# iPERDance/iPERCore

Hardware: AMD Instinct MI355X
Metric: synthesized frames/sec at 512x512 (run_imitator) (higher is better)
Workload: dtype f32; 1 GPU; run_imitator 512x512 single src/ref pair, 300-frame reference clip frame-sharded over 1 GPU(s), AttLWB-SPADE generator fp32 (BASELINE configs[1] at N = 1, configs[2] at N = 8); poses=imitate, image_size=512, frame_batch=300, frame_batch_requested=384, world_size=1, parallelism=frame-shard x1, batches_in_flight=1, weights=random-init (seeded) of the real architecture, 36,276,992 params

## Files before the change

### include/lwg_hip.h

```cpp
#ifndef LWG_HIP_H
#define LWG_HIP_H

#include <stddef.h>
#include <stdint.h>

#ifdef __cplusplus
extern "C" {
#endif

typedef void* lwg_stream_t;

#define LWG_ABI_VERSION 10
int lwg_abi_version(void);

#define LWG_MAX_TAPS 52
enum { LWG_EPI_NONE = 0, LWG_EPI_RESIDUAL = 1, LWG_EPI_SPADE = 2 };
enum { LWG_ACTIVATION_NONE = 0, LWG_ACTIVATION_RELU = 1, LWG_ACTIVATION_TANH = 2, LWG_ACTIVATION_SIGMOID = 3 };
#define LWG_ACTIVATION_RELU_MASK 5
enum { LWG_DT_F32 = 0, LWG_DT_BF16 = 1,
       LWG_DT_F32_Q4 = 2 };

typedef struct LwgConvArgs {
    const float* x0;
    const float* x1;
    int C0, C1;
    int B, H, W;
    int OH, OW;
    int M;
    int stride;
    int ntaps;
    int cshift;
    const float* w;
    int N;
    const float* bias;
    float* y;
    int YH, YW, YC, ycoff;
    int omul, ooy, oox;
    int epi;
    int act;
    const float* res;
    const float* xn;
    const float* mean;
    const float* rstd;
    int xdt;
    int ydt;
    signed char dy[LWG_MAX_TAPS];
    signed char dx[LWG_MAX_TAPS];
} LwgConvArgs;

int lwg_conv2d_nhwc_f32(const LwgConvArgs* args, lwg_stream_t stream);
size_t lwg_conv2d_ws_floats(const LwgConvArgs* args);
int lwg_conv2d_nhwc_f32_ws(const LwgConvArgs* args, float* ws, lwg_stream_t stream);
int lwg_conv_slice_count(const LwgConvArgs* args);

int lwg_conv2d_nhwc_bf16(const LwgConvArgs* args, lwg_stream_t stream);
int lwg_conv2d_winograd_f32(const LwgConvArgs* args, lwg_stream_t stream);
size_t lwg_conv2d_winograd_ws_floats(const LwgConvArgs* args);
int lwg_conv2d_winograd_f32_ws(const LwgConvArgs* args, float* ws, lwg_stream_t stream);
int lwg_conv2d_winograd_plan(const LwgConvArgs* args, int with_ws, long long* blocks, int* slices, int* nbv, int* workgroups);
int lwg_winograd_panel_f32(const float* wpanel, float* upk, int Cin, int N, const int* tap9, lwg_stream_t stream);
typedef struct LwgWinoDesc {
    const float* wpanel;
    float* upk;
    int Cin, N, first_block;
    int tap9[9];
} LwgWinoDesc;
int lwg_winograd_panels_f32(const LwgWinoDesc* descs_dev, int ndesc, int total_blocks, lwg_stream_t stream);
int lwg_conv2d_winograd4_f32(const LwgConvArgs* args, lwg_stream_t stream);
int lwg_winograd4_panel_f32(const float* wpanel, float* upk, int Cin, int N, const int* tap9, lwg_stream_t stream);
int lwg_conv2d_nhwc_bf16_hr(const LwgConvArgs* args, lwg_stream_t stream);
int lwg_conv2d_winograd_bf16(const LwgConvArgs* args, lwg_stream_t stream);
int lwg_conv2d_nhwc_c8_bf16(const LwgConvArgs* args, lwg_stream_t stream);
int lwg_conv_transpose4_nhwc_bf16(const LwgConvArgs* args, lwg_stream_t stream);
int lwg_conv_transpose4_nhwc_f32(const LwgConvArgs* args, lwg_stream_t stream);
int lwg_conv_transpose4_is_one_grid(const LwgConvArgs* args);
int lwg_conv_transpose4_winograd_f32(const LwgConvArgs* args, lwg_stream_t stream);

int lwg_conv_transpose4_winograd24_f32(const LwgConvArgs* args, lwg_stream_t stream);

int lwg_conv2d_nhwc_f32_split(const LwgConvArgs* args, lwg_stream_t stream);

size_t lwg_conv2d_wgrad_ws_floats(int Ktot, int N, int M);
int lwg_conv2d_wgrad_nhwc_f32(const LwgConvArgs* args, const float* dy, float* dw, float* ws, lwg_stream_t stream);
int lwg_conv2d_wgrad_unpacked_f32(const LwgConvArgs* args, const float* dy, float* ws, float* dw, int D0, int D1, int KH, int KW,
                                  int transposed, const int* kidx, int cin, int nout, float* db, lwg_stream_t stream);
int lwg_colsum_nhwc_f32(const float* x, size_t rows, int C, float* out, float* ws, lwg_stream_t stream);
size_t lwg_conv2d_wgrad_winograd_ws_floats(const LwgConvArgs* args);
int lwg_conv2d_wgrad_winograd_f32(const LwgConvArgs* args, const float* dy, float* ws, float* dw, int cin, int nout, lwg_stream_t stream);

int lwg_act_bwd_f32(const float* dy, const float* y, size_t n, int act, float* out, lwg_stream_t stream);
int lwg_norm_fwd_nhwc_f32(const float* x, const float* mean, const float* rstd, const float* gamma, const float* beta, int gstride,
                          int B, int HW, int C, int act, float* y, lwg_stream_t stream);
int lwg_norm_bwd_nhwc_f32(const float* dy, const float* y, const float* x, const float* mean, const float* rstd,
                          const float* gamma, int gstride, int B, int HW, int C, int act, int nsplit, float* dx, float* dgamma,
                          float* dbeta, float* ws, lwg_stream_t stream);
int lwg_adam_step_f32(float* p, const float* g, float* m, float* v, size_t n, float lr, float beta1, float beta2, float eps, int t,
                      lwg_stream_t stream);
int lwg_adam_step_dev_f32(float* p, const float* g, float* m, float* v, size_t n, float lr, float beta1, float beta2, float eps,
                          int* t_dev, lwg_stream_t stream);
int lwg_pack_panel_f32(const float* w, int D0, int D1, int KH, int KW, int transposed, const int* kidx, int ntaps, int cin,
                       int cin_pad, int nout, int n_pad, float* out, lwg_stream_t stream);
int lwg_unpack_wgrad_f32(const float* dwk, int D0, int D1, int KH, int KW, int transposed, const int* kidx, int ntaps, int cin,
                         int cin_pad, int nout, int n_pad, float* dw, lwg_stream_t stream);
typedef struct LwgPackDesc {
    const float* w;
    float* out;
    int D1, KHW, transposed, ntaps, cin, cin_pad, nout, n_pad, Kp, first_block;
    int kidx[LWG_MAX_TAPS];
} LwgPackDesc;
int lwg_pack_panels_f32(const LwgPackDesc* descs_dev, int ndesc, int total_blocks, lwg_stream_t stream);
int lwg_maxpool2_fwd_nhwc_f32(const float* x, float* y, int B, int H, int W, int C, lwg_stream_t stream);
int lwg_maxpool2_bwd_nhwc_f32(const float* x, const float* dy, float* dx, int B, int H, int W, int C, lwg_stream_t stream);
int lwg_crop_resize_bilinear_f32(const float* x, const long long* box, float* y, float* valid, int N, int C, int H, int W, int OH, int OW,
                                 lwg_stream_t stream);
int lwg_crop_resize_bilinear_bwd_f32(const float* dy, const long long* box, float* dx, int N, int C, int H, int W, int OH, int OW, lwg_stream_t stream);
int lwg_prelu_f32(const float* x, const float* slope, const float* res, size_t rows, int C, float* y, lwg_stream_t stream);
int lwg_prelu_bwd_f32(const float* x, const float* slope, const float* dy, size_t rows, int C, float* dx, lwg_stream_t stream);

int lwg_instnorm_stats_nhwc_f32(const float* x, int B, int HW, int C, float eps, float* mean, float* rstd,
                                float* ws, int nsplit, lwg_stream_t stream);
int lwg_instnorm_stats_nhwc_bf16(const void* x, int B, int HW, int C, float eps, float* mean, float* rstd, float* ws, int nsplit,
                                 lwg_stream_t stream);
int lwg_instnorm_apply_nhwc_f32(const float* x, const float* mean, const float* rstd, const float* res,
                                float* y, int B, int HW, int C, int act, lwg_stream_t stream);

int lwg_flow_resize_f32(const float* T, int n, int S, int h, int w, float* out, lwg_stream_t stream);
int lwg_lwb_attention_f32(const float* q, const float* Ks, const float* Vs, const float* bk, const float* bv,
                          const float* T, float* out, int B, int ns, int h, int w, int C, int S,
                          int src_batched, lwg_stream_t stream);
int lwg_lwb_attention_bf16(const void* q, const void* Ks, const void* Vs, const float* bk, const float* bv, const float* T, void* out,
                           int B, int ns, int h, int w, int C, int S, int src_batched, lwg_stream_t stream);
int lwg_lwb_attention_x_records(int h, int w, int C, int element_size);
int lwg_lwb_attention_x_f32(const float* x, const float* Kq, const float* kappa, const float* Vs, const float* bv, const float* T,
                            float* out, float* stats, int B, int ns, int h, int w, int C, int src_batched, lwg_stream_t stream);
int lwg_lwb_attention_x_bf16(const void* x, const void* Kq, const float* kappa, const void* Vs, const float* bv, const float* T,
                             void* out, float* stats, int B, int ns, int h, int w, int C, int src_batched, lwg_stream_t stream);
size_t lwg_instnorm_finalize_ws_floats(int B, int C, int nrec);
int lwg_instnorm_finalize_f32(float* ws, int B, int C, int nrec, float eps, float* mean, float* rstd, lwg_stream_t stream);
int lwg_lwb_attention_bwd_f32(const float* q, const float* Ks, const float* Vs, const float* bk, const float* bv,
                              const float* T, const float* dout, float* dq, float* dKs, float* dVs, int B, int ns,
                              int h, int w, int C, int S, int src_batched, lwg_stream_t stream);
int lwg_lwb_attention_kv_f32(const float* q, const float* kv, const float* bk, const float* bv, const float* T, float* out,
                             int B, int ns, int h, int w, int C, int S, int src_batched, lwg_stream_t stream);
int lwg_lwb_attention_kv_bwd_f32(const float* q, const float* kv, const float* bk, const float* bv, const float* T,
                                 const float* dout, float* dq, float* dkv, int B, int ns, int h, int w, int C, int S,
                                 int src_batched, lwg_stream_t stream);
int lwg_lwb_fuse_f32(const float* tsf_x, const float* src_x, const float* gate, const float* T, float* out, int B, int ns,
                     int h, int w, int C, int S, int src_batched, float scale_w, float scale_o, lwg_stream_t stream);
int lwg_lwb_fuse_bf16(const void* tsf_x, const void* src_x, const void* gate, const float* T, void* out, int B, int ns, int h, int w,
                      int C, int S, int src_batched, float scale_w, float scale_o, lwg_stream_t stream);
int lwg_lwb_fuse_bwd_f32(const float* src_x, const float* gate, const float* T, const float* dout, float* d_tsf, float* d_src,
                         float* d_gate, int B, int ns, int h, int w, int C, int S, int src_batched, float scale_w, float scale_o,
                         lwg_stream_t stream);

size_t lwg_rasterize_ws_bytes(int B, int nf, int S);
int lwg_project_faces_f32(const float* verts, const float* cam, const int32_t* faces, int B, int nv, int nf,
                          float eye_dist, float* faces_v, float* f2pts, lwg_stream_t stream);
int lwg_rasterize_fim_wim_f32(const float* faces_v, int B, int nf, int S, float near, float far, int32_t* fim,
                              float* wim, void* ws, lwg_stream_t stream);
int lwg_texture_sample_f32(const int32_t* fim, const float* wim, const float* faces_v, const float* textures, int B, int nf,
                           int S, int T, int tex_batched, float eps, const float* bg_color3_host, float* rgb, lwg_stream_t stream);

int lwg_flow_compose_f32(const int32_t* fim, const float* wim, int B, int S, const float* map_fn, int nf,
                         const float* f_uvs2img, const float* uv_img4, int Hu, int Wu, const float* src_f2pts,
                         int ns, float* tsf_inputs, float* Tst, float* cond_nchw, float* Tuv, lwg_stream_t stream);
int lwg_bc_transform_f32(const float* f2pts, const int32_t* fim, const float* wim, int B, int S, int nf, float* T,
                         lwg_stream_t stream);
int lwg_encode_fim_f32(const int32_t* fim, const float* map_fn, int B, int S, int nf, int D, float* out,
                       lwg_stream_t stream);

size_t lwg_smpl_lbs_ws_floats(int B, int nv, int nj);
int lwg_smpl_lbs_f32(const float* pose, int pose_stride, const float* beta, int beta_stride, int nbeta,
                     const float* cam, int cam_stride, const float* v_template, const float* offsets, int off_batched,
                     const float* shapedirs, const float* posedirs, const float* J_regressor, const int32_t* parents,
                     const float* lbs_weights, const int32_t* links, int nlinks, int B, int nv, int nj, float* verts,
                     float* j3d, float* j2d, float* ws, lwg_stream_t stream);

int lwg_head_compose_f32(const float* x, const float* wpk, const float* bg, size_t bg_bstride, int B, int S, int C,
                         float* pred, float* mask, float* img, lwg_stream_t stream);
int lwg_head_compose_q4_f32(const float* x, const float* wpk, const float* bg, size_t bg_bstride, int B, int S, int C,
                            float* pred, float* mask, float* img, lwg_stream_t stream);
int lwg_thin_conv_f32(const float* x, const float* wpk, int B, int S, int C, int ks, float* y, lwg_stream_t stream);
int lwg_head_compose_bf16(const void* x, const void* wb, const float* bg, size_t bg_bstride, int B, int S, int C, float* pred,
                          float* mask, float* img, lwg_stream_t stream);
int lwg_up4_head_compose_bf16(const LwgConvArgs* args, const void* whead, const float* bg, size_t bg_bstride, float* pred, float* mask, float* img,
                              lwg_stream_t stream);
int lwg_frames_to_u8(const float* pred, int B, int S, int bgr, uint8_t* out, lwg_stream_t stream);
int lwg_nchw_to_nhwc_f32(const float* src, float* dst, int B, int C, int Cp, int P, lwg_stream_t stream);
int lwg_nhwc_to_nchw_f32(const float* src, float* dst, int B, int C, int Cs, int P, lwg_stream_t stream);

int lwg_morph_f32(const float* in, float* out, int n, int H, int W, int ks, int mode, float* ws, lwg_stream_t stream);
int lwg_canny_f32(const float* sil, int n, int H, int W, const float* gauss9, const float* sobelx9, float low, float high,
                  float* edges, float* ws, lwg_stream_t stream);
int lwg_boundary_fill_f32(const float* src, const float* confidant, const float* outpad, const float* edges, int n, int H,
                          int W, float* out, int32_t* top3, int32_t* ws, lwg_stream_t stream);
int lwg_grid_sample_nchw_f32(const float* img, size_t img_bstride, const float* grid, int n, int C, int H, int W, int Ho,
                             int Wo, float* out, lwg_stream_t stream);
int lwg_uv_merge_f32(const float* src_warp, const float* vis, int ns, int H, int W, float* out, lwg_stream_t stream);
int lwg_uv_merge_parts_f32(const float* uv_imgs, const float* vis, int n, int H, int W, float* out, lwg_stream_t stream);
int lwg_pack_inputs_f32(const float* a, int Ca, const float* b, int Cb, const float* mask, int n, int H, int W, int Cp,
                        float* out, lwg_stream_t stream);

int lwg_device_cu_count(void);

#ifdef __cplusplus
}
#endif
#endif
```

### ipercore_amd/_lib.py

```python
import ctypes
import os
import re

_HERE = os.path.dirname(os.path.abspath(__file__))
LIB_PATH = os.path.join(_HERE, "liblwg_hip.so")
HEADER_PATH = os.path.join(os.path.dirname(_HERE), "include", "lwg_hip.h")

LWG_MAX_TAPS = 52
EPI_NONE, EPI_RESIDUAL, EPI_SPADE = 0, 1, 2
ACT_NONE, ACT_RELU, ACT_TANH, ACT_SIGMOID, ACT_LRELU = 0, 1, 2, 3, 4
ACT_RELU_MASK = 5
DT_F32, DT_BF16, DT_F32_Q4 = 0, 1, 2

c_f = ctypes.c_void_p
c_i = ctypes.c_int


class LwgConvArgs(ctypes.Structure):
    _fields_ = [
        ("x0", c_f), ("x1", c_f),
        ("C0", c_i), ("C1", c_i),
        ("B", c_i), ("H", c_i), ("W", c_i),
        ("OH", c_i), ("OW", c_i),
        ("M", c_i), ("stride", c_i), ("ntaps", c_i), ("cshift", c_i),
        ("w", c_f), ("N", c_i), ("bias", c_f),
        ("y", c_f), ("YH", c_i), ("YW", c_i), ("YC", c_i), ("ycoff", c_i),
        ("omul", c_i), ("ooy", c_i), ("oox", c_i),
        ("epi", c_i), ("act", c_i),
        ("res", c_f), ("xn", c_f), ("mean", c_f), ("rstd", c_f),
        ("xdt", c_i), ("ydt", c_i),
        ("dy", ctypes.c_byte * LWG_MAX_TAPS), ("dx", ctypes.c_byte * LWG_MAX_TAPS),
    ]


class LwgWinoDesc(ctypes.Structure):
    _fields_ = [("wpanel", ctypes.c_void_p), ("upk", ctypes.c_void_p), ("Cin", c_i), ("N", c_i), ("first_block", c_i), ("tap9", c_i * 9)]


class LwgPackDesc(ctypes.Structure):
    _fields_ = [("w", c_f), ("out", c_f)] + [(n, c_i) for n in ("D1", "KHW", "transposed", "ntaps", "cin", "cin_pad", "nout", "n_pad", "Kp",
                                                               "first_block")] + [("kidx", c_i * LWG_MAX_TAPS)]


_SIGS = {
    "lwg_abi_version": (c_i, []),
    "lwg_device_cu_count": (c_i, []),
    "lwg_conv2d_nhwc_f32": (c_i, [ctypes.POINTER(LwgConvArgs), c_f]),
    "lwg_conv2d_ws_floats": (ctypes.c_size_t, [ctypes.POINTER(LwgConvArgs)]),
    "lwg_conv2d_nhwc_f32_ws": (c_i, [ctypes.POINTER(LwgConvArgs), c_f, c_f]),
    "lwg_conv2d_nhwc_bf16": (c_i, [ctypes.POINTER(LwgConvArgs), c_f]),
    "lwg_conv2d_winograd_f32": (c_i, [ctypes.POINTER(LwgConvArgs), c_f]),
    "lwg_conv2d_winograd_ws_floats": (ctypes.c_size_t, [ctypes.POINTER(LwgConvArgs)]),
    "lwg_conv2d_winograd_f32_ws": (c_i, [ctypes.POINTER(LwgConvArgs), c_f, c_f]),
    "lwg_conv2d_winograd_plan": (c_i, [ctypes.POINTER(LwgConvArgs), c_i, ctypes.POINTER(ctypes.c_longlong), ctypes.POINTER(c_i), ctypes.POINTER(c_i),
                                       ctypes.POINTER(c_i)]),
    "lwg_winograd_panel_f32": (c_i, [c_f, c_f, c_i, c_i, ctypes.POINTER(c_i), c_f]),
    "lwg_winograd_panels_f32": (c_i, [c_f, c_i, c_i, c_f]),
    "lwg_conv2d_winograd4_f32": (c_i, [ctypes.POINTER(LwgConvArgs), c_f]),
    "lwg_winograd4_panel_f32": (c_i, [c_f, c_f, c_i, c_i, ctypes.POINTER(c_i), c_f]),
    "lwg_conv2d_nhwc_bf16_hr": (c_i, [ctypes.POINTER(LwgConvArgs), c_f]),
    "lwg_conv2d_winograd_bf16": (c_i, [ctypes.POINTER(LwgConvArgs), c_f]),
    "lwg_conv2d_nhwc_c8_bf16": (c_i, [ctypes.POINTER(LwgConvArgs), c_f]),
    "lwg_conv_transpose4_nhwc_bf16": (c_i, [ctypes.POINTER(LwgConvArgs), c_f]),
    "lwg_conv_transpose4_nhwc_f32": (c_i, [ctypes.POINTER(LwgConvArgs), c_f]),
    "lwg_conv_transpose4_winograd_f32": (c_i, [ctypes.POINTER(LwgConvArgs), c_f]),
    "lwg_conv_transpose4_winograd24_f32": (c_i, [ctypes.POINTER(LwgConvArgs), c_f]),
    "lwg_conv_transpose4_is_one_grid": (c_i, [ctypes.POINTER(LwgConvArgs)]),
    "lwg_conv_slice_count": (c_i, [ctypes.POINTER(LwgConvArgs)]),
    "lwg_conv2d_nhwc_f32_split": (c_i, [ctypes.POINTER(LwgConvArgs), c_f]),
    "lwg_conv2d_wgrad_ws_floats": (ctypes.c_size_t, [c_i, c_i, c_i]),
    "lwg_conv2d_wgrad_nhwc_f32": (c_i, [ctypes.POINTER(LwgConvArgs), c_f, c_f, c_f, c_f]),
    "lwg_conv2d_wgrad_unpacked_f32": (c_i, [ctypes.POINTER(LwgConvArgs), c_f, c_f, c_f] + [c_i] * 5 + [ctypes.POINTER(ctypes.c_int), c_i, c_i, c_f, c_f]),
    "lwg_colsum_nhwc_f32": (c_i, [c_f, ctypes.c_size_t, c_i, c_f, c_f, c_f]),
    "lwg_conv2d_wgrad_winograd_ws_floats": (ctypes.c_size_t, [ctypes.POINTER(LwgConvArgs)]),
    "lwg_conv2d_wgrad_winograd_f32": (c_i, [ctypes.POINTER(LwgConvArgs), c_f, c_f, c_f, c_i, c_i, c_f]),
    "lwg_act_bwd_f32": (c_i, [c_f, c_f, ctypes.c_size_t, c_i, c_f, c_f]),
    "lwg_norm_fwd_nhwc_f32": (c_i, [c_f, c_f, c_f, c_f, c_f, c_i, c_i, c_i, c_i, c_i, c_f, c_f]),
    "lwg_norm_bwd_nhwc_f32": (c_i, [c_f, c_f, c_f, c_f, c_f, c_f, c_i, c_i, c_i, c_i, c_i, c_i, c_f, c_f, c_f, c_f, c_f]),
    "lwg_adam_step_f32": (c_i, [c_f, c_f, c_f, c_f, ctypes.c_size_t, ctypes.c_float, ctypes.c_float, ctypes.c_float, ctypes.c_float, c_i, c_f]),
    "lwg_adam_step_dev_f32": (c_i, [c_f, c_f, c_f, c_f, ctypes.c_size_t, ctypes.c_float, ctypes.c_float, ctypes.c_float, ctypes.c_float, c_f, c_f]),
    "lwg_pack_panel_f32": (c_i, [c_f] + [c_i] * 5 + [ctypes.POINTER(ctypes.c_int)] + [c_i] * 5 + [c_f, c_f]),
    "lwg_pack_panels_f32": (c_i, [c_f, c_i, c_i, c_f]),
    "lwg_unpack_wgrad_f32": (c_i, [c_f] + [c_i] * 5 + [ctypes.POINTER(ctypes.c_int)] + [c_i] * 5 + [c_f, c_f]),
    "lwg_maxpool2_fwd_nhwc_f32": (c_i, [c_f, c_f, c_i, c_i, c_i, c_i, c_f]),
    "lwg_maxpool2_bwd_nhwc_f32": (c_i, [c_f, c_f, c_f, c_i, c_i, c_i, c_i, c_f]),
    "lwg_crop_resize_bilinear_f32": (c_i, [c_f, c_f, c_f, c_f, c_i, c_i, c_i, c_i, c_i, c_i, c_f]),
    "lwg_crop_resize_bilinear_bwd_f32": (c_i, [c_f, c_f, c_f, c_i, c_i, c_i, c_i, c_i, c_i, c_f]),
    "lwg_prelu_f32": (c_i, [c_f, c_f, c_f, ctypes.c_size_t, c_i, c_f, c_f]),
    "lwg_prelu_bwd_f32": (c_i, [c_f, c_f, c_f, ctypes.c_size_t, c_i, c_f, c_f]),
    "lwg_instnorm_stats_nhwc_f32": (c_i, [c_f, c_i, c_i, c_i, ctypes.c_float, c_f, c_f, c_f, c_i, c_f]),
    "lwg_instnorm_apply_nhwc_f32": (c_i, [c_f, c_f, c_f, c_f, c_f, c_i, c_i, c_i, c_i, c_f]),
    "lwg_lwb_attention_f32": (c_i, [c_f, c_f, c_f, c_f, c_f, c_f, c_f, c_i, c_i, c_i, c_i, c_i, c_i, c_i, c_f]),
    "lwg_lwb_attention_bf16": (c_i, [c_f, c_f, c_f, c_f, c_f, c_f, c_f, c_i, c_i, c_i, c_i, c_i, c_i, c_i, c_f]),
    "lwg_instnorm_stats_nhwc_bf16": (c_i, [c_f, c_i, c_i, c_i, ctypes.c_float, c_f, c_f, c_f, c_i, c_f]),
    "lwg_head_compose_bf16": (c_i, [c_f, c_f, c_f, ctypes.c_size_t, c_i, c_i, c_i, c_f, c_f, c_f, c_f]),
    "lwg_up4_head_compose_bf16": (c_i, [ctypes.POINTER(LwgConvArgs), c_f, c_f, ctypes.c_size_t, c_f, c_f, c_f, c_f]),
    "lwg_flow_resize_f32": (c_i, [c_f, c_i, c_i, c_i, c_i, c_f, c_f]),
    "lwg_lwb_fuse_f32": (c_i, [c_f] * 5 + [c_i] * 7 + [ctypes.c_float, ctypes.c_float, c_f]),
    "lwg_lwb_fuse_bf16": (c_i, [c_f] * 5 + [c_i] * 7 + [ctypes.c_float, ctypes.c_float, c_f]),
    "lwg_lwb_fuse_bwd_f32": (c_i, [c_f] * 7 + [c_i] * 7 + [ctypes.c_float, ctypes.c_float, c_f]),
    "lwg_lwb_attention_x_f32": (c_i, [c_f] * 8 + [c_i] * 6 + [c_f]),
    "lwg_lwb_attention_x_bf16": (c_i, [c_f] * 8 + [c_i] * 6 + [c_f]),
    "lwg_lwb_attention_x_records": (c_i, [c_i, c_i, c_i, c_i]),
    "lwg_instnorm_finalize_ws_floats": (ctypes.c_size_t, [c_i, c_i, c_i]),
    "lwg_instnorm_finalize_f32": (c_i, [c_f, c_i, c_i, c_i, ctypes.c_float, c_f, c_f, c_f]),
    "lwg_lwb_attention_bwd_f32": (c_i, [c_f] * 10 + [c_i] * 7 + [c_f]),
    "lwg_lwb_attention_kv_f32": (c_i, [c_f] * 6 + [c_i] * 7 + [c_f]),
    "lwg_lwb_attention_kv_bwd_f32": (c_i, [c_f] * 8 + [c_i] * 7 + [c_f]),
    "lwg_rasterize_ws_bytes": (ctypes.c_size_t, [c_i, c_i, c_i]),
    "lwg_project_faces_f32": (c_i, [c_f, c_f, c_f, c_i, c_i, c_i, ctypes.c_float, c_f, c_f, c_f]),
    "lwg_rasterize_fim_wim_f32": (c_i, [c_f, c_i, c_i, c_i, ctypes.c_float, ctypes.c_float, c_f, c_f, c_f, c_f]),
    "lwg_texture_sample_f32": (c_i, [c_f, c_f, c_f, c_f, c_i, c_i, c_i, c_i, c_i, ctypes.c_float, ctypes.POINTER(ctypes.c_float), c_f, c_f]),
    "lwg_flow_compose_f32": (c_i, [c_f, c_f, c_i, c_i, c_f, c_i, c_f, c_f, c_i, c_i, c_f, c_i, c_f, c_f, c_f, c_f, c_f]),
    "lwg_bc_transform_f32": (c_i, [c_f, c_f, c_f, c_i, c_i, c_i, c_f, c_f]),
    "lwg_encode_fim_f32": (c_i, [c_f, c_f, c_i, c_i, c_i, c_i, c_f, c_f]),
    "lwg_smpl_lbs_ws_floats": (ctypes.c_size_t, [c_i, c_i, c_i]),
    "lwg_smpl_lbs_f32": (c_i, [c_f, c_i, c_f, c_i, c_i, c_f, c_i, c_f, c_f, c_i, c_f, c_f, c_f, c_f, c_f, c_f, c_i, c_i, c_i,
                               c_i, c_f, c_f, c_f, c_f, c_f]),
    "lwg_head_compose_f32": (c_i, [c_f, c_f, c_f, ctypes.c_size_t, c_i, c_i, c_i, c_f, c_f, c_f, c_f]),
    "lwg_head_compose_q4_f32": (c_i, [c_f, c_f, c_f, ctypes.c_size_t, c_i, c_i, c_i, c_f, c_f, c_f, c_f]),
    "lwg_thin_conv_f32": (c_i, [c_f, c_f, c_i, c_i, c_i, c_i, c_f, c_f]),
    "lwg_nchw_to_nhwc_f32": (c_i, [c_f, c_f, c_i, c_i, c_i, c_i, c_f]),
    "lwg_nhwc_to_nchw_f32": (c_i, [c_f, c_f, c_i, c_i, c_i, c_i, c_f]),
    "lwg_frames_to_u8": (c_i, [c_f, c_i, c_i, c_i, c_f, c_f]),
    "lwg_morph_f32": (c_i, [c_f, c_f, c_i, c_i, c_i, c_i, c_i, c_f, c_f]),
    "lwg_canny_f32": (c_i, [c_f, c_i, c_i, c_i, ctypes.POINTER(ctypes.c_float), ctypes.POINTER(ctypes.c_float),
                            ctypes.c_float, ctypes.c_float, c_f, c_f, c_f]),
    "lwg_boundary_fill_f32": (c_i, [c_f, c_f, c_f, c_f, c_i, c_i, c_i, c_f, c_f, c_f, c_f]),
    "lwg_grid_sample_nchw_f32": (c_i, [c_f, ctypes.c_size_t, c_f, c_i, c_i, c_i, c_i, c_i, c_i, c_f, c_f]),
    "lwg_uv_merge_f32": (c_i, [c_f, c_f, c_i, c_i, c_i, c_f, c_f]),
    "lwg_uv_merge_parts_f32": (c_i, [c_f, c_f, c_i, c_i, c_i, c_f, c_f]),
    "lwg_pack_inputs_f32": (c_i, [c_f, c_i, c_f, c_i, c_f, c_i, c_i, c_i, c_i, c_f, c_f]),
}

_lib = None


def header_symbols():
    with open(HEADER_PATH) as fp:
        src = re.sub(r"/\*.*?\*/", "", fp.read(), flags=re.S)
    return sorted(set(re.findall(r"\b(lwg_[a-z0-9_]+)\s*\(", src)))


def lib():
    global _lib
    if _lib is None:
        if not os.path.exists(LIB_PATH):
            raise RuntimeError(
                f"{LIB_PATH} not found: the HIP kernels are not built (run `python -c 'import __graft_entry__ as g; "
                "g.build()'` or `make -C ipercore_amd/csrc`).  There is no CPU fallback.")
        import torch
        handle = ctypes.CDLL(LIB_PATH)
        for name, (res, args) in _SIGS.items():
            fn = getattr(handle, name)
            fn.restype = res
            fn.argtypes = args
        if handle.lwg_abi_version() != 10:
            raise RuntimeError("liblwg_hip.so ABI version mismatch")
        _lib = handle
    return _lib


def check(err, what):
    if err != 0:
        raise RuntimeError(f"{what} failed with hipError_t {err}")
```

### ipercore_amd/csrc/conv_winograd4.hip

```cpp
#include <hip/hip_runtime.h>
#include "lwg_common.h"
#include "lwg_conv_wino.h"

#define W4_THREADS 512
#define W4_PBX 8
#define W4_PBY 4
#define W4_NB 64
#define W4_KS 8
#define W4_HW 34
#define W4_HH 18
#ifndef W4_RS
#define W4_RS 40
#endif
#define W4_PLANE (18 * W4_RS + 4)
#define W4_RAW (W4_KS * W4_PLANE)
#define W4_VS (36 * W4_KS * 32)
#define W4_NEL (W4_HW * W4_HH * 2)
#define W4_NQ 3
#define W4_DUMP_OFF (2 * W4_RAW + 2 * W4_VS)
#define W4_DUMP (W4_THREADS + 3 * W4_PLANE)
#define W4_LOOP (W4_DUMP_OFF + W4_DUMP)
#define W4_MSR 68
#define W4_NPL 28
#define W4_MS (W4_NPL * 16 * W4_MSR)
#define W4_BIAS_OFF (W4_LOOP > W4_MS ? W4_LOOP : W4_MS)
#ifndef LWG_W4_XCD
#define LWG_W4_XCD 1
#endif
#ifndef LWG_W4_CHUNK
#define LWG_W4_CHUNK 1
#endif
#ifndef LWG_W4_RDMAP
#define LWG_W4_RDMAP 1
#endif
#ifndef LWG_W4_SMALL
#define LWG_W4_SMALL 1
#endif
#define W4SB() __builtin_amdgcn_sched_barrier(0)

#ifdef LWG_W4_TS
#define W4TS(i) do { if (tid == 0 && lab_bi == 1) reinterpret_cast<unsigned long long*>(const_cast<float*>(a.res))[(size_t)blockIdx.x * 16 + (i)] = __builtin_readcyclecounter(); } while (0)
#define W4TSA(i) do { if (tid == 0) reinterpret_cast<unsigned long long*>(const_cast<float*>(a.res))[(size_t)blockIdx.x * 16 + (i)] = __builtin_readcyclecounter(); } while (0)
#else
#define W4TS(i) do { } while (0)
#define W4TSA(i) do { } while (0)
#endif

#ifndef W4_NT
#define W4_NT 0
#endif
#ifndef W4_NT_LD
#define W4_NT_LD W4_NT
#endif
#ifndef W4_NT_RES
#define W4_NT_RES 0
#endif
#ifndef W4_NT_ST
#define W4_NT_ST 2
#endif

__device__ __forceinline__ void w4_bt6(const float (&r)[6], float (&v)[6]) {
    const float a = __builtin_fmaf(-4.f, r[2], r[4]), b = __builtin_fmaf(-4.f, r[1], r[3]);
    const float c = r[4] - r[2], e = r[3] - r[1];
    v[0] = __builtin_fmaf(-5.f, r[2], __builtin_fmaf(4.f, r[0], r[4]));
    v[1] = a + b;
    v[2] = a - b;
    v[3] = __builtin_fmaf(2.f, e, c);
    v[4] = __builtin_fmaf(-2.f, e, c);
    v[5] = __builtin_fmaf(-5.f, r[3], __builtin_fmaf(4.f, r[1], r[5]));
}

template <int EPI, bool TWO, bool SM = false>
__global__ __launch_bounds__(SM ? 256 : W4_THREADS, 1) void lwg_conv_winograd4_kernel(const LwgConvArgs a) {
    constexpr bool SMS = SM && EPI == LWG_EPI_SPADE;
    constexpr int NVP = SM && !SMS ? 2 : 1;
    constexpr int NTH = SM ? 256 : W4_THREADS;
    constexpr int NQ = SM ? 5 : W4_NQ;
    constexpr int NBV = SM ? 32 : W4_NB;
    constexpr int MSR = SM ? 36 : W4_MSR;
    constexpr int NHF = SM ? 2 : 1;
    extern __shared__ __attribute__((aligned(16))) float smem[];
    const int wid = __builtin_amdgcn_readfirstlane(threadIdx.x >> 6);
    const float* __restrict__ bias = a.bias;
    const int H = a.H, W = a.W, Cin = a.C0 + a.C1, N = a.N;
    float* __restrict__ y = a.y;
    float* const raw0 = smem;
    float* const Ms = smem;
    const int tid = threadIdx.x, lane = tid & 63;
    const CwGrid g = cw_grid(a.B, H, W, N, 4 * W4_PBX, 4 * W4_PBY, NBV);
    const CwOrder o = cw_order(cw4_order_kind(LWG_W4_XCD, LWG_W4_CHUNK, SM, gridDim.x, N / NBV, Cin, N, g.tiles, g.total), gridDim.x, blockIdx.x, N / NBV, g);
    int blk = blockIdx.x;
    const int nst = Cin / W4_KS;
    const __amdgpu_buffer_rsrc_t ru = __builtin_amdgcn_make_buffer_rsrc(const_cast<float*>(a.w), 0, (int)(144u * (unsigned)Cin * (unsigned)N), 0x00020000);
    const int q = wid & 3, ct = SM ? 0 : wid >> 2;
    const int half = SM ? 0 : wid >> 2;
    floatx16 acc[9];
    CwBlock<NQ, TWO> bk;
    unsigned uvoff, uvoffc;
    auto setup = [&](int id) {
        int cb, t;
        cw_block(o, id, cb, t);
        bk.locate(a, g, t, 4 * W4_PBX, 4 * W4_PBY, SMS ? cw4_n0_spade_small(cb) : cw_n0(cb, NBV));
        int tids = tid;
        asm volatile("" : "+v"(tids));
        bk.halo(a, tids, NTH, W4_HW, W4_NEL);
        const int col = SMS ? bk.n0 + (((lane & 31) >> 4) << 5) + (lane & 15) : bk.n0 + ct * 32 + (lane & 31);
        uvoff = (unsigned)(((lane >> 5) * 9 * N + 4 * col) * 4);
        uvoffc = (unsigned)(((lane >> 5) * 9 * N + 8 * N + col) * 4);
    };
    setup(blk);
    int wst[NQ];
#pragma unroll
    for (int k = 0; k < NQ; ++k) {
        const int i = tid + NTH * k;
        const int pix = i >> 1, hq = i & 1, hy = pix / W4_HW, hx = pix - hy * W4_HW;
        wst[k] = i < W4_NEL ? 4 * hq * W4_PLANE + hy * W4_RS + hx : W4_DUMP_OFF + tid;
    }
    floatx4 rreg[NQ];
    auto rld1 = [&](int st, int k) -> floatx4 {
#ifdef W4_LAB_HFIX
        const int c = 0 * st;
#else
        const int c = st * W4_KS;
#endif
        return bk.template rld1<W4_NT_LD>(a, c, k);
    };
    auto rst1 = [&](int buf, int k, floatx4 v) { cw_rst1(raw0 + buf * W4_RAW + wst[k], W4_PLANE, v); };
    floatx4 ufa[4], ufb[4];
    float ufc[4];
    const unsigned ukk = (unsigned)N * 72u;
    const unsigned uq = (unsigned)q * (unsigned)nst * 4u * ukk;
    const unsigned ubo = (unsigned)N * 16u;
    auto uldpart = [&](int set, int st, int kk, int part) {
#ifdef W4_LAB_UFIX
        const unsigned so = uq + 0u * (unsigned)(st + kk);
#else
        const unsigned so = uq + (unsigned)(st * 4 + kk) * ukk;
#endif
        if (part == 0) ufa[set] = cw_buf_load(ru, uvoff, so);
        else if (part == 1) ufb[set] = cw_buf_load(ru, uvoff, so + ubo);
        else ufc[set] = __builtin_bit_cast(float, __builtin_amdgcn_raw_buffer_load_b32(ru, (int)uvoffc, (int)so, 0));
    };
    auto uldset = [&](int set, int st, int kk) {
#ifdef W4_LAB_UFIX
        const unsigned so = uq + 0u * (unsigned)(st + kk);
#else
        const unsigned so = uq + (unsigned)(st * 4 + kk) * ukk;
#endif
        ufa[set] = cw_buf_load(ru, uvoff, so);
        ufb[set] = cw_buf_load(ru, uvoff, so + ubo);
        ufc[set] = __builtin_bit_cast(float, __builtin_amdgcn_raw_buffer_load_b32(ru, (int)uvoffc, (int)so, 0));
    };
    const int patch = tid & 31, tc = (tid >> 5) & 7;
    const int pty = patch >> 3, ptx = patch & 7;
    unsigned dbs = (unsigned)(tc * W4_PLANE + (4 * pty) * W4_RS + 4 * ptx) >> 2;
    asm volatile("" : "+v"(dbs));
    dbs <<= 2;
    unsigned dbx[NHF], vbx[NHF], vbt[NHF];
    float alpha[NHF], beta[NHF], nbeta[NHF];
#pragma unroll
    for (int hi = 0; hi < NHF; ++hi) {
        const int hf = SM ? hi : half;
        dbx[hi] = (unsigned)(tc * W4_PLANE + (4 * pty + hf) * W4_RS + 4 * ptx) >> 2;
        asm volatile("" : "+v"(dbx[hi]));
        dbx[hi] <<= 2;
        vbx[hi] = (unsigned)(2 * W4_RAW + (hf ? 30 : 0) * W4_KS * 32 + tc * 32 + patch);
        vbt[hi] = (unsigned)(2 * W4_RAW + (hf ? 18 : 6) * W4_KS * 32 + tc * 32 + patch);
        asm volatile("" : "+v"(vbx[hi]));
        asm volatile("" : "+v"(vbt[hi]));
        alpha[hi] = hf ? -1.f : -4.f;
        beta[hi] = hf ? 2.f : 1.f;
        nbeta[hi] = -beta[hi];
    }
    unsigned fbs[2];
    fbs[0] = (unsigned)(2 * W4_RAW + (6 * q) * W4_KS * 32 + lane);
    fbs[1] = (unsigned)(2 * W4_RAW + (6 * (4 + (q >> 1)) + 3 * (q & 1)) * W4_KS * 32 + lane);
    asm volatile("" : "+v"(fbs[0]));
    asm volatile("" : "+v"(fbs[1]));
    float fb[9];
    auto frag1 = [&](int buf, int kk, int j) -> float {
        return smem[fbs[j < 6 ? 0 : 1] + buf * W4_VS + ((j < 6 ? j : j - 6) * W4_KS + 2 * kk) * 32];
    };
    auto rd6 = [&](unsigned base, int buf, int r, float (&d)[6]) {
        const floatx4 v4 = *reinterpret_cast<const floatx4*>(smem + base + buf * W4_RAW + r * W4_RS);
        const float2 v2 = *reinterpret_cast<const float2*>(smem + base + buf * W4_RAW + r * W4_RS + 4);
        d[0] = v4[0]; d[1] = v4[1]; d[2] = v4[2]; d[3] = v4[3]; d[4] = v2.x; d[5] = v2.y;
    };
    auto vst6 = [&](unsigned base, int buf, int i, const float (&v)[6]) {
        float* dst = smem + base + buf * W4_VS + (6 * i) * W4_KS * 32;
#pragma unroll
        for (int nu = 0; nu < 6; ++nu) dst[nu * W4_KS * 32] = v[nu];
    };
    auto transform_full = [&](int buf) {
#pragma unroll
        for (int hi = 0; hi < NHF; ++hi) {
            float X[6], P[6], Q[6], v[6];
            {
                float dR[3][6];
                rd6(dbx[hi], buf, 0, dR[0]); rd6(dbx[hi], buf, 2, dR[1]); rd6(dbx[hi], buf, 4, dR[2]);
#pragma unroll
                for (int j = 0; j < 6; ++j) X[j] = __builtin_fmaf(-5.f, dR[1][j], __builtin_fmaf(4.f, dR[0][j], dR[2][j]));
            }
            {
                float dR[2][6];
                rd6(dbs, buf, 2, dR[0]); rd6(dbs, buf, 4, dR[1]);
#pragma unroll
                for (int j = 0; j < 6; ++j) P[j] = __builtin_fmaf(alpha[hi], dR[0][j], dR[1][j]);
                rd6(dbs, buf, 1, dR[0]); rd6(dbs, buf, 3, dR[1]);
#pragma unroll
                for (int j = 0; j < 6; ++j) Q[j] = __builtin_fmaf(alpha[hi], dR[0][j], dR[1][j]);
            }
            w4_bt6(X, v); vst6(vbx[hi], buf, 0, v);
            float T[6];
#pragma unroll
            for (int j = 0; j < 6; ++j) T[j] = __builtin_fmaf(beta[hi], Q[j], P[j]);
            w4_bt6(T, v); vst6(vbt[hi], buf, 0, v);
#pragma unroll
            for (int j = 0; j < 6; ++j) T[j] = __builtin_fmaf(nbeta[hi], Q[j], P[j]);
            w4_bt6(T, v); vst6(vbt[hi], buf, 1, v);
        }
    };
    auto iteration = [&](int s, auto SET, auto NXT) {
        constexpr int set = decltype(SET)::value;
        constexpr bool nxt = decltype(NXT)::value != 0;
        const int s3 = s + 3 < nst ? s + 3 : nst - 1;
        float X[6], P[6], Q[6], dR[3][6];
        auto mf = [&](int kk, int j, bool refill) {
            acc[j] = __builtin_amdgcn_mfma_f32_32x32x2f32(j < 4 ? ufa[kk][j & 3] : j < 8 ? ufb[kk][j & 3] : ufc[kk], fb[j], acc[j], 0, 0, 0);
#ifndef W4_KO_FRAG
            if (refill && (j & 1)) {
                fb[j - 1] = kk < 3 ? frag1(set, kk + 1, j - 1) : frag1(set ^ 1, 0, j - 1);
                fb[j] = kk < 3 ? frag1(set, kk + 1, j) : frag1(set ^ 1, 0, j);
            } else if (refill && j == 8) {
                fb[8] = kk < 3 ? frag1(set, kk + 1, 8) : frag1(set ^ 1, 0, 8);
            }
#endif
            W4SB();
        };
        auto ul = [&](int kk, int part) {
#ifndef W4_KO_ULD
            if (kk < 2) uldpart(kk + 2, s, kk + 2, part);
            else if (nxt) uldpart(kk - 2, s + 1, kk - 2, part);
#endif
            W4SB();
        };
        auto halo = [&](int k) {
#ifdef W4_KO_HALO
            return;
#endif
            if (nxt) { rst1(set, k, rreg[k]); rreg[k] = rld1(s3, k); }
            W4SB();
        };
#ifdef W4_KO_TR
        constexpr bool trn = false;
#else
        constexpr bool trn = nxt;
#endif
        auto tr = [&](int hi, int step) {
            if (trn) {
                if (step < 3) rd6(dbx[hi], set ^ 1, 2 * step, dR[step]);
                else if (step < 5) {
#pragma unroll
                    for (int j = 3 * (step - 3); j < 3 * (step - 3) + 3; ++j) X[j] = __builtin_fmaf(-5.f, dR[1][j], __builtin_fmaf(4.f, dR[0][j], dR[2][j]));
                } else if (step < 7) rd6(dbs, set ^ 1, 2 * (step - 5) + 2, dR[step - 5]);
                else if (step == 7) {
                    float v[6];
                    w4_bt6(X, v);
                    vst6(vbx[hi], set ^ 1, 0, v);
                } else if (step == 8) {
#pragma unroll
                    for (int j = 0; j < 6; ++j) P[j] = __builtin_fmaf(alpha[hi], dR[0][j], dR[1][j]);
                } else if (step < 11) rd6(dbs, set ^ 1, 2 * (step - 9) + 1, dR[step - 9]);
                else if (step == 11) {
#pragma unroll
                    for (int j = 0; j < 6; ++j) Q[j] = __builtin_fmaf(alpha[hi], dR[0][j], dR[1][j]);
                } else {
                    float T[6], v[6];
#pragma unroll
                    for (int j = 0; j < 6; ++j) T[j] = __builtin_fmaf(step == 12 ? beta[hi] : nbeta[hi], Q[j], P[j]);
                    w4_bt6(T, v);
                    vst6(vbt[hi], set ^ 1, step - 12, v);
                }
            }
            W4SB();
        };
        if constexpr (!SM) {
            mf(0, 0, true); ul(0, 0);
            mf(0, 1, true); halo(0);
            mf(0, 2, true); ul(0, 1); tr(0, 0);
            mf(0, 3, true); halo(1); tr(0, 1);
            mf(0, 4, true); ul(0, 2); tr(0, 2);
            mf(0, 5, true); halo(2);
            mf(0, 6, true); tr(0, 3);
            mf(0, 7, true); tr(0, 4);
            mf(0, 8, true); tr(0, 5);
            mf(1, 0, true); ul(1, 0); tr(0, 6);
            mf(1, 1, true); tr(0, 7);
            mf(1, 2, true); ul(1, 1); tr(0, 8); tr(0, 9);
            mf(1, 3, true); tr(0, 10);
            mf(1, 4, true); ul(1, 2);
            mf(1, 5, true); tr(0, 11);
            mf(1, 6, true); tr(0, 12);
            mf(1, 7, true);
            mf(1, 8, true); tr(0, 13);
            mf(2, 0, true); ul(2, 0);
            mf(2, 1, true);
            mf(2, 2, true); ul(2, 1);
            mf(2, 3, true);
            mf(2, 4, true); ul(2, 2);
            mf(2, 5, true); mf(2, 6, true); mf(2, 7, true); mf(2, 8, true);
        } else {
            mf(0, 0, true); ul(0, 0); halo(0);
            mf(0, 1, true); tr(0, 0);
            mf(0, 2, true); ul(0, 1); tr(0, 1);
            mf(0, 3, true); halo(1); tr(0, 2);
            mf(0, 4, true); ul(0, 2); tr(0, 3);
            mf(0, 5, true); halo(2); tr(0, 4);
            mf(0, 6, true); tr(0, 5);
            mf(0, 7, true); halo(3); tr(0, 6);
            mf(0, 8, true); tr(0, 7);
            mf(1, 0, true); ul(1, 0); tr(0, 8); tr(0, 9);
            mf(1, 1, true); halo(4); tr(0, 10);
            mf(1, 2, true); ul(1, 1); tr(0, 11);
            mf(1, 3, true); tr(0, 12);
            mf(1, 4, true); ul(1, 2); tr(0, 13);
            mf(1, 5, true); tr(1, 0);
            mf(1, 6, true); tr(1, 1);
            mf(1, 7, true); tr(1, 2);
            mf(1, 8, true); tr(1, 3);
            mf(2, 0, true); ul(2, 0); tr(1, 4);
            mf(2, 1, true); tr(1, 5);
            mf(2, 2, true); ul(2, 1); tr(1, 6);
            mf(2, 3, true); tr(1, 7);
            mf(2, 4, true); ul(2, 2); tr(1, 8); tr(1, 9);
            mf(2, 5, true); tr(1, 10);
            mf(2, 6, true); tr(1, 11);
            mf(2, 7, true); tr(1, 12);
            mf(2, 8, true); tr(1, 13);
        }
        __syncthreads();
        W4SB();
        mf(3, 0, nxt); ul(3, 0);
        mf(3, 1, nxt);
        mf(3, 2, nxt); ul(3, 1);
        mf(3, 3, nxt);
        mf(3, 4, nxt); ul(3, 2);
        mf(3, 5, nxt); mf(3, 6, nxt); mf(3, 7, nxt); mf(3, 8, nxt);
    };

    floatx4 r0[NQ], r1[NQ];
    float bq;
    auto issue_loads = [&]() {
        bq = bias ? bias[SMS ? bk.n0 + (((tid & 31) >> 4) << 5) + (tid & 15) : bk.n0 + (tid & (NBV - 1))] : 0.f;
#pragma unroll
        for (int k = 0; k < NQ; ++k) {
            r0[k] = rld1(0, k);
            r1[k] = rld1(1, k);
        }
        uldset(0, 0, 0);
        uldset(1, 0, 1);
#pragma unroll
        for (int k = 0; k < NQ; ++k) rreg[k] = rld1(nst > 2 ? 2 : 1, k);
    };
    issue_loads();
#ifdef LWG_W4_TS
    int lab_bi = 0;
#endif
    W4TSA(11);
    for (;;) {
    W4TS(0);
#pragma unroll
    for (int k = 0; k < NQ; ++k) {
        rst1(0, k, r0[k]);
        rst1(1, k, r1[k]);
    }
    if (tid < NBV) smem[W4_BIAS_OFF + tid] = bq;
    __syncthreads();
    transform_full(0);
    __syncthreads();
#pragma unroll
    for (int j = 0; j < 9; ++j) fb[j] = frag1(0, 0, j);
#pragma unroll
    for (int j = 0; j < 9; ++j)
#pragma unroll
        for (int r = 0; r < 16; ++r) acc[j][r] = 0.f;
    if (q == 1) {
#pragma unroll
        for (int g = 0; g < 4; ++g) {
            const floatx4 b4 = *reinterpret_cast<const floatx4*>(smem + W4_BIAS_OFF + ct * 32 + 8 * g + 4 * (lane >> 5));
#pragma unroll
            for (int k = 0; k < 4; ++k) acc[1][4 * g + k] = b4[k];
        }
    }
    W4TS(1);
    {
        int s = 0;
        for (; s + 2 < nst; s += 2) {
            iteration(s, IntC<0>(), IntC<1>());
            iteration(s + 1, IntC<1>(), IntC<1>());
        }
        iteration(s, IntC<0>(), IntC<1>());
        iteration(s + 1, IntC<1>(), IntC<0>());
    }
    W4TS(2);
    const int eb = bk.b, ex0 = bk.x0, ey0 = bk.y0, en0 = bk.n0;
#pragma unroll
    for (int r = 0; r < 16; ++r) {
        const float m0 = acc[0][r], m1 = acc[1][r], m2 = acc[2][r], m3 = acc[3][r], m4 = acc[4][r], m5 = acc[5][r];
        const float s12 = m1 + m2, d12 = m1 - m2, s34 = m3 + m4, d34 = m3 - m4;
        acc[0][r] = (m0 + s12) + s34;
        acc[1][r] = __builtin_fmaf(2.f, d34, d12);
        acc[2][r] = __builtin_fmaf(4.f, s34, s12);
        acc[3][r] = __builtin_fmaf(8.f, d34, d12) + m5;
    }
    if (q & 1) {
#pragma unroll
        for (int r = 0; r < 16; ++r) {
            const float h0 = acc[6][r], h1 = acc[7][r];
            acc[6][r] = h0 + h1;
            acc[7][r] = h0 - h1;
        }
    } else {
#pragma unroll
        for (int r = 0; r < 16; ++r) {
            const float h0 = acc[6][r], h1 = acc[7][r], h2 = acc[8][r];
            acc[6][r] = (h0 + h1) + h2;
            acc[7][r] = h1 - h2;
            acc[8][r] = h1 + h2;
        }
    }
    W4TS(4);
    int tide = tid;
    asm volatile("" : "+v"(tide));
    const int lanee = tide & 63;
    const int rb = wid & 3;
    const unsigned l5 = (unsigned)lanee & 31u, gsel = (0x0FF0F00Fu >> l5) & 1u;
    const int gidx = __builtin_popcount((gsel ? 0x0FF0F00Fu : 0xF00F0FF0u) & ((1u << l5) - 1u));
    const int p16 = LWG_W4_RDMAP && !SM ? (wid >> 2) * 4 + 2 * (lanee >> 5) + (gsel ? 0 : 1) + 8 * (gidx >> 3) : (wid >> 2) * 8 + (lanee >> 3);
    const int n4 = SMS ? (lanee & 3) * 4 : LWG_W4_RDMAP && !SM ? (gidx & 7) * 4 : (lanee & 7) * 4;
    const int cbase = SMS ? (en0 >> 6) * 32 + ((en0 >> 4) & 1) * 16 : en0 >> 1;
    floatx4 mu, rs;
    if (EPI == LWG_EPI_SPADE) {
        mu = *reinterpret_cast<const floatx4*>(a.mean + (size_t)eb * a.YC + cbase + n4);
        rs = *reinterpret_cast<const floatx4*>(a.rstd + (size_t)eb * a.YC + cbase + n4);
    }
    typedef unsigned int w4_u4 __attribute__((ext_vector_type(4)));
    const unsigned img_bytes = (unsigned)(H * W) * (unsigned)a.YC * 4u;
    const __amdgpu_buffer_rsrc_t ry = __builtin_amdgcn_make_buffer_rsrc(y + (size_t)eb * H * W * a.YC, 0, (int)img_bytes, 0x00020000);
    const float* const esrc = EPI == LWG_EPI_SPADE ? a.xn : EPI == LWG_EPI_RESIDUAL ? a.res : a.y;
    const __amdgpu_buffer_rsrc_t re = __builtin_amdgcn_make_buffer_rsrc(const_cast<float*>(esrc) + (size_t)eb * H * W * a.YC, 0, (int)img_bytes, 0x00020000);
    const int chan = EPI == LWG_EPI_SPADE ? cbase + n4 : a.ycoff + en0 + n4;
    bool more = false;
    int nblk = blk;
#pragma unroll
    for (int ph = 0; ph < 2; ++ph) {
        if (ph == 1) __syncthreads();
        if (((lanee >> 4) & 1) == ph) {
            float* dst = Ms + (lanee & 15) * MSR + ct * 32 + 4 * (lanee >> 5);
#pragma unroll
            for (int g = 0; g < 4; ++g) {
#pragma unroll
                for (int bb = 0; bb < 4; ++bb)
                    *reinterpret_cast<floatx4*>(dst + (4 * q + bb) * 16 * MSR + 8 * g) = floatx4{acc[bb][4 * g], acc[bb][4 * g + 1], acc[bb][4 * g + 2], acc[bb][4 * g + 3]};
#pragma unroll
                for (int i = 0; i < 3; ++i)
                    *reinterpret_cast<floatx4*>(dst + (16 + 3 * q + i) * 16 * MSR + 8 * g) = floatx4{acc[6 + i][4 * g], acc[6 + i][4 * g + 1], acc[6 + i][4 * g + 2], acc[6 + i][4 * g + 3]};
            }
        }
        unsigned vo[NVP][4];
#pragma unroll
        for (int hp = 0; hp < NVP; ++hp) {
            const int p = ph * 16 + (SMS ? lanee >> 2 : SM ? 8 * hp + (lanee >> 3) : p16);
            const int ox = ex0 + 4 * (p & 7) + rb, oyb = ey0 + 4 * (p >> 3);
#pragma unroll
            for (int i = 0; i < 4; ++i)
                vo[hp][i] = cw4_out_voff(ox, oyb + i, H, W, a.YC, chan);
        }
        floatx4 ext[2][4];
        if (EPI != LWG_EPI_NONE) {
#pragma unroll
            for (int h = 0; h < (EPI == LWG_EPI_SPADE ? 1 : 2); ++h)
#pragma unroll
                for (int i = 0; i < 4; ++i) ext[h][i] = __builtin_bit_cast(floatx4, __builtin_amdgcn_raw_buffer_load_b128(re, (int)cw4_out_group(vo[NVP == 2 ? h : 0][i], h, !SM), 0, W4_NT_RES));
        }
        if (ph == 1) {
            W4TS(8);
            nblk = blk + (int)gridDim.x;
            more = cw_has_block(o, nblk);
            setup(more ? nblk : blk);
            W4TS(9);
            issue_loads();
            W4TS(10);
        }
        __syncthreads();
        if (ph == 0) W4TS(5); else W4TS(7);
        floatx4 gam[4];
#pragma unroll
        for (int h = 0; h < 2; ++h) {
            const float* base = Ms + (SMS ? lanee >> 2 : SM ? 8 * h + (lanee >> 3) : p16) * MSR + (SMS ? h * 16 : SM ? 0 : h * 32) + n4;
            floatx4 F[6];
#pragma unroll
            for (int xi = 0; xi < 4; ++xi) F[xi] = *reinterpret_cast<const floatx4*>(base + (4 * xi + rb) * 16 * MSR);
            const int ia = rb == 0 ? 0 : rb == 2 ? 2 : 1, ib = (rb & 1) ? 4 : 3;
            const float cb = (float)(1 << rb);
#pragma unroll
            for (int r = 0; r < 2; ++r) {
                const float* hb = base + (16 + 6 * r) * 16 * MSR;
                const floatx4 pa = *reinterpret_cast<const floatx4*>(hb + ia * 16 * MSR);
                const floatx4 pb = *reinterpret_cast<const floatx4*>(hb + ib * 16 * MSR);
                floatx4 f;
#pragma unroll
                for (int c = 0; c < 4; ++c) f[c] = __builtin_fmaf(cb, pb[c], pa[c]);
                if (rb == 3) f += *reinterpret_cast<const floatx4*>(hb + 5 * 16 * MSR);
                F[4 + r] = f;
            }
            floatx4 o[4];
#pragma unroll
            for (int c = 0; c < 4; ++c) {
                const float s12 = F[1][c] + F[2][c], d12 = F[1][c] - F[2][c], s34 = F[3][c] + F[4][c], d34 = F[3][c] - F[4][c];
                o[0][c] = (F[0][c] + s12) + s34;
                o[1][c] = __builtin_fmaf(2.f, d34, d12);
                o[2][c] = __builtin_fmaf(4.f, s34, s12);
                o[3][c] = __builtin_fmaf(8.f, d34, d12) + F[5][c];
            }
            if (EPI == LWG_EPI_SPADE) {
                if (h == 0) {
#pragma unroll
                    for (int i = 0; i < 4; ++i) gam[i] = o[i];
                    continue;
                }
#pragma unroll
                for (int i = 0; i < 4; ++i)
#pragma unroll
                    for (int c = 0; c < 4; ++c) o[i][c] = (ext[0][i][c] - mu[c]) * rs[c] * (1.f + gam[i][c]) + o[i][c];
            } else if (EPI == LWG_EPI_RESIDUAL) {
                if (a.act == LWG_ACT_RELU_MASK) {
#pragma unroll
                    for (int i = 0; i < 4; ++i)
#pragma unroll
                        for (int c = 0; c < 4; ++c) o[i][c] = ext[h][i][c] > 0.f ? o[i][c] : 0.f;
                } else {
#pragma unroll
                    for (int i = 0; i < 4; ++i) o[i] += ext[h][i];
                }
            }
            lwg_act_dispatch(a.act, [&](auto ACTC) {
                constexpr int EA = decltype(ACTC)::value;
#pragma unroll
                for (int i = 0; i < 4; ++i)
#pragma unroll
                    for (int c = 0; c < 4; ++c) o[i][c] = lwg_act_c<EA>(o[i][c], a.act);
            });
#pragma unroll
            for (int i = 0; i < 4; ++i)
                __builtin_amdgcn_raw_buffer_store_b128(__builtin_bit_cast(w4_u4, o[i]), ry, (int)cw4_out_group(vo[NVP == 2 ? h : 0][i], h, EPI != LWG_EPI_SPADE && !SM), 0, W4_NT_ST);
        }
        if (ph == 0) W4TS(6);
    }
    W4TS(3);
#ifdef LWG_W4_TS
    ++lab_bi;
#endif
    if (!more) break;
    blk = nblk;
    __syncthreads();
    }
    W4TSA(12);
#ifdef LWG_W4_TS
    if (tid == 0) reinterpret_cast<unsigned long long*>(const_cast<float*>(a.res))[(size_t)blockIdx.x * 16 + 13] = (unsigned long long)lab_bi;
#endif
}


__global__ __launch_bounds__(256) void lwg_winograd4_panel_kernel(const float* __restrict__ wp, float* __restrict__ U, int Cin, int N, LwgWinoTaps taps) {
    const int n = blockIdx.x * 64 + (threadIdx.x & 63), c = blockIdx.y * 4 + (threadIdx.x >> 6);
    if (n >= N || c >= Cin) return;
    double g[3][3];
#pragma unroll
    for (int r = 0; r < 3; ++r)
#pragma unroll
        for (int s = 0; s < 3; ++s) {
            const int k = ((c >> 5) * 9 + taps.t[3 * r + s]) * 32 + (c & 31);
            g[r][s] = (double)wp[((size_t)(k >> 2) * N + n) * 4 + (k & 3)];
        }
    const double G[6][3] = {{1.0 / 4, 0, 0}, {-1.0 / 6, -1.0 / 6, -1.0 / 6}, {-1.0 / 6, 1.0 / 6, -1.0 / 6}, {1.0 / 24, 1.0 / 12, 1.0 / 6}, {1.0 / 24, -1.0 / 12, 1.0 / 6}, {0, 0, 1}};
    double t[6][3];
#pragma unroll
    for (int i = 0; i < 6; ++i)
#pragma unroll
        for (int s = 0; s < 3; ++s) t[i][s] = G[i][0] * g[0][s] + G[i][1] * g[1][s] + G[i][2] * g[2][s];
    const int s8 = c >> 3, kk = (c & 7) >> 1, kh = c & 1;
#pragma unroll
    for (int qq = 0; qq < 4; ++qq) {
        float* dst = U + ((((size_t)qq * (Cin >> 3) + s8) * 4 + kk) * 2 + kh) * 9 * (size_t)N;
        float o[9];
#pragma unroll
        for (int j = 0; j < 9; ++j) {
            const int xi = j < 6 ? qq : 4 + (qq >> 1), nu = j < 6 ? j : 3 * (qq & 1) + (j - 6);
            o[j] = (float)(t[xi][0] * G[nu][0] + t[xi][1] * G[nu][1] + t[xi][2] * G[nu][2]);
        }
        *reinterpret_cast<floatx4*>(dst + 4 * n) = floatx4{o[0], o[1], o[2], o[3]};
        *reinterpret_cast<floatx4*>(dst + 4 * (size_t)N + 4 * n) = floatx4{o[4], o[5], o[6], o[7]};
        dst[8 * (size_t)N + n] = o[8];
    }
}

extern "C" int lwg_winograd4_panel_f32(const float* wpanel, float* upk, int Cin, int N, const int* tap9, lwg_stream_t stream_) {
    LwgWinoTaps taps;
    if (!cw_panel_args_ok(wpanel, upk, Cin, N, tap9, taps)) return (int)hipErrorInvalidValue;
    hipLaunchKernelGGL(lwg_winograd4_panel_kernel, dim3((unsigned)((N + 63) / 64), (unsigned)((Cin + 3) / 4)), dim3(256), 0,
                       reinterpret_cast<hipStream_t>(stream_), wpanel, upk, Cin, N, taps);
    return (int)hipGetLastError();
}

template <int EPI, bool SM>
static int lwg_wino4_go(const LwgConvArgs& a, dim3 grid, size_t lds, hipStream_t stream) {
    return a.C1 > 0 ? cw_launch<lwg_conv_winograd4_kernel<EPI, true, SM>>(grid, SM ? 256 : W4_THREADS, lds, stream, a)
                    : cw_launch<lwg_conv_winograd4_kernel<EPI, false, SM>>(grid, SM ? 256 : W4_THREADS, lds, stream, a);
}

extern "C" int lwg_conv2d_winograd4_f32(const LwgConvArgs* pa, lwg_stream_t stream_) {
    hipStream_t stream = reinterpret_cast<hipStream_t>(stream_);
    if (!pa || !cw_contract_ok(*pa, 144ull, 256ll)) return (int)hipErrorInvalidValue;
    const LwgConvArgs& a = *pa;
    const size_t lds = (size_t)(W4_BIAS_OFF + 64) * 4;
    const int cus = lwg_device_cus();
    long long total = cw_total_blocks(a.B, a.H, a.W, a.N, 4 * W4_PBX, 4 * W4_PBY, W4_NB);
    const bool sm = LWG_W4_SMALL && 2 * total <= cus;
    if (sm) total *= 2;
    const dim3 grid = cw_persistent_grid(total, cus);
    if (a.epi == LWG_EPI_SPADE) return sm ? lwg_wino4_go<LWG_EPI_SPADE, true>(a, grid, lds, stream) : lwg_wino4_go<LWG_EPI_SPADE, false>(a, grid, lds, stream);
    if (a.epi == LWG_EPI_RESIDUAL) return sm ? lwg_wino4_go<LWG_EPI_RESIDUAL, true>(a, grid, lds, stream) : lwg_wino4_go<LWG_EPI_RESIDUAL, false>(a, grid, lds, stream);
    return sm ? lwg_wino4_go<LWG_EPI_NONE, true>(a, grid, lds, stream) : lwg_wino4_go<LWG_EPI_NONE, false>(a, grid, lds, stream);
}
```

### ipercore_amd/csrc/lwb_attn_x.hip

```cpp
#include "lwg_common.h"
#include "lwg_conv_args.h"

typedef unsigned int uintx4 __attribute__((ext_vector_type(4)));

template <typename ST> struct AttnXTraits;
template <> struct AttnXTraits<float> {
    static constexpr int CPL = 4;
    __device__ static __forceinline__ void unpack(const uintx4 v, float (&f)[4]) {
#pragma unroll
        for (int k = 0; k < 4; ++k) {
            const unsigned u = v[k];
            f[k] = __builtin_bit_cast(float, u);
        }
    }
    __device__ static __forceinline__ uintx4 pack(const float (&f)[4]) {
        uintx4 v;
#pragma unroll
        for (int k = 0; k < 4; ++k) v[k] = __builtin_bit_cast(unsigned, f[k]);
        return v;
    }
};
template <> struct AttnXTraits<__bf16> {
    static constexpr int CPL = 8;
    __device__ static __forceinline__ void unpack(const uintx4 v, float (&f)[8]) {
#pragma unroll
        for (int k = 0; k < 4; ++k) {
            f[2 * k] = __builtin_bit_cast(float, v[k] << 16);
            f[2 * k + 1] = __builtin_bit_cast(float, v[k] & 0xffff0000u);
        }
    }
    __device__ static __forceinline__ uintx4 pack(const float (&f)[8]) {
        typedef __bf16 bf16x2 __attribute__((ext_vector_type(2)));
        uintx4 v;
#pragma unroll
        for (int k = 0; k < 4; ++k) {
            bf16x2 p;
            p[0] = (__bf16)f[2 * k];
            p[1] = (__bf16)f[2 * k + 1];
            v[k] = __builtin_bit_cast(unsigned, p);
        }
        return v;
    }
};

template <typename ST, int LPP, bool STATS, int NSU, int PW, int OCC, bool PIPE = false>
__global__ __launch_bounds__(256 * PW, PW == 1 ? OCC : 1) void lwg_lwb_attnx_kernel(const ST* __restrict__ x, const ST* __restrict__ Kq,
                                                                 const float* __restrict__ kappa, const ST* __restrict__ Vs,
                                                                 const float* __restrict__ bv, const float* __restrict__ T,
                                                                 ST* __restrict__ out, float* __restrict__ stats, int B, int ns, int h, int w,
                                                                 int src_batched) {
    using TR = AttnXTraits<ST>;
    constexpr int CPL = TR::CPL;
    constexpr int C = CPL * LPP;
    constexpr int PPW = 64 / LPP;
    constexpr int PPP = 4 * PPW;
    constexpr int NPASS = 64 / PPP;
    constexpr int NIT = NPASS / PW;
    static_assert(NPASS % PW == 0, "PW must divide the tile's pass count");
    constexpr int NT = NSU > 0 ? NSU : 1;
    constexpr unsigned ROWB = (unsigned)C * sizeof(ST);
    const int lane = threadIdx.x & 63, wid = threadIdx.x >> 6;
    const int wq = wid & 3, pl = wid >> 2;
    const int cl = lane % LPP, pg = lane / LPP;
    const int tiles_x = (w + 7) >> 3;
    int tile, b;
    if (LWG_ATTNX_INTERLEAVE) {
        const int xcd = blockIdx.x & 7;
        const long idx = blockIdx.x >> 3;
        const long grp = idx / B;
        tile = (int)(grp * 8 + xcd);
        b = (int)(idx - grp * B);
        if (tile >= tiles_x * ((h + 7) >> 3)) return;
    } else {
        const long L = lwg_xcd_remap(blockIdx.x, gridDim.x);
        tile = (int)(L / B);
        b = (int)(L - (long)tile * B);
    }
    const int ty = tile / tiles_x, tx = tile - ty * tiles_x;
    const int hw = h * w;
    const unsigned nsrc = (unsigned)(src_batched ? B * ns : ns);
    __amdgpu_buffer_rsrc_t rK = __builtin_amdgcn_make_buffer_rsrc(const_cast<ST*>(Kq), 0, (int)(nsrc * (unsigned)hw * ROWB), 0x00020000);
    __amdgpu_buffer_rsrc_t rV = __builtin_amdgcn_make_buffer_rsrc(const_cast<ST*>(Vs), 0, (int)(nsrc * (unsigned)hw * ROWB), 0x00020000);
    __amdgpu_buffer_rsrc_t rA = __builtin_amdgcn_make_buffer_rsrc(const_cast<float*>(kappa), 0, (int)(nsrc * (unsigned)hw * 4u), 0x00020000);
    const float inv_sqrt_c = 1.0f / sqrtf((float)C);
    constexpr bool BV_REG = CPL == 4 || LWG_ATTNX_BVREG16;
    float bvr[CPL];
    if (BV_REG) {
#pragma unroll
        for (int k = 0; k < CPL; ++k) bvr[k] = bv[CPL * cl + k];
    }
    const float2* Tb = reinterpret_cast<const float2*>(T) + (size_t)b * ns * hw;

    auto pixel_of = [&](int pass, int& yc, int& xc) -> bool {
        const int p = pass * PPP + wq * PPW + pg;
        const int y = ty * 8 + (p >> 3), xx = tx * 8 + (p & 7);
        const bool live = y < h && xx < w;
        yc = live ? y : ty * 8;
        xc = live ? xx : tx * 8;
        return live;
    };
    extern __shared__ __attribute__((aligned(16))) char smem_ax[];
    char* xs = smem_ax;
    float2* Tl = reinterpret_cast<float2*>(smem_ax + NPASS * 4096);
    {
        __amdgpu_buffer_rsrc_t rX = __builtin_amdgcn_make_buffer_rsrc(const_cast<ST*>(x) + (size_t)b * hw * C, 0, (int)((unsigned)hw * ROWB), 0x00020000);
#pragma unroll
        for (int it = 0; it < NIT; ++it) {
            const int pass = it * PW + pl;
            int yc, xc;
            pixel_of(pass, yc, xc);
            const unsigned voff = (unsigned)(yc * w + xc) * ROWB + (unsigned)(CPL * cl) * (unsigned)sizeof(ST);
            __builtin_amdgcn_raw_ptr_buffer_load_lds(rX, (__attribute__((address_space(3))) void*)(xs + (pass * 4 + wq) * 1024), 16, (int)voff, 0, 0, 0);
        }
        for (int i = threadIdx.x; i < ns * 64; i += 256 * PW) {
            const int s = i >> 6, p = i & 63;
            const int y = ty * 8 + (p >> 3), xx = tx * 8 + (p & 7);
            const bool in = y < h && xx < w;
            Tl[i] = Tb[(size_t)s * hw + (size_t)(in ? y : ty * 8) * w + (in ? xx : tx * 8)];
        }
        asm volatile("s_waitcnt vmcnt(0)" ::: "memory");
        __syncthreads();
    }
    auto x_row = [&](int pass) -> uintx4 { return *reinterpret_cast<const uintx4*>(xs + ((pass * 4 + wq) * 64 + lane) * 16); };

    float shift[CPL], s1[CPL], s2[CPL];
    if (STATS) {
        TR::unpack(*reinterpret_cast<const uintx4*>(xs + cl * 16), shift);
#pragma unroll
        for (int k = 0; k < CPL; ++k) s1[k] = s2[k] = 0.f;
    }
    int nlive = 0;
    auto stats_add = [&](const float (&xv)[CPL]) {
        ++nlive;
        if (PW == 1) {
#pragma unroll
            for (int k = 0; k < CPL; ++k) {
                const float d = xv[k] - shift[k];
                s1[k] += d;
                s2[k] = __builtin_fmaf(d, d, s2[k]);
            }
        }
    };
    auto taps_of = [&](const float2 t, float (&wt)[4], int& tx0, int& ty0) {
        const float ix = ((t.x + 1.f) * (float)w - 1.f) * 0.5f, iy = ((t.y + 1.f) * (float)h - 1.f) * 0.5f;
        const float fx0 = floorf(ix), fy0 = floorf(iy);
        const float wx1 = ix - fx0, wy1 = iy - fy0, wx0 = (fx0 + 1.f) - ix, wy0 = (fy0 + 1.f) - iy;
        tx0 = (int)fminf(fmaxf(fx0, -2.f), (float)w + 1.f);
        ty0 = (int)fminf(fmaxf(fy0, -2.f), (float)h + 1.f);
        wt[0] = wy0 * wx0; wt[1] = wy0 * wx1; wt[2] = wy1 * wx0; wt[3] = wy1 * wx1;
    };
    auto fold = [&](const float (&ka)[CPL], const float (&va)[CPL], float kap, const float (&xv)[CPL], float& mrun, float& lrun, float (&o)[CPL]) {
        float dot = 0.f;
#pragma unroll
        for (int k = 0; k < CPL; ++k) dot = __builtin_fmaf(ka[k], xv[k], dot);
#pragma unroll
        for (int off = LPP >> 1; off > 0; off >>= 1) dot += __shfl_xor(dot, off, 64);
        const float logit = (dot + kap) * inv_sqrt_c;
        const float mnew = fmaxf(mrun, logit);
        const float corr = expf(mrun - mnew);
        const float pr = expf(logit - mnew);
        lrun = __builtin_fmaf(lrun, corr, pr);
#pragma unroll
        for (int k = 0; k < CPL; ++k) o[k] = __builtin_fmaf(o[k], corr, pr * va[k]);
        mrun = mnew;
    };
    auto finish = [&](long gp, float lrun, const float (&o)[CPL]) {
        const float invl = 1.f / lrun;
        float r[CPL];
        if (!BV_REG) {
#pragma unroll
            for (int k = 0; k < CPL; k += 4) {
                const floatx4 b4 = *reinterpret_cast<const floatx4*>(bv + CPL * cl + k);
#pragma unroll
                for (int j = 0; j < 4; ++j) bvr[k + j] = b4[j];
            }
        }
#pragma unroll
        for (int k = 0; k < CPL; ++k) r[k] = __builtin_fmaf(o[k], invl, bvr[k]);
        *reinterpret_cast<uintx4*>(out + gp * C + CPL * cl) = TR::pack(r);
    };

    if constexpr (PIPE) {
        static_assert(NSU == 2 && PW == 1 && (NIT % 2) == 0, "the pipelined form is the ns = 2 frame-batch form");
        bool mine = false;
#pragma unroll 1
        for (int it = 0; it < NIT; ++it) {
            int yc, xc;
            const bool live = pixel_of(it, yc, xc);
            const int ptile = it * PPP + wq * PPW + pg;
#pragma unroll
            for (int s = 0; s < 2; ++s) {
                const float2 t = Tl[s * 64 + ptile];
                float wt[4];
                int tx0, ty0;
                taps_of(t, wt, tx0, ty0);
                mine |= live && tx0 >= -1 && tx0 < w && ty0 >= -1 && ty0 < h;
            }
        }
        if (__syncthreads_or(mine ? 1 : 0) == 0) {
#pragma unroll 1
            for (int it = 0; it < NIT; ++it) {
                int yc, xc;
                const bool live = pixel_of(it, yc, xc);
                float xv[CPL];
                TR::unpack(x_row(it), xv);
                if (live) {
                    if (STATS) stats_add(xv);
                    float o[CPL];
#pragma unroll
                    for (int k = 0; k < CPL; ++k) o[k] = 0.f;
                    finish(((long)b * h + yc) * w + xc, 2.f, o);
                }
            }
        } else {
            struct Taps { uintx4 kr[2][4], vr[2][4]; float ar[2][4], wt[2][4]; };
            auto issue = [&](int pass, Taps& g) {
                int yc, xc;
                const bool live = pixel_of(pass, yc, xc);
                const int ptile = pass * PPP + wq * PPW + pg;
#pragma unroll
                for (int s = 0; s < 2; ++s) {
                    int tx0, ty0;
                    taps_of(Tl[s * 64 + ptile], g.wt[s], tx0, ty0);
                    const unsigned pbase = (unsigned)(src_batched ? b * ns + s : s) * (unsigned)hw;
#pragma unroll
                    for (int tp = 0; tp < 4; ++tp) {
                        const int tyy = ty0 + (tp >> 1), txx = tx0 + (tp & 1);
                        const bool ok = live && tyy >= 0 && tyy < h && txx >= 0 && txx < w;
                        const unsigned pix = pbase + (unsigned)(tyy * w + txx);
                        const unsigned voff = ok ? pix * ROWB + (unsigned)(CPL * cl) * (unsigned)sizeof(ST) : 0xC0000000u;
                        g.kr[s][tp] = __builtin_bit_cast(uintx4, __builtin_amdgcn_raw_buffer_load_b128(rK, (int)voff, 0, 0));
                        g.vr[s][tp] = __builtin_bit_cast(uintx4, __builtin_amdgcn_raw_buffer_load_b128(rV, (int)voff, 0, 0));
                        g.ar[s][tp] = __builtin_bit_cast(float, __builtin_amdgcn_raw_buffer_load_b32(rA, ok ? (int)(pix * 4u) : (int)0xC0000000u, 0, 0));
                    }
                }
            };
            auto consume = [&](int pass, const Taps& g) {
                int yc, xc;
                const bool live = pixel_of(pass, yc, xc);
                float xv[CPL];
                TR::unpack(x_row(pass), xv);
                if (STATS && live) stats_add(xv);
                float mrun = -INFINITY, lrun = 0.f;
                float o[CPL];
#pragma unroll
                for (int k = 0; k < CPL; ++k) o[k] = 0.f;
#pragma unroll
                for (int s = 0; s < 2; ++s) {
                    float ka[CPL], va[CPL], kap = 0.f;
#pragma unroll
                    for (int k = 0; k < CPL; ++k) ka[k] = va[k] = 0.f;
#pragma unroll
                    for (int tp = 0; tp < 4; ++tp) {
                        float k8[CPL], v8[CPL];
                        TR::unpack(g.kr[s][tp], k8);
                        TR::unpack(g.vr[s][tp], v8);
#pragma unroll
                        for (int k = 0; k < CPL; ++k) {
                            ka[k] = __builtin_fmaf(k8[k], g.wt[s][tp], ka[k]);
                            va[k] = __builtin_fmaf(v8[k], g.wt[s][tp], va[k]);
                        }
                        kap = __builtin_fmaf(g.ar[s][tp], g.wt[s][tp], kap);
                    }
                    fold(ka, va, kap, xv, mrun, lrun, o);
                }
                if (live) finish(((long)b * h + yc) * w + xc, lrun, o);
            };
            Taps g0, g1;
            issue(0, g0);
#pragma unroll 1
            for (int it = 0; it < NIT; it += 2) {
                issue(it + 1, g1);
                consume(it, g0);
                issue(it + 2 < NIT ? it + 2 : it + 1, g0);
                consume(it + 1, g1);
            }
        }
    } else {
#pragma unroll 1
    for (int it = 0; it < NIT; ++it) {
        const int pass = it * PW + pl;
        int yc, xc;
        const bool live = pixel_of(pass, yc, xc);
        const long gp = ((long)b * h + yc) * w + xc;
        const int ptile = pass * PPP + wq * PPW + pg;
        float xv[CPL];
        TR::unpack(x_row(pass), xv);
        if (STATS && live) stats_add(xv);
        float mrun = -INFINITY, lrun = 0.f;
        float o[CPL];
#pragma unroll
        for (int k = 0; k < CPL; ++k) o[k] = 0.f;

        auto source = [&](int s, const float2 t) {
            float wt[4];
            int tx0, ty0;
            taps_of(t, wt, tx0, ty0);
            const bool any_tap = live && tx0 >= -1 && tx0 < w && ty0 >= -1 && ty0 < h;
            float ka[CPL], va[CPL], kap = 0.f;
#pragma unroll
            for (int k = 0; k < CPL; ++k) ka[k] = va[k] = 0.f;
            if (__builtin_amdgcn_ballot_w64(any_tap) != 0ull) {
                const unsigned sidx = (unsigned)(src_batched ? b * ns + s : s);
                const unsigned pbase = sidx * (unsigned)hw;
                uintx4 kr[4], vr[4];
                float ar[4];
#pragma unroll
                for (int tp = 0; tp < 4; ++tp) {
                    const int tyy = ty0 + (tp >> 1), txx = tx0 + (tp & 1);
                    const bool ok = live && tyy >= 0 && tyy < h && txx >= 0 && txx < w;
                    const unsigned pix = pbase + (unsigned)(tyy * w + txx);
                    const unsigned voff = ok ? pix * ROWB + (unsigned)(CPL * cl) * (unsigned)sizeof(ST) : 0xC0000000u;
                    kr[tp] = __builtin_bit_cast(uintx4, __builtin_amdgcn_raw_buffer_load_b128(rK, (int)voff, 0, 0));
                    vr[tp] = __builtin_bit_cast(uintx4, __builtin_amdgcn_raw_buffer_load_b128(rV, (int)voff, 0, 0));
                    ar[tp] = __builtin_bit_cast(float, __builtin_amdgcn_raw_buffer_load_b32(rA, ok ? (int)(pix * 4u) : (int)0xC0000000u, 0, 0));
                }
#pragma unroll
                for (int tp = 0; tp < 4; ++tp) {
                    float k8[CPL], v8[CPL];
                    TR::unpack(kr[tp], k8);
                    TR::unpack(vr[tp], v8);
#pragma unroll
                    for (int k = 0; k < CPL; ++k) {
                        ka[k] = __builtin_fmaf(k8[k], wt[tp], ka[k]);
                        va[k] = __builtin_fmaf(v8[k], wt[tp], va[k]);
                    }
                    kap = __builtin_fmaf(ar[tp], wt[tp], kap);
                }
            }
            fold(ka, va, kap, xv, mrun, lrun, o);
        };
        if (NSU > 0) {
#pragma unroll
            for (int s = 0; s < NT; ++s) source(s, Tl[s * 64 + ptile]);
        } else {
#pragma unroll 1
            for (int s = 0; s < ns; ++s) source(s, Tl[s * 64 + ptile]);
        }
        if (live) finish(gp, lrun, o);
    }
    }

    if (STATS) {
        if (PW > 1) {
            __shared__ float acc[4][64][2 * CPL];
            if (pl == 0) {
#pragma unroll
                for (int k = 0; k < 2 * CPL; ++k) acc[wq][lane][k] = 0.f;
            }
            __syncthreads();
#pragma unroll 1
            for (int p = 0; p < NPASS; ++p) {
                if (pl == p % PW) {
                    int yc, xc;
                    if (pixel_of(p, yc, xc)) {
                        float xv[CPL];
                        TR::unpack(x_row(p), xv);
#pragma unroll
                        for (int k = 0; k < CPL; ++k) {
                            const float d = xv[k] - shift[k];
                            acc[wq][lane][k] += d;
                            acc[wq][lane][CPL + k] = __builtin_fmaf(d, d, acc[wq][lane][CPL + k]);
                        }
                    }
                }
                __syncthreads();
            }
            if (pl == 0) {
#pragma unroll
                for (int k = 0; k < CPL; ++k) {
                    s1[k] = acc[wq][lane][k];
                    s2[k] = acc[wq][lane][CPL + k];
                }
            }
        }
        __syncthreads();
        float (*sh)[2][C] = reinterpret_cast<float (*)[2][C]>(smem_ax);
        float* shn = reinterpret_cast<float*>(smem_ax + 4 * 2 * C * sizeof(float));
        float fn = (float)nlive;
#pragma unroll
        for (int off = LPP; off < 64; off <<= 1) {
#pragma unroll
            for (int k = 0; k < CPL; ++k) {
                s1[k] += __shfl_xor(s1[k], off, 64);
                s2[k] += __shfl_xor(s2[k], off, 64);
            }
            fn += __shfl_xor(fn, off, 64);
        }
        if (pg == 0) {
            if (pl == 0) {
#pragma unroll
                for (int k = 0; k < CPL; ++k) {
                    sh[wq][0][CPL * cl + k] = s1[k];
                    sh[wq][1][CPL * cl + k] = s2[k];
                }
            }
            if (cl == 0) shn[wid] = fn;
        }
        __syncthreads();
        if (wid == 0 && pg == 0) {
            float tn = 0.f;
#pragma unroll
            for (int k = 0; k < 4 * PW; ++k) tn += shn[k];
            const int nrec = tiles_x * ((h + 7) >> 3);
#pragma unroll
            for (int k = 0; k < CPL; ++k) {
                const int c = CPL * cl + k;
                const float t1 = ((sh[0][0][c] + sh[1][0][c]) + sh[2][0][c]) + sh[3][0][c];
                const float t2 = ((sh[0][1][c] + sh[1][1][c]) + sh[2][1][c]) + sh[3][1][c];
                const float mean = shift[k] + t1 / tn;
                const float m2 = t2 - t1 * t1 / tn;
                float* rec = stats + (((size_t)b * nrec + tile) * C + c) * 3;
                rec[0] = tn;
                rec[1] = mean;
                rec[2] = m2 > 0.f ? m2 : 0.f;
            }
        }
    }
}

extern "C" int lwg_lwb_attention_x_records(int h, int w, int C, int esz) {
    if (h <= 0 || w <= 0 || C <= 0 || (esz != 2 && esz != 4)) return 0;
    const int lpp = C / (16 / esz);
    if (lpp < 8 || lpp > 64 || (lpp & (lpp - 1)) != 0) return 0;
    return ((w + 7) >> 3) * ((h + 7) >> 3);
}

template <typename ST>
static int lwg_attnx_launch(const ST* x, const ST* Kq, const float* kappa, const ST* Vs, const float* bv, const float* T, ST* out, float* stats,
                            int B, int ns, int h, int w, int C, int src_batched, hipStream_t stream) {
    if (!x || !Kq || !kappa || !Vs || !bv || !T || !out || B <= 0 || ns <= 0 || ns > 64 || h <= 0 || w <= 0) return (int)hipErrorInvalidValue;
    const unsigned long long nsrc = (unsigned long long)(src_batched ? B * ns : ns);
    if (nsrc * (unsigned long long)h * w * (unsigned long long)C * sizeof(ST) >= 0xC0000000ull) return (int)hipErrorInvalidValue;
    const long tiles = (long)((w + 7) >> 3) * ((h + 7) >> 3);
    constexpr int CPL = AttnXTraits<ST>::CPL;
    const int npass = (C / CPL) / 4;
    const dim3 grid((unsigned)((LWG_ATTNX_INTERLEAVE ? (tiles + 7) / 8 * 8 : tiles) * B));
    const bool wide = LWG_ATTNX_WIDE && tiles * B < 512 && npass >= 4;
#define LWG_ATTNX_GO(LPP, ST_, NSU, PW)                                                                                              \
    {                                                                                                                                \
             \
        constexpr bool pipe = LWG_ATTNX_PIPE && CPL == 4 && (LPP) == 64 && (NSU) == 2 && (PW) == 1;                                  \
        auto kern = lwg_lwb_attnx_kernel<ST, LPP, ST_, NSU, PW, (pipe ? 2 : CPL == 4 ? LWG_ATTNX_OCC : LWG_ATTNX_OCC16), pipe>;        \
        const size_t lds = (size_t)((LPP) / 4) * 4096 + (size_t)ns * 512;                         \
        static unsigned long long lds_ok = 0;                                                                                        \
        if (lds > 65536) {                                                                                                           \
            const hipError_t e = lwg_allow_dynamic_lds(reinterpret_cast<const void*>(kern), lds, lds_ok);                            \
            if (e != hipSuccess) return (int)e;                                                                                      \
        }                                                                                                                            \
        hipLaunchKernelGGL(kern, grid, dim3(256 * PW), lds, stream, x, Kq, kappa, Vs, bv, T, out, stats, B, ns, h, w, src_batched);   \
    }
#define LWG_ATTNX_PW(LPP, ST_, NSU)                                                                                                  \
    {                                                                                                                                \
        if constexpr ((LPP) / 4 >= 4) {                                                                                              \
            if (wide) LWG_ATTNX_GO(LPP, ST_, NSU, 4) else LWG_ATTNX_GO(LPP, ST_, NSU, 1)                                             \
        } else {                                                                                                                     \
            LWG_ATTNX_GO(LPP, ST_, NSU, 1)                                                                                           \
        }                                                                                                                            \
    }
#define LWG_ATTNX_LAUNCH(LPP)                                                                                                        \
    if (stats) { if (LWG_ATTNX_NSU2 && ns == 2) LWG_ATTNX_PW(LPP, true, 2) else LWG_ATTNX_PW(LPP, true, 0) }                         \
    else { if (LWG_ATTNX_NSU2 && ns == 2) LWG_ATTNX_PW(LPP, false, 2) else LWG_ATTNX_PW(LPP, false, 0) }
    switch (C / CPL) {
        case 8: LWG_ATTNX_LAUNCH(8) break;
        case 16: LWG_ATTNX_LAUNCH(16) break;
        case 32: LWG_ATTNX_LAUNCH(32) break;
        case 64: if constexpr (CPL == 4) { LWG_ATTNX_LAUNCH(64) break; }
                 return (int)hipErrorInvalidValue;
        default: return (int)hipErrorInvalidValue;
    }
#undef LWG_ATTNX_LAUNCH
#undef LWG_ATTNX_PW
#undef LWG_ATTNX_GO
    return (int)hipGetLastError();
}

extern "C" int lwg_lwb_attention_x_f32(const float* x, const float* Kq, const float* kappa, const float* Vs, const float* bv, const float* T,
                                       float* out, float* stats, int B, int ns, int h, int w, int C, int src_batched, lwg_stream_t stream_) {
    if (C != 32 && C != 64 && C != 128 && C != 256) return (int)hipErrorInvalidValue;
    return lwg_attnx_launch<float>(x, Kq, kappa, Vs, bv, T, out, stats, B, ns, h, w, C, src_batched, reinterpret_cast<hipStream_t>(stream_));
}

extern "C" int lwg_lwb_attention_x_bf16(const void* x, const void* Kq, const float* kappa, const void* Vs, const float* bv, const float* T,
                                        void* out, float* stats, int B, int ns, int h, int w, int C, int src_batched, lwg_stream_t stream_) {
    if (C != 64 && C != 128 && C != 256) return (int)hipErrorInvalidValue;
    return lwg_attnx_launch<__bf16>(static_cast<const __bf16*>(x), static_cast<const __bf16*>(Kq), kappa, static_cast<const __bf16*>(Vs), bv, T,
                                    static_cast<__bf16*>(out), stats, B, ns, h, w, C, src_batched, reinterpret_cast<hipStream_t>(stream_));
}

__global__ __launch_bounds__(1024) void lwg_in_stats_merge_seg(const float* __restrict__ ws, int C, int nrec, int nseg, float eps,
                                                              float* __restrict__ part, float* __restrict__ mean, float* __restrict__ rstd) {
    const int lane = threadIdx.x & 63, wid = threadIdx.x >> 6;
    const int c = blockIdx.x * 64 + lane, b = blockIdx.y, seg = blockIdx.z;
    const bool cok = c < C;
    const float* base = ws + ((size_t)b * nrec * C + (cok ? c : 0)) * 3;
    const float r = base[1];
    const int per = (nrec + nseg - 1) / nseg;
    const int r0 = seg * per, r1 = min(nrec, r0 + per);
    float sa = 0.f, ss = 0.f, sq = 0.f;
    if (cok) {
        for (int i = r0 + wid; i < r1; i += 16) {
            const float* o = base + (size_t)i * C * 3;
            const float n = o[0], d = o[1] - r;
            sa += n;
            ss = __builtin_fmaf(n, d, ss);
            sq += __builtin_fmaf(n * d, d, o[2]);
        }
    }
    __shared__ float sh[16][3][64];
    sh[wid][0][lane] = sa;
    sh[wid][1][lane] = ss;
    sh[wid][2][lane] = sq;
    __syncthreads();
    if (wid == 0 && cok) {
        float ta = 0.f, ts = 0.f, tq = 0.f;
#pragma unroll
        for (int k = 0; k < 16; ++k) { ta += sh[k][0][lane]; ts += sh[k][1][lane]; tq += sh[k][2][lane]; }
        if (nseg == 1) {
            const float m2 = tq - ts * ts / ta;
            mean[(size_t)b * C + c] = r + ts / ta;
            rstd[(size_t)b * C + c] = 1.0f / sqrtf((m2 > 0.f ? m2 : 0.f) / ta + eps);
        } else {
            float* o = part + (((size_t)b * nseg + seg) * C + c) * 3;
            o[0] = ta; o[1] = ts; o[2] = tq;
        }
    }
}

__global__ __launch_bounds__(256) void lwg_in_stats_merge_fin(const float* __restrict__ ws, const float* __restrict__ part, int BC, int C, int nrec,
                                                             int nseg, float eps, float* __restrict__ mean, float* __restrict__ rstd) {
    const int i = blockIdx.x * 256 + threadIdx.x;
    if (i >= BC) return;
    const int b = i / C, c = i - b * C;
    const float r = ws[((size_t)b * nrec * C + c) * 3 + 1];
    float ta = 0.f, ts = 0.f, tq = 0.f;
    for (int s = 0; s < nseg; ++s) {
        const float* o = part + (((size_t)b * nseg + s) * C + c) * 3;
        ta += o[0]; ts += o[1]; tq += o[2];
    }
    const float m2 = tq - ts * ts / ta;
    mean[i] = r + ts / ta;
    rstd[i] = 1.0f / sqrtf((m2 > 0.f ? m2 : 0.f) / ta + eps);
}

extern "C" size_t lwg_instnorm_finalize_ws_floats(int B, int C, int nrec) {
    if (B <= 0 || C <= 0 || nrec <= 0) return 0;
    const size_t nseg = nrec > 512 ? (size_t)(nrec + 255) / 256 : 0;
    return (size_t)B * nrec * C * 3 + (size_t)B * nseg * C * 3;
}
extern "C" int lwg_instnorm_finalize_f32(float* ws, int B, int C, int nrec, float eps, float* mean, float* rstd, lwg_stream_t stream_) {
    if (!ws || !mean || !rstd || B <= 0 || C <= 0 || nrec <= 0 || B > 65535) return (int)hipErrorInvalidValue;
    hipStream_t stream = reinterpret_cast<hipStream_t>(stream_);
    const int nseg = nrec > 512 ? (nrec + 255) / 256 : 1;
    if (nseg > 65535) return (int)hipErrorInvalidValue;
    float* part = ws + (size_t)B * nrec * C * 3;
    hipLaunchKernelGGL(lwg_in_stats_merge_seg, dim3((C + 63) / 64, B, nseg), dim3(1024), 0, stream, ws, C, nrec, nseg, eps, part, mean, rstd);
    if (nseg > 1)
        hipLaunchKernelGGL(lwg_in_stats_merge_fin, dim3((B * C + 255) / 256), dim3(256), 0, stream, ws, part, B * C, C, nrec, nseg, eps, mean, rstd);
    return (int)hipGetLastError();
}
```

### ipercore_amd/csrc/lwg_conv_wino.h

```cpp
#pragma once
#include <stddef.h>
#include "lwg_conv_args.h"

#ifdef __HIPCC__
#define CW_FN __host__ __device__ __forceinline__
#else
#define CW_FN static inline
#endif
#ifdef __HIP_DEVICE_COMPILE__
#define CW_UNIFORM(v) __builtin_amdgcn_readfirstlane(v)
#else
#define CW_UNIFORM(v) (v)
#endif
#define CW_OOB 0xC0000000u
#define CW_KS 8
#define CW_NB 64
struct CwGrid { int bx, by, tiles, total; };
CW_FN CwGrid cw_grid(int B, int H, int W, int N, int ex, int ey, int nbv) {
    const int bx = (W + ex - 1) / ex, by = (H + ey - 1) / ey, tiles = bx * by * B;
    return CwGrid{bx, by, tiles, tiles * (N / nbv)};
}
CW_FN long long cw_total_blocks(int B, int H, int W, int N, int ex, int ey, int nbv) {
    return (long long)((W + ex - 1) / ex) * ((H + ey - 1) / ey) * B * (N / nbv);
}

enum { CW_COLMAJOR = 0, CW_CHUNK = 1, CW_XCD = 2 };
struct CwOrder { int kind, nwg, wg, ncb, tiles, total, xg, xr; };

CW_FN int cw4_order_kind(int xcd_sw, int chunk_sw, bool sm, unsigned nwg, int ncb, int Cin, int N, int tiles, int total) {
    const bool xcd = xcd_sw && !sm && (nwg & 7u) == 0 && (ncb == 4 || ncb == 8 || (ncb == 2 && (Cin >= 192 || xcd_sw == 2))) && (int)nwg < total && tiles >= (int)nwg / ncb;
    return xcd ? CW_XCD : chunk_sw == 2 || (chunk_sw == 1 && 144u * (unsigned)Cin * (unsigned)N <= (5u << 20)) ? CW_CHUNK : CW_COLMAJOR;
}
CW_FN CwOrder cw_order(int kind, unsigned nwg, unsigned wg, int ncb, const CwGrid& g) {
    return CwOrder{kind, (int)nwg, (int)wg, ncb, g.tiles, g.total, (int)nwg / ncb, (int)(((wg & 7u) / (unsigned)ncb) * (nwg >> 3) + (wg >> 3))};
}
CW_FN bool cw_has_block(const CwOrder& o, int id) {
    return o.kind == CW_XCD ? (id / o.nwg) * o.xg + o.xr < o.tiles : id < o.total;
}
CW_FN void cw_block(const CwOrder& o, int id, int& cb, int& t) {
    if (o.kind == CW_XCD) {
        cb = (int)((unsigned)o.wg & 7u) & (o.ncb - 1);
        t = CW_UNIFORM((id / o.nwg) * o.xg + o.xr);
    } else if (o.kind == CW_CHUNK) {
        const int G = o.nwg, per = G * o.ncb;
        const int ch = CW_UNIFORM(id / per);
        const int r = id - ch * per, base = ch * G;
        const int nt = o.tiles - base < G ? o.tiles - base : G;
        cb = CW_UNIFORM(r / nt);
        t = CW_UNIFORM(base + r - cb * nt);
    } else {
        cb = CW_UNIFORM(id / o.tiles);
        t = CW_UNIFORM(id - cb * o.tiles);
    }
}
CW_FN int cw_image(const CwGrid& g, int t) { return t / (g.bx * g.by); }
CW_FN void cw_corner(const CwGrid& g, int t_in_image, int ex, int ey, int& x0, int& y0) { x0 = (t_in_image % g.bx) * ex, y0 = (t_in_image / g.bx) * ey; }
CW_FN int cw_n0(int cb, int nbv) { return cb * nbv; }
CW_FN int cw4_n0_spade_small(int cb) { return (cb >> 1) * 64 + (cb & 1) * 16; }
CW_FN int cw_halo_pixel(int i, int hw, int nel, int lgp, int x0, int y0, int H, int W) {
    const int pix = i >> lgp, hy = pix / hw, hx = pix - hy * hw;
    const int gy = y0 - 1 + hy, gx = x0 - 1 + hx;
    return i < nel && gy >= 0 && gy < H && gx >= 0 && gx < W ? gy * W + gx : -1;
}
CW_FN unsigned cw_halo_pixel_voff(int lin, int i, int lgp, int C, int ebytes) {
    return lin >= 0 ? (unsigned)(lin * C + (16 / ebytes) * (i & ((1 << lgp) - 1))) * (unsigned)ebytes : CW_OOB;
}
CW_FN unsigned cw_halo_voff(int i, int hw, int nel, int lgp, int x0, int y0, int H, int W, int C, int ebytes) {
    return cw_halo_pixel_voff(cw_halo_pixel(i, hw, nel, lgp, x0, y0, H, W), i, lgp, C, ebytes);
}
CW_FN bool cw_stage_second(int c, int C0, bool two) { return two && c >= C0; }
CW_FN unsigned cw_stage_soff(int c, int C0, bool two, int ebytes) { return (unsigned)(cw_stage_second(c, C0, two) ? c - C0 : c) * (unsigned)ebytes; }
CW_FN unsigned cw4_out_voff(int ox, int oy, int H, int W, int YC, int chan) {
    return ox < W && oy < H ? (unsigned)((oy * W + ox) * YC + chan) * 4u : CW_OOB;
}
CW_FN unsigned cw4_out_group(unsigned vo, int h, bool grouped) { return vo + (grouped ? 128u * (unsigned)h : 0u); }

#define CW_NO_OUT_BUFFER (-1ll)
CW_FN bool cw_contract_ok(const LwgConvArgs& a, unsigned long long pair_bytes, long long out_slack) {
    if (!a.x0 || !a.w || !a.y || a.M <= 0 || a.ntaps != 9 || a.stride != 1 || a.omul != 1 || a.C0 <= 0 || (a.C0 % CW_KS) != 0 || a.C1 < 0 ||
        (a.C1 % CW_KS) != 0 || ((a.C0 + a.C1) % (2 * CW_KS)) != 0 || (a.C1 > 0 && !a.x1) || a.N <= 0 || (a.N % CW_NB) != 0 || a.OH != a.H ||
        a.OW != a.W || a.YH != a.H || a.YW != a.W || a.xdt != LWG_DT_F32 || a.ydt != LWG_DT_F32 || (long long)a.M != (long long)a.B * a.H * a.W ||
        a.ycoff < 0 || (a.ycoff % 4) != 0 || (a.YC % 4) != 0 || (a.act == LWG_ACTIVATION_RELU_MASK && a.epi != LWG_EPI_RESIDUAL))
        return false;
    if (a.epi == LWG_EPI_SPADE) {
        if (!a.xn || !a.mean || !a.rstd || !a.bias || a.YC * 2 != a.N || a.ycoff != 0) return false;
    } else {
        if (a.ycoff + a.N > a.YC) return false;
        if (a.epi != LWG_EPI_NONE && (a.epi != LWG_EPI_RESIDUAL || !a.res)) return false;
    }
    const unsigned long long cmax = (unsigned long long)(a.C0 > a.C1 ? a.C0 : a.C1);
    if ((unsigned long long)a.H * a.W * cmax * 4ull >= (unsigned long long)CW_OOB || pair_bytes * (a.C0 + a.C1) * a.N >= 0xffffffffull) return false;
    if (out_slack >= 0 && (unsigned long long)a.H * a.W * a.YC * 4ull + (unsigned long long)out_slack >= (unsigned long long)CW_OOB) return false;
    return true;
}
CW_FN bool cwb_contract_ok(const LwgConvArgs& a) {
    if (!a.x0 || !a.w || !a.y || a.B <= 0 || a.H <= 0 || a.W <= 0 || a.C0 <= 0 || a.C1 < 0 || a.N <= 0 || a.xdt != LWG_DT_BF16 || a.ydt != LWG_DT_BF16 ||
        a.ntaps != 9 || a.stride != 1 || a.omul != 1 || a.ooy != 0 || a.oox != 0 || a.OH != a.H || a.OW != a.W || a.YH != a.H || a.YW != a.W ||
        (long long)a.M != (long long)a.B * a.H * a.W)
        return false;
    for (int t = 0; t < 9; ++t)
        if (a.dy[t] != t / 3 - 1 || a.dx[t] != t % 3 - 1) return false;
    const int Cin = a.C0 + a.C1;
    if (a.N % 64 != 0 || Cin % 64 != 0 || (a.YC & 7) != 0 || (a.ycoff & 7) != 0 || a.ycoff < 0 || (a.C1 != 0 && (a.C0 % 64 != 0 || !a.x1))) return false;
    if (a.act != LWG_ACTIVATION_NONE && a.act != LWG_ACTIVATION_RELU && a.act != LWG_ACTIVATION_TANH && a.act != LWG_ACTIVATION_SIGMOID) return false;
    if ((unsigned long long)a.H * a.W * (unsigned long long)(a.C0 > a.C1 ? a.C0 : a.C1) * 2ull >= (unsigned long long)CW_OOB ||
        32ull * (unsigned long long)Cin * (unsigned long long)a.N >= (unsigned long long)CW_OOB || cw_total_blocks(a.B, a.H, a.W, a.N, 16, 16, 64) >= 0x7fffffffll)
        return false;
    if (a.epi == LWG_EPI_SPADE) return a.xn && a.mean && a.rstd && a.bias && a.YC * 2 == a.N && a.ycoff == 0;
    return a.ycoff + a.N <= a.YC && (a.epi == LWG_EPI_NONE || (a.epi == LWG_EPI_RESIDUAL && a.res));
}

struct LwgWinoTaps { int t[9]; };
CW_FN bool cw_panel_args_ok(const float* wpanel, const float* upk, int Cin, int N, const int* tap9, LwgWinoTaps& taps) {
    if (!wpanel || !upk || !tap9 || Cin <= 0 || (Cin % 32) != 0 || N <= 0) return false;
    for (int i = 0; i < 9; ++i) {
        if (tap9[i] < 0 || tap9[i] > 8) return false;
        taps.t[i] = tap9[i];
    }
    return true;
}

#ifdef __HIPCC__
#include "lwg_common.h"

template <int V> struct IntC { static constexpr int value = V; };
template <int POLICY = 0>
__device__ __forceinline__ floatx4 cw_buf_load(__amdgpu_buffer_rsrc_t r, unsigned voff, unsigned soff) {
    return __builtin_bit_cast(floatx4, __builtin_amdgcn_raw_buffer_load_b128(r, (int)voff, (int)soff, POLICY));
}
__device__ __forceinline__ __amdgpu_buffer_rsrc_t cw_image_rsrc(const void* x, int b, int H, int W, int C, unsigned ebytes) {
    const unsigned img = (unsigned)(H * W);
    return __builtin_amdgcn_make_buffer_rsrc(const_cast<char*>(static_cast<const char*>(x)) + (size_t)b * img * C * ebytes, 0, (int)(img * (unsigned)C * ebytes), 0x00020000);
}

template <int NQ, bool TWO>
struct CwBlock {
    int b, x0, y0, n0;
    __amdgpu_buffer_rsrc_t rx0, rx1;
    unsigned voff0[NQ], voff1[NQ];

    __device__ __forceinline__ void locate(const LwgConvArgs& a, const CwGrid& g, int t, int ex, int ey, int n) {
        b = __builtin_amdgcn_readfirstlane(cw_image(g, t));
        cw_corner(g, t - b * g.bx * g.by, ex, ey, x0, y0);
        n0 = n;
        rx0 = cw_image_rsrc(a.x0, b, a.H, a.W, a.C0, 4u);
        if constexpr (TWO) rx1 = cw_image_rsrc(a.x1, b, a.H, a.W, a.C1, 4u);
    }
    __device__ __forceinline__ void halo(const LwgConvArgs& a, int tid, int nth, int hw, int nel) {
#pragma unroll
        for (int k = 0; k < NQ; ++k) {
            voff0[k] = cw_halo_voff(tid + nth * k, hw, nel, 1, x0, y0, a.H, a.W, a.C0, 4);
            if constexpr (TWO) voff1[k] = cw_halo_voff(tid + nth * k, hw, nel, 1, x0, y0, a.H, a.W, a.C1, 4);
        }
    }
    template <int POLICY = 0>
    __device__ __forceinline__ floatx4 rld1(const LwgConvArgs& a, int c, int k) const {
        if constexpr (!TWO) {
            return cw_buf_load<POLICY>(rx0, voff0[k], cw_stage_soff(c, a.C0, false, 4));
        } else {
            const bool second = cw_stage_second(c, a.C0, true);
            const __amdgpu_buffer_rsrc_t r = second ? rx1 : rx0;
            const unsigned v = second ? voff1[k] : voff0[k];
            return cw_buf_load<POLICY>(r, v, cw_stage_soff(c, a.C0, true, 4));
        }
    }
};
__device__ __forceinline__ void cw_rst1(float* dst, int plane, floatx4 v) {
#pragma unroll
    for (int k = 0; k < 4; ++k) dst[k * plane] = v[k];
}

template <void (*KERNEL)(const LwgConvArgs)>
static inline int cw_launch(dim3 grid, unsigned threads, size_t lds, hipStream_t stream, const LwgConvArgs& a) {
    static unsigned long long done = 0ull;
    if (hipError_t e = lwg_allow_dynamic_lds(reinterpret_cast<const void*>(KERNEL), lds, done); e != hipSuccess) return (int)e;
    hipLaunchKernelGGL(KERNEL, grid, dim3(threads), lds, stream, a);
    return (int)hipGetLastError();
}
static inline dim3 cw_persistent_grid(long long total, int cus) { return dim3((unsigned)(LWG_WINO_PERSIST && total > cus ? cus : total)); }
#endif
```

### ipercore_amd/networks/generator.py

```python
import math

import torch
import torch.nn as nn

from .. import ops
from . import packing
from .params import generator_param_shapes


class _Node(nn.Module):

    def __init__(self):
        super().__init__()


class ParamTree(nn.Module):
    def __init__(self, shapes):
        super().__init__()
        self._shapes = dict(shapes)
        for name, shape in shapes.items():
            parts = name.split(".")
            node = self
            for p in parts[:-1]:
                if not hasattr(node, p):
                    node.add_module(p, _Node())
                node = getattr(node, p)
            node.register_parameter(parts[-1], nn.Parameter(torch.empty(*shape)))
        self.reset_parameters()

    @torch.no_grad()
    def reset_parameters(self):
        named = dict(self.named_parameters())
        for name, p in named.items():
            if name.endswith(".weight"):
                fan_in = p.shape[1] * p.shape[2] * p.shape[3]
                bound = 1.0 / math.sqrt(fan_in)
                p.uniform_(-bound, bound)
                b = named.get(name[:-len("weight")] + "bias")
                if b is not None:
                    b.uniform_(-bound, bound)


class _Packed:

    def __init__(self, gen):
        sd = {k: v for k, v in gen.named_parameters()}
        dev = next(gen.parameters()).device
        self.device = dev
        self.version = _param_version(gen)
        nf, n_res, n_down = gen.num_filters, gen.n_res_block, len(gen.num_filters)
        P = packing

        def conv(name, stride=1, pad=None, cin_pad=None, n_pad=None):
            return P.spec_to(P.pack_conv(sd[name + ".weight"], sd.get(name + ".bias"), stride, pad, cin_pad, n_pad), dev)

        def convT(name, n_pad=None):
            return [P.spec_to(s, dev) for s in P.pack_conv_transpose(sd[name + ".weight"], sd.get(name + ".bias"), n_pad)]

        def site(p):
            Wq = sd[p + ".fq.weight"].detach()[:, :, 0, 0].double()
            Wk = sd[p + ".fk.weight"].detach()[:, :, 0, 0].double()
            bq = sd[p + ".fq.bias"].detach().double()
            Wkq = (Wq.t() @ Wk).float()[:, :, None, None].contiguous()
            wkap = (Wk.t() @ bq).float()[None, :, None, None].contiguous()
            d = {
                "fkq": P.spec_to(P.pack_conv(Wkq, None, 1, 0), dev),
                "fkap": P.spec_to(P.pack_conv(wkap, None, 1, 0, None, 64), dev),
                "fv": P.spec_to(P.pack_conv(sd[p + ".fv.weight"], None, 1, 0), dev),
                "bv": sd[p + ".fv.bias"].detach().float().contiguous(),
                "shared": conv(p + ".spade.mlp_shared.0"),
                "gb": P.spec_to(P.pack_spade_gamma_beta(sd[p + ".spade.mlp_gamma.weight"], sd[p + ".spade.mlp_gamma.bias"],
                                                        sd[p + ".spade.mlp_beta.weight"], sd[p + ".spade.mlp_beta.bias"]), dev),
            }
            return d

        cin_pad = 8
        self.tsf_enc = [conv(f"tsf_net_enc.layers.{i}.0", stride=2, cin_pad=cin_pad if i == 0 else None) for i in range(n_down)]
        self.src_enc = [conv(f"src_net.encoders.layers.{i}.0", stride=2, cin_pad=cin_pad if i == 0 else None) for i in range(n_down)]
        self.src_res = [(conv(f"src_net.res_blocks.{i}.main.0"), conv(f"src_net.res_blocks.{i}.main.2")) for i in range(n_res)]
        self.src_dec = [convT(f"src_net.decoders.layers.{i}.0") for i in range(n_down)]
        self.src_head = P.pack_head(sd["src_net.img_reg.0.weight"], sd["src_net.att_reg.0.weight"]).to(dev)
        self.res = [(conv(f"res_blocks.{i}.main.0"), conv(f"res_blocks.{i}.main.2")) for i in range(n_res)]
        if gen.lwb_kind == "att":
            pass
        elif gen.lwb_kind in ("sg_add", "sg_avg"):
            site = lambda p: {"g0": conv(p + ".gate_conv.0"), "g2": conv(p + ".gate_conv.2")}
        else:
            site = lambda p: {}
        self.enc_sites = [site(f"enc_attlwbs.{i}") for i in range(n_down)]
        self.res_sites = [site(f"res_attlwbs.{i}") for i in range(n_res)]
        self.upconvs = [convT(f"tsf_net_dec.upconvs.{i}.0") for i in range(n_down)]
        self.skippers = [conv(f"tsf_net_dec.skippers.{i}.0") for i in range(n_down - 1)]
        self.head = P.pack_head(sd["tsf_img_reg.0.weight"], sd["tsf_att_reg.0.weight"]).to(dev)
        self.head16 = P.pack_head_bf16(sd["tsf_img_reg.0.weight"], sd["tsf_att_reg.0.weight"]).to(dev) if nf[0] == 64 else None
        self.bg = pack_bg_layers(sd, gen.bg_filters, n_res, dev) if gen.has_bg else None


def pack_bg_layers(sd, bgf, n_res, dev):
    P = packing

    def conv(name, stride=1, pad=None, cin_pad=None, n_pad=None):
        return P.spec_to(P.pack_conv(sd[name + ".weight"], sd.get(name + ".bias"), stride, pad, cin_pad, n_pad), dev)

    def convT(name, n_pad=None):
        return [P.spec_to(s, dev) for s in P.pack_conv_transpose(sd[name + ".weight"], sd.get(name + ".bias"), n_pad)]
    i = 0
    layers = [("conv", conv(f"bg_net.main.{i}", stride=1, pad=3, cin_pad=4))]
    i += 3
    for d in range(1, len(bgf)):
        layers.append(("conv", conv(f"bg_net.main.{i}", stride=2)))
        i += 3
    for _ in range(n_res):
        layers.append(("res", (conv(f"bg_net.main.{i}.main.0"), conv(f"bg_net.main.{i}.main.3"))))
        i += 1
    for d in range(len(bgf) - 1, 0, -1):
        layers.append(("convT", convT(f"bg_net.main.{i}")))
        i += 3
    layers.append(("out", conv(f"bg_net.main.{i}", stride=1, pad=3, n_pad=64)))
    return layers


def run_bg_layers(layers, bg4):
    scratch = _Scratch()
    x = bg4

    def norm(t, act, res=None):
        B, h, w, C = t.shape
        mean, rstd = t.new_empty(B, C), t.new_empty(B, C)
        nsplit = max(1, min(64, (h * w) // 64))
        ops.instnorm_stats(t, mean, rstd, scratch.get(B * C * nsplit * 3, t.device), eps=1e-5, nsplit=nsplit)
        return ops.instnorm_apply(t, mean, rstd, torch.empty_like(t), act=act, res=res)

    for kind, spec in layers:
        B, H, W, _ = x.shape
        if kind == "conv":
            y = ops.conv2d(x, spec, x.new_empty(B, H // spec.stride, W // spec.stride, spec.N))
            x = norm(y, ops.ACT_RELU)
        elif kind == "res":
            h = norm(ops.conv2d(x, spec[0], torch.empty_like(x)), ops.ACT_RELU)
            x = norm(ops.conv2d(h, spec[1], torch.empty_like(x)), ops.ACT_NONE, res=x)
        elif kind == "convT":
            y = x.new_empty(B, 2 * H, 2 * W, spec[0].N)
            x = norm(ops.conv_transpose2d(x, spec, y, act=ops.ACT_NONE), ops.ACT_RELU)
        else:
            y = ops.conv2d(x, spec, x.new_empty(B, H, W, spec.N), act=ops.ACT_TANH)
            return ops.nhwc_to_nchw(y, channels=3)


def _param_version(gen):
    return tuple((p.data_ptr(), p._version) for p in gen.parameters())


class SourceFeatures:

    def __init__(self, enc, res, kv, ns, batched=False):
        self.enc, self.res, self.kv, self.ns, self.batched = enc, res, kv, ns, batched


class AttentionLWBGenerator(nn.Module):
    has_bg = True
    lwb_kind = "att"

    def __init__(self, cfg, temporal=False):
        super().__init__()
        self._name = _get(cfg, "name", "AttLWB-SPADE")
        tsf = _get(cfg, "TSFNet")
        sid = _get(cfg, "SIDNet")
        self.num_filters = [int(c) for c in _get(tsf, "num_filters")]
        self.n_res_block = int(_get(tsf, "n_res_block"))
        if [int(c) for c in _get(sid, "num_filters")] != self.num_filters or int(_get(sid, "n_res_block")) != self.n_res_block:
            raise ValueError("SIDNet and TSFNet must share num_filters / n_res_block (the LWB sites pair them up)")
        for c in self.num_filters:
            if c not in (64, 128, 256):
                raise ValueError(f"num_filters entries must be in {{64,128,256}} for the HIP kernels, got {c}")
        self.cond_nc = int(_get(tsf, "cond_nc"))
        self.temporal = temporal
        self.bg_filters, bg_cond = None, 4
        if self.has_bg:
            bgc = _get(cfg, "BGNet")
            self.bg_filters = [int(c) for c in _get(bgc, "num_filters")]
            bg_cond = int(_get(bgc, "cond_nc"))
        shapes = generator_param_shapes(self.num_filters, self.n_res_block, self.bg_filters or (), cond_nc=self.cond_nc,
                                        bg_cond_nc=bg_cond, with_bg=self.has_bg,
                                        lwb={"att": "att", "add": "plain", "avg": "plain"}.get(self.lwb_kind, "softgate"))
        tree = ParamTree(shapes)
        for name, child in tree.named_children():
            self.add_module(name, child)
        self._packed = None
        self.conv_precision = "winograd"

    def packed(self):
        if self._packed is None or self._packed.version != _param_version(self):
            self._packed = _Packed(self)
        return self._packed

    def _check(self, *tensors):
        if torch.is_grad_enabled() and any(p.requires_grad for p in self.parameters()) and self.training:
            raise NotImplementedError("these methods are the no_grad inference engine: call under torch.no_grad() / .eval(), or train "
                                      "through ipercore_amd.networks.training.TrainableGenerator (trainers.LWGTrainer; all five LWB generators)")
        for t in tensors:
            if t is not None and not t.is_cuda:
                raise RuntimeError("ipercore_amd generator runs on the MI355X only: got a CPU tensor (no fallback)")

    @staticmethod
    def _check_square(t):
        if t.shape[-1] != t.shape[-2]:
            raise ValueError(f"square images only (got {t.shape[-2]} x {t.shape[-1]}): the reference's image_size is one number and the "
                             "attention blocks' flow fields are resized to square feature maps")

    @torch.no_grad()
    def _encode_sources_impl(self, src8, batched=False, ns=None):
        pk = self.packed()
        x = src8
        adt = self._act_dtype()
        enc, res = [], []
        for i, spec in enumerate(pk.src_enc):
            n, H, W, _ = x.shape
            y = x.new_empty(n, H // 2, W // 2, spec.N, dtype=adt)
            x = ops.conv2d(x, spec, y, act=ops.ACT_RELU)
            enc.append(x)
        for c0, c1 in pk.src_res:
            h = ops.conv2d(x, c0, torch.empty_like(x), act=ops.ACT_RELU)
            x = ops.conv2d(h, c1, torch.empty_like(x), epi=ops.EPI_RESIDUAL, res=x)
            res.append(x)
        return SourceFeatures(enc, res, self._project_sources(pk, enc, res), ns if ns is not None else src8.shape[0], batched)

    def _project_sources(self, pk, enc, res):
        kv = []
        for feats, sites in ((enc, pk.enc_sites), (res, pk.res_sites)):
            for f, st in zip(feats, sites):
                if self.lwb_kind == "att":
                    n, h, w, _ = f.shape
                    with ops.conv_precision("fp32" if self.conv_precision in ("bf16", "bf16_winograd") else self.conv_precision):
                        kap = ops.conv2d(f.float(), st["fkap"], f.new_empty(n, h, w, 64, dtype=torch.float32))[..., 0].contiguous()
                    kv.append((ops.conv2d(f, st["fkq"], torch.empty_like(f)), ops.conv2d(f, st["fv"], torch.empty_like(f)), kap))
                else:
                    kv.append((f, None, None))
        return kv

    def _attlwb(self, st, tsf_x, kv, Tst, batched, scratch):
        B, h, w, C = tsf_x.shape
        if self.lwb_kind != "att":
            ns = Tst.shape[1]
            Tst = scratch.flow(Tst, h, w)
            if self.lwb_kind == "add":
                return ops.lwb_fuse(tsf_x, kv[0], Tst, torch.empty_like(tsf_x), src_batched=batched)
            if self.lwb_kind == "avg":
                return ops.lwb_fuse(tsf_x, kv[0], Tst, torch.empty_like(tsf_x), scale_o=1.0 / (ns + 1), src_batched=batched)
            g = ops.conv2d(tsf_x, st["g0"], torch.empty_like(tsf_x), act=ops.ACT_RELU)
            g = ops.conv2d(g, st["g2"], torch.empty_like(tsf_x), act=ops.ACT_SIGMOID)
            return ops.lwb_fuse(tsf_x, kv[0], Tst, torch.empty_like(tsf_x), gate=g,
                                scale_w=1.0 if self.lwb_kind == "sg_add" else 1.0 / ns, src_batched=batched)
        mean = tsf_x.new_empty(B, C, dtype=torch.float32)
        rstd = tsf_x.new_empty(B, C, dtype=torch.float32)
        nrec = ops.attn_records(h, w, C, tsf_x.dtype)
        ws = scratch.get(ops.instnorm_finalize_ws(B, C, nrec), tsf_x.device)
        flow = scratch.flow(Tst, h, w)
        if tuple(flow.shape[2:4]) != (h, w):
            raise NotImplementedError("the attention block takes flows resized to its feature size: non-square feature maps are not built "
                                      "(image_size is one number throughout the reference)")
        att = ops.lwb_attention_x(tsf_x, kv[0], kv[2], kv[1], st["bv"], flow, torch.empty_like(tsf_x), stats=ws,
                                  src_batched=batched)
        ops.instnorm_finalize(ws, B, C, nrec, mean, rstd, eps=1e-5)
        actv = ops.conv2d(att, st["shared"], tsf_x.new_empty(B, h, w, st["shared"].N), act=ops.ACT_RELU)
        return ops.conv2d(actv, st["gb"], torch.empty_like(tsf_x), epi=ops.EPI_SPADE, xn=tsf_x, mean=mean, rstd=rstd)

    @staticmethod
    def _upconv(x, specs, act, q4=False):
        B, H, W, _ = x.shape
        if q4:
            return ops.conv_transpose2d(x, specs, x.new_empty(B, specs[0].N // 4, 2 * H, 2 * W, 4), act=act, q4=True)
        y = x.new_empty(B, 2 * H, 2 * W, specs[0].N)
        return ops.conv_transpose2d(x, specs, y, act=act)

    @torch.no_grad()
    def _run_tsf_impl(self, tsf8, feats, Tst, bg=None, want_pred=True, want_mask=True, want_img=False):
        pk = self.packed()
        scratch = _Scratch()
        n_down = len(pk.tsf_enc)
        x = tsf8
        adt = self._act_dtype()
        if feats.kv[0][0].dtype != adt:
            raise RuntimeError(f"source features are {feats.kv[0][0].dtype} but the generator runs in {self.conv_precision} mode: "
                               "rebuild them (Imitator.set_source / forward_src) after changing conv_precision")
        enc = []
        site = 0
        for i, spec in enumerate(pk.tsf_enc):
            B, H, W, _ = x.shape
            x = ops.conv2d(x, spec, x.new_empty(B, H // 2, W // 2, spec.N, dtype=adt), act=ops.ACT_RELU)
            x = self._attlwb(pk.enc_sites[i], x, feats.kv[site], Tst, feats.batched, scratch)
            site += 1
            enc.append(x)
        for i, (c0, c1) in enumerate(pk.res):
            h = ops.conv2d(x, c0, torch.empty_like(x), act=ops.ACT_RELU)
            x = ops.conv2d(h, c1, torch.empty_like(x), epi=ops.EPI_RESIDUAL, res=x)
            x = self._attlwb(pk.res_sites[i], x, feats.kv[site], Tst, feats.batched, scratch)
            site += 1
        q4 = adt == torch.float32 and self.conv_precision in ("fp32", "winograd", "winograd2x2")
        for i in range(n_down):
            if i == n_down - 1 and pk.head16 is not None and ops.up4_head_eligible(x, pk.upconvs[i], ops.ACT_RELU):
                return ops.up4_head_compose_bf16(x, pk.upconvs[i], pk.head16, bg, want_pred=want_pred and bg is not None, want_mask=want_mask,
                                                 want_img=want_img)
            x = self._upconv(x, pk.upconvs[i], ops.ACT_RELU, q4=q4 and i == n_down - 1)
            if i != n_down - 1:
                skip = enc[n_down - 2 - i]
                sp = pk.skippers[i]
                x = ops.conv2d(skip, sp, x.new_empty(x.shape[0], x.shape[1], x.shape[2], sp.N), x1=x, act=ops.ACT_RELU)
        head = pk.head
        if x.dtype == torch.bfloat16:
            if pk.head16 is not None:
                head = pk.head16
            else:
                x = x.float()
        return ops.head_compose(x, head, bg, want_pred=want_pred and bg is not None, want_mask=want_mask, want_img=want_img, q4=q4)

    def _act_dtype(self):
        return torch.bfloat16 if self.conv_precision in ("bf16", "bf16_winograd") else torch.float32

    @torch.no_grad()
    def _run_bg_impl(self, bg4):
        return run_bg_layers(self.packed().bg, bg4)

    @torch.no_grad()
    def _run_src_decode_impl(self, x):
        pk = self.packed()
        for specs in pk.src_dec:
            x = self._upconv(x, specs, ops.ACT_RELU)
        _, mask, img = ops.head_compose(x.float(), pk.src_head, None, want_pred=False, want_mask=True, want_img=True)
        return img, mask

    def encode_sources(self, *a, **k):
        with ops.conv_precision(self.conv_precision):
            return self._encode_sources_impl(*a, **k)

    def run_tsf(self, *a, **k):
        with ops.conv_precision(self.conv_precision):
            return self._run_tsf_impl(*a, **k)

    def run_bg(self, *a, **k):
        with ops.conv_precision("fp32" if self.conv_precision in ("bf16", "bf16_winograd") else self.conv_precision):
            return self._run_bg_impl(*a, **k)

    def run_src_decode(self, *a, **k):
        with ops.conv_precision(self.conv_precision):
            return self._run_src_decode_impl(*a, **k)

    @torch.no_grad()
    def forward_bg(self, bg_inputs):
        if not self.has_bg:
            raise AttributeError("this generator has no background network")
        self._check(bg_inputs)
        bs, ns, c, h, w = bg_inputs.shape
        x = ops.nchw_to_nhwc(bg_inputs.reshape(bs * ns, c, h, w).contiguous().float(), c_pad=4)
        return self.run_bg(x).view(bs, ns, 3, h, w)

    @torch.no_grad()
    def forward_src(self, src_inputs, only_enc=True):
        self._check(src_inputs)
        self._check_square(src_inputs)
        bs, ns, c, h, w = src_inputs.shape
        src8 = ops.nchw_to_nhwc(src_inputs.reshape(bs * ns, c, h, w).contiguous().float(), c_pad=8)
        feats = self.encode_sources(src8, batched=bs > 1, ns=ns)
        enc = _FeatList(ops.nhwc_to_nchw(t.float()) for t in feats.enc)
        res = _FeatList(ops.nhwc_to_nchw(t.float()) for t in feats.res)
        enc.lwg_cache = res.lwg_cache = feats
        if only_enc:
            return enc, res
        img, mask = self.run_src_decode(feats.res[-1])
        return enc, res, img.view(bs, ns, 3, h, w), mask.view(bs, ns, 1, h, w)

    def _features_from_api(self, src_enc_outs, src_res_outs, bs):
        cache = getattr(src_enc_outs, "lwg_cache", None)
        if cache is not None and getattr(src_res_outs, "lwg_cache", None) is cache:
            return cache
        pk = self.packed()
        adt = self._act_dtype()
        enc = [ops.nchw_to_nhwc(t.contiguous().float()).to(adt) for t in src_enc_outs]
        res = [ops.nchw_to_nhwc(t.contiguous().float()).to(adt) for t in src_res_outs]
        n = enc[0].shape[0]
        return SourceFeatures(enc, res, self._project_sources(pk, enc, res), n // bs, batched=bs > 1)

    @torch.no_grad()
    def forward_tsf(self, tsf_inputs, src_enc_outs, src_res_outs, Tst, temp_enc_outs=None, temp_res_outs=None, Ttt=None):
        self._check(tsf_inputs, Tst)
        self._check_square(tsf_inputs)
        bs = tsf_inputs.shape[0]
        feats = self._features_from_api(src_enc_outs, src_res_outs, bs)
        T = Tst.contiguous().float()
        if temp_enc_outs is not None and Ttt is not None and self.lwb_kind == "att":
            if bs != 1:
                raise NotImplementedError("temporal attention runs one clip per process (bs = 1), as Imitator.inference does")
            tfe = self._features_from_api(temp_enc_outs, temp_res_outs, bs)
            feats = SourceFeatures(feats.enc, feats.res, [tuple(torch.cat([a, ta], dim=0) for a, ta in zip(site, tsite))
                                                          for site, tsite in zip(feats.kv, tfe.kv)],
                                   feats.ns + Ttt.shape[1], batched=False)
            T = torch.cat([T, Ttt.contiguous().float()], dim=1).contiguous()
        tsf8 = ops.nchw_to_nhwc(tsf_inputs.contiguous().float(), c_pad=8)
        _, mask, img = self.run_tsf(tsf8, feats, T, bg=None, want_pred=False, want_mask=True, want_img=True)
        return img, mask

    @torch.no_grad()
    def _forward_streams(self, src_inputs, tsf_inputs, Tst, only_tsf):
        bs, nt = Tst.shape[0], Tst.shape[1]
        if only_tsf:
            enc, res = self.forward_src(src_inputs, only_enc=True)
            src_imgs = src_masks = None
        else:
            enc, res, src_imgs, src_masks = self.forward_src(src_inputs, only_enc=False)
        imgs, masks = [], []
        for t in range(nt):
            if t != 0 and self.temporal:
                raise NotImplementedError("multi-step temporal training forward (Ttt inside forward()) is not built; "
                                          "temporal INFERENCE goes through Imitator(temporal=True) / forward_tsf(temp_*)")
            img, mask = self.forward_tsf(tsf_inputs[:, t], enc, res, Tst[:, t].contiguous())
            imgs.append(img)
            masks.append(mask)
        return src_imgs, src_masks, torch.stack(imgs, dim=1), torch.stack(masks, dim=1)

    @torch.no_grad()
    def forward(self, bg_inputs, src_inputs, tsf_inputs, Tst, Ttt=None, only_tsf=True):
        bg_img = self.forward_bg(bg_inputs)
        src_imgs, src_masks, imgs, masks = self._forward_streams(src_inputs, tsf_inputs, Tst, only_tsf)
        if only_tsf:
            return bg_img, imgs, masks
        return bg_img, src_imgs, src_masks, imgs, masks


class AttentionLWBFrontGenerator(AttentionLWBGenerator):
    has_bg = False

    @torch.no_grad()
    def forward(self, src_inputs, tsf_inputs, Tst, Ttt=None, only_tsf=True):
        src_imgs, src_masks, imgs, masks = self._forward_streams(src_inputs, tsf_inputs, Tst, only_tsf)
        if only_tsf:
            return imgs, masks
        return src_imgs, src_masks, imgs, masks


class AddLWBGenerator(AttentionLWBGenerator):
    lwb_kind = "add"


class AvgLWBGenerator(AttentionLWBGenerator):
    lwb_kind = "avg"


class SoftGateAddLWBGenerator(AttentionLWBGenerator):
    lwb_kind = "sg_add"


class SoftGateAvgLWBGenerator(AttentionLWBGenerator):
    lwb_kind = "sg_avg"


class _FeatList(list):
    """A list that can carry the engine's cache as an attribute (plain lists cannot)."""


class _Scratch:
    def __init__(self):
        self.buf = None
        self.flows = {}

    def flow(self, Tst, h, w):
        if Tst.shape[2] == h and Tst.shape[3] == w:
            return Tst
        if h != w:
            return Tst
        key = (h, w, Tst.data_ptr())
        if key not in self.flows:
            self.flows[key] = ops.flow_resize(Tst, h, w)
        return self.flows[key]

    def get(self, n, device):
        if self.buf is None or self.buf.numel() < n or self.buf.device != device:
            self.buf = torch.empty(max(n, 1 << 16), device=device, dtype=torch.float32)
        return self.buf


def _get(cfg, key, default=None):
    if isinstance(cfg, dict):
        if key in cfg:
            return cfg[key]
    elif hasattr(cfg, key):
        return getattr(cfg, key)
    if default is not None:
        return default
    raise KeyError(key)


class _ConcatPacked:

    def __init__(self, gen):
        sd = {k: v for k, v in gen.named_parameters()}
        dev = next(gen.parameters()).device
        self.version = _param_version(gen)
        P = packing
        nf, n_down = gen.num_filters, len(gen.num_filters)

        def conv(name, stride=1, pad=None, cin_pad=None):
            return P.spec_to(P.pack_conv(sd[name + ".weight"], sd.get(name + ".bias"), stride, pad, cin_pad, None), dev)
        self.enc = [conv(f"tsf_net.encoders.layers.{i}.0", stride=2, cin_pad=gen.cin_pad if i == 0 else None) for i in range(n_down)]
        self.res = [(conv(f"tsf_net.res_blocks.{i}.main.0"), conv(f"tsf_net.res_blocks.{i}.main.2")) for i in range(gen.n_res_block)]
        self.dec = [[P.spec_to(sp, dev) for sp in P.pack_conv_transpose(sd[f"tsf_net.decoders.layers.{i}.0.weight"],
                                                                       sd[f"tsf_net.decoders.layers.{i}.0.bias"], None)] for i in range(n_down)]
        self.head = P.pack_head(sd["tsf_net.img_reg.0.weight"], sd["tsf_net.att_reg.0.weight"]).to(dev)
        self.bg = pack_bg_layers(sd, gen.bg_filters, gen.bg_n_res_block, dev)


class InputConcatGenerator(nn.Module):
    has_bg = True

    def __init__(self, cfg, temporal=False):
        super().__init__()
        self._name = _get(cfg, "name", "InputConcat")
        tsf, bgc = _get(cfg, "TSFNet"), _get(cfg, "BGNet")
        self.num_filters = [int(c) for c in _get(tsf, "num_filters")]
        self.n_res_block = int(_get(tsf, "n_res_block"))
        self.cond_nc = int(_get(tsf, "cond_nc"))
        self.num_source = int(_get(tsf, "num_source", 4)) if self._uses_sources() else None
        self.bg_filters = [int(c) for c in _get(bgc, "num_filters")]
        self.bg_n_res_block = int(_get(bgc, "n_res_block"))
        self.temporal = temporal
        if self.num_filters[0] != 64 or any(c not in (64, 128, 256) for c in self.num_filters):
            raise ValueError(f"num_filters must start with 64 and stay in {{64,128,256}} for the HIP kernels, got {self.num_filters}")
        self.cin_pad = 8 if self.cond_nc <= 8 else (16 if self.cond_nc <= 16 else (self.cond_nc + 31) // 32 * 32)
        from .params import concat_generator_param_shapes
        tree = ParamTree(concat_generator_param_shapes(self.num_filters, self.n_res_block, self.bg_filters, self.cond_nc,
                                                        int(_get(bgc, "cond_nc", 4)), self.bg_n_res_block))
        for name, child in tree.named_children():
            self.add_module(name, child)
        self._packed = None

    def _uses_sources(self):
        return True

    def packed(self):
        if self._packed is None or self._packed.version != _param_version(self):
            self._packed = _ConcatPacked(self)
        return self._packed

    @staticmethod
    def _check(*tensors):
        for t in tensors:
            if t is not None and not t.is_cuda:
                raise RuntimeError("ipercore_amd generator runs on the MI355X only: got a CPU tensor (no fallback)")

    @torch.no_grad()
    def forward_bg(self, bg_inputs):
        self._check(bg_inputs)
        bs, ns, c, h, w = bg_inputs.shape
        x = ops.nchw_to_nhwc(bg_inputs.reshape(bs * ns, c, h, w).contiguous().float(), c_pad=4)
        return run_bg_layers(self.packed().bg, x).view(bs, ns, 3, h, w)

    def forward_src(self, src_inputs, only_enc=True):
        bs, ns, _, h, w = src_inputs.shape
        need = self.num_source
        if ns > need:
            src_inputs = src_inputs[:, 0:need]
        elif ns < need:
            src_inputs = torch.cat([src_inputs, torch.stack([src_inputs[:, s % ns] for s in range(need - ns)], dim=1)], dim=1)
        enc = src_inputs.reshape(bs, -1, h, w)
        return (enc, enc) if only_enc else (enc, enc, None, None)

    @torch.no_grad()
    def _autoencode(self, inputs):
        self._check(inputs)
        pk = self.packed()
        x = ops.nchw_to_nhwc(inputs.contiguous().float(), c_pad=self.cin_pad)
        for spec in pk.enc:
            n, H, W, _ = x.shape
            x = ops.conv2d(x, spec, x.new_empty(n, H // 2, W // 2, spec.N), act=ops.ACT_RELU)
        for c0, c1 in pk.res:
            t = ops.conv2d(x, c0, torch.empty_like(x), act=ops.ACT_RELU)
            x = ops.conv2d(t, c1, torch.empty_like(x), epi=ops.EPI_RESIDUAL, res=x)
        for specs in pk.dec:
            n, H, W, _ = x.shape
            x = ops.conv_transpose2d(x, specs, x.new_empty(n, 2 * H, 2 * W, specs[0].N), act=ops.ACT_RELU)
        _, mask, img = ops.head_compose(x, pk.head, None, want_pred=False, want_mask=True, want_img=True)
        return img, mask

    @torch.no_grad()
    def forward_tsf(self, tsf_inputs, src_enc_outs, src_res_outs=None, Tst=None, temp_enc_outs=None, temp_res_outs=None, Ttt=None):
        return self._autoencode(torch.cat([src_enc_outs, tsf_inputs[:, -3:]], dim=1))

    @torch.no_grad()
    def forward(self, bg_inputs, src_inputs, tsf_inputs, Tst=None, Ttt=None, only_tsf=True):
        bg_img = self.forward_bg(bg_inputs)
        enc, _ = self.forward_src(src_inputs, only_enc=True)
        outs = [self.forward_tsf(tsf_inputs[:, t], enc) for t in range(tsf_inputs.shape[1])]
        return bg_img, torch.stack([o[0] for o in outs], dim=1), torch.stack([o[1] for o in outs], dim=1)


class TextureWarpingGenerator(InputConcatGenerator):

    def __init__(self, cfg, temporal=False):
        super().__init__(cfg, temporal)
        self._name = _get(cfg, "name", "TextureWarping")

    def _uses_sources(self):
        return False

    def forward_src(self, src_inputs, only_enc=True):
        bs, ns, _, h, w = src_inputs.shape
        enc = src_inputs.reshape(bs, -1, h, w)
        return (enc, enc) if only_enc else (enc, enc, None, None)

    @torch.no_grad()
    def forward_tsf(self, tsf_inputs, src_enc_outs=None, src_res_outs=None, Tst=None, temp_enc_outs=None, temp_res_outs=None, Ttt=None):
        return self._autoencode(tsf_inputs)

    @torch.no_grad()
    def forward(self, bg_inputs, src_inputs, tsf_inputs, Tst=None, Ttt=None, only_tsf=True):
        bg_img = self.forward_bg(bg_inputs)
        bs, nt, c, h, w = tsf_inputs.shape
        img, mask = self._autoencode(tsf_inputs.reshape(bs * nt, c, h, w))
        return bg_img, img.view(bs, nt, 3, h, w), mask.view(bs, nt, 1, h, w)
```

### ipercore_amd/ops.py

```python
import ctypes

import torch

from . import _lib
from ._lib import ACT_LRELU, ACT_NONE, ACT_RELU, ACT_RELU_MASK, ACT_SIGMOID, ACT_TANH, EPI_NONE, EPI_RESIDUAL, EPI_SPADE

EYE_DIST = 2.7320508075688776


def _ptr(t, dtype=torch.float32):
    if t is None:
        return None
    if not t.is_cuda:
        raise RuntimeError("ipercore_amd ops need CUDA (HIP) tensors: the MI355X path has no CPU fallback")
    if t.dtype != dtype:
        raise TypeError(f"expected {dtype}, got {t.dtype}")
    if not t.is_contiguous():
        raise ValueError("tensor must be contiguous")
    return t.data_ptr()


CONV_PRECISION = "fp32"


class conv_precision(object):

    def __init__(self, mode):
        assert mode in ("fp32", "bf16", "bf16_winograd", "split", "winograd", "winograd2x2")
        self.mode = mode

    def __enter__(self):
        global CONV_PRECISION, WINO4
        self.prev = CONV_PRECISION, WINO4
        if self.mode == "winograd2x2":
            CONV_PRECISION, WINO4 = "winograd", False
        else:
            CONV_PRECISION = self.mode

    def __exit__(self, *exc):
        global CONV_PRECISION, WINO4
        CONV_PRECISION, WINO4 = self.prev


CONV_HOOK = None


def _stream():
    return torch.cuda.current_stream().cuda_stream


class ConvSpec:
    __slots__ = ("w", "bias", "N", "Cin", "ntaps", "dy", "dx", "stride", "cshift", "omul", "ooy", "oox", "algo_kn", "_w16v2", "_w16hr", "_w16x3", "_w16c8", "_w16up", "_w32up", "_wwino", "_wwino_t", "_wwino_t24", "_wwino4", "_wwino16")

    def __init__(self, w, bias, N, Cin, taps, stride=1, omul=1, ooy=0, oox=0, algo_kn=None):
        self.w, self.bias, self.N, self.Cin = w, bias, int(N), int(Cin)
        self.algo_kn = int(algo_kn) if algo_kn is not None else len(taps) * int(Cin) * int(N)
        self.ntaps = len(taps)
        self.dy = [int(t[0]) for t in taps]
        self.dx = [int(t[1]) for t in taps]
        self.stride, self.omul, self.ooy, self.oox = stride, omul, ooy, oox
        self._w16v2 = None
        self._w16hr = None
        self._w16x3 = None
        self._w16c8 = None
        self._w16up = None
        self._w32up = None
        self._wwino = None
        self._wwino_t = None
        self._wwino_t24 = None
        self._wwino4 = None
        self._wwino16 = None
        self.cshift = 0
        if self.Cin % 32 != 0:
            q = self.Cin // 4
            assert q in (1, 2, 4), "small-Cin path handles Cin in {4, 8, 16}"
            self.cshift = q.bit_length() - 1


def _w16v2(spec):
    if spec._w16v2 is None or spec._w16v2.device != spec.w.device:
        K4, N, _ = spec.w.shape
        cin, nt = spec.Cin, spec.ntaps
        assert cin % 64 == 0 and K4 * 4 == nt * cin, (cin, nt, K4)
        wk = spec.w.permute(0, 2, 1).reshape(cin // 64, 2, nt, 32, N)
        wk = wk.permute(0, 2, 1, 3, 4).reshape(cin // 64 * nt, 64, N)
        rows = wk.permute(0, 2, 1).reshape(cin // 64 * nt, N, 8, 8)
        n = torch.arange(N, device=spec.w.device)
        slot = torch.arange(8, device=spec.w.device)
        src = slot[None, :] ^ ((n[:, None] >> 1) & 7)
        rows = torch.gather(rows, 2, src[None, :, :, None].expand(rows.shape[0], N, 8, 8))
        spec._w16v2 = rows.reshape(cin // 64 * nt, N, 64).contiguous().to(torch.bfloat16)
    return spec._w16v2


def _hr_eligible(spec, x0, y, out_hw):
    if not BF16_HR or spec.stride != 1 or spec.ntaps not in (9, 4) or spec.N % 64 != 0 or spec.Cin % 64 != 0:
        return False
    if any(abs(d) > 1 for d in spec.dy) or any(abs(d) > 1 for d in spec.dx):
        return False
    OH, OW = ((y.shape[1], y.shape[2]) if spec.omul == 1 else (y.shape[1] // spec.omul, y.shape[2] // spec.omul)) if out_hw is None else out_hw
    return (OH, OW) == (x0.shape[1], x0.shape[2])


def _hr_tap_order(spec):
    return sorted(range(spec.ntaps), key=lambda t: (spec.dy[t], spec.dx[t]))


def _w16hr(spec, spade):
    key = bool(spade)
    if spec._w16hr is None or spec._w16hr[0] != key or spec._w16hr[1].device != spec.w.device:
        K4, N, _ = spec.w.shape
        cin, nt = spec.Cin, spec.ntaps
        wk = spec.w.permute(0, 2, 1).reshape(cin // 64, 2, nt, 32, N).permute(0, 2, 1, 3, 4).reshape(cin // 64, nt, 64, N)
        wk = wk[:, _hr_tap_order(spec)].reshape(cin // 64 * nt, 64, N)
        bias = spec.bias
        if spade:
            j = torch.arange(N, device=spec.w.device)
            q, r = j // 32, j % 32
            ch = 16 * q + (r % 16)
            old = 64 * (ch // 32) + (ch % 32) + 32 * (r // 16)
            wk = wk[:, :, old]
            bias = None if bias is None else bias[old].contiguous()
        panel = wk.reshape(cin // 64 * nt, 4, 16, N).permute(0, 1, 3, 2).contiguous().to(torch.bfloat16)
        spec._w16hr = (key, panel, bias)
    return spec._w16hr[1], spec._w16hr[2]


BF16_WINO_MIN_CIN = 64
_WINO_G = ((1.0, 0.0, 0.0), (0.5, 0.5, 0.5), (0.5, -0.5, 0.5), (0.0, 0.0, 1.0))


def _bf16_wino_eligible(spec, x0, y, x1, epi, act, out_hw, ycoff=0):
    if spec.ntaps != 9 or spec.stride != 1 or spec.omul != 1 or spec.N % 64 != 0 or spec.Cin % 64 != 0 or spec.Cin < BF16_WINO_MIN_CIN:
        return False
    if (y.shape[1], y.shape[2]) != (x0.shape[1], x0.shape[2]) or (out_hw is not None and tuple(out_hw) != (x0.shape[1], x0.shape[2])):
        return False
    if sorted(zip(spec.dy, spec.dx)) != _WINO_TAPS or epi not in (EPI_NONE, EPI_RESIDUAL, EPI_SPADE):
        return False
    if act not in (ACT_NONE, ACT_RELU, ACT_TANH, ACT_SIGMOID) or y.dtype != torch.bfloat16:
        return False
    if x1 is not None and (x1.dtype != torch.bfloat16 or x0.shape[3] % 64 != 0):
        return False
    if epi == EPI_SPADE:
        return y.shape[3] * 2 == spec.N and ycoff == 0
    return y.shape[3] % 8 == 0 and ycoff % 8 == 0 and ycoff + spec.N <= y.shape[3]


def wwino16_index(ks, p, n, e, N):
    return ((ks * 16 + p) * N + n) * 16 + e


def wwino16_spade_column(j):
    return 4 * (j // 8) + j % 4, (j % 8) // 4


def _wwino16(spec, spade):
    key = bool(spade)
    if spec._wwino16 is None or spec._wwino16[0] != key or spec._wwino16[1].device != spec.w.device:
        K4, N, _ = spec.w.shape
        cin, nt = spec.Cin, spec.ntaps
        assert nt == 9 and cin % 64 == 0 and N % 64 == 0 and K4 * 4 == nt * cin, (cin, nt, K4, N)
        dev = spec.w.device
        wk = spec.w.permute(0, 2, 1).reshape(cin // 32, nt, 32, N).permute(1, 0, 2, 3).reshape(nt, cin, N)
        order = [0] * 9
        for t in range(nt):
            order[3 * (spec.dy[t] + 1) + spec.dx[t] + 1] = t
        w33 = wk[order].reshape(3, 3, cin, N).to(torch.float64)
        G = torch.tensor(_WINO_G, dtype=torch.float64, device=dev)
        U = torch.einsum("ar,rscn,bs->abcn", G, w33, G)
        bias = spec.bias
        if spade:
            j = torch.arange(N, device=dev)
            ch, beta = 4 * (j // 8) + j % 4, (j % 8) // 4
            old = 64 * (ch // 32) + (ch % 32) + 32 * beta
            U = U[:, :, :, old]
            bias = None if bias is None else bias[old].contiguous()
        panel = U.reshape(16, cin // 16, 16, N).permute(1, 0, 3, 2).contiguous().to(torch.bfloat16)
        spec._wwino16 = (key, panel, bias)
    return spec._wwino16[1], spec._wwino16[2]


BF16_HR = True
BF16_PW = True
BF16_C8 = True


def _pw_eligible(spec, x0, y, x1, epi, out_hw):
    if not BF16_PW or spec.ntaps != 1 or spec.stride != 1 or spec.omul != 1 or x1 is not None or epi != EPI_NONE:
        return False
    if spec.dy[0] != 0 or spec.dx[0] != 0 or spec.N != spec.Cin or spec.N not in (64, 128, 256):
        return False
    OH, OW = (y.shape[1], y.shape[2]) if out_hw is None else out_hw
    return (OH, OW) == (x0.shape[1], x0.shape[2])


def _w16c8(spec):
    if spec._w16c8 is None or spec._w16c8.device != spec.w.device:
        K4, N, _ = spec.w.shape
        nks = (spec.ntaps + 1) // 2
        wk = spec.w.permute(0, 2, 1).reshape(K4 * 4, N)
        if wk.shape[0] < nks * 16:
            wk = torch.cat([wk, wk.new_zeros(nks * 16 - wk.shape[0], N)], dim=0)
        spec._w16c8 = wk[:nks * 16].reshape(nks, 16, N).permute(0, 2, 1).contiguous().to(torch.bfloat16)
    return spec._w16c8


def _w16x3(spec):
    if spec._w16x3 is None or spec._w16x3.device != spec.w.device:
        K4, N, _ = spec.w.shape
        wk = spec.w.permute(0, 2, 1).reshape(K4 * 4, N)
        hi = wk.to(torch.bfloat16)
        r1 = wk - hi.float()
        mid = r1.to(torch.bfloat16)
        lo = (r1 - mid.float()).to(torch.bfloat16)
        spec._w16x3 = torch.stack([hi, mid, lo]).view(3, K4 // 2, 8, N).permute(0, 1, 3, 2).contiguous()
    return spec._w16x3


_WINO_TAPS = sorted((dy, dx) for dy in (-1, 0, 1) for dx in (-1, 0, 1))


def _wino_eligible(spec, x0, y, x1, epi, act, out_hw, q4, ycoff=0):
    if q4 or x0.dtype != torch.float32 or y.dtype != torch.float32 or epi not in (EPI_NONE, EPI_RESIDUAL, EPI_SPADE) or \
            (act == ACT_RELU_MASK and epi != EPI_RESIDUAL):
        return False
    if x1 is not None and (x1.dtype != torch.float32 or x0.shape[3] % 8 != 0 or x1.shape[3] % 8 != 0):
        return False
    if spec.ntaps != 9 or spec.stride != 1 or spec.omul != 1 or spec.Cin % 32 != 0 or spec.N % 64 != 0:
        return False
    if epi == EPI_SPADE and (y.shape[3] * 2 != spec.N or ycoff != 0):
        return False
    if sorted(zip(spec.dy, spec.dx)) != _WINO_TAPS:
        return False
    hw = (y.shape[1], y.shape[2]) if out_hw is None else tuple(out_hw)
    return hw == (x0.shape[1], x0.shape[2]) == (y.shape[1], y.shape[2])


WINO_MIN_GRID = 128
WINO_SPLITK = True


def _wino_plan(a, spec, y, splitk):
    if not splitk:
        return 0
    blocks, slices, nbv = ctypes.c_longlong(0), ctypes.c_int(0), ctypes.c_int(0)
    if _lib.lib().lwg_conv2d_winograd_plan(a, 1 if WINO_SPLITK else 0, ctypes.byref(blocks), ctypes.byref(slices), ctypes.byref(nbv), None) != 0:
        return None
    units32 = blocks.value * (nbv.value // 32)
    return slices.value * a.M * spec.N if units32 >= WINO_MIN_GRID else None


def _wwino(spec):
    if spec._wwino is None or spec._wwino.device != spec.w.device:
        K4, N, _ = spec.w.shape
        cin, nt = spec.Cin, spec.ntaps
        assert nt == 9 and cin % 32 == 0 and K4 * 4 == nt * cin, (cin, nt, K4)
        if not spec.w.is_cuda:
            raise RuntimeError("ipercore_amd ops need CUDA (HIP) tensors: the MI355X path has no CPU fallback")
        tap9 = (ctypes.c_int * 9)()
        for t in range(nt):
            tap9[3 * (spec.dy[t] + 1) + spec.dx[t] + 1] = t
        if PANEL_CACHE is not None:
            U = PANEL_CACHE.winograd(spec, list(tap9))
            if U is not None:
                spec._wwino = U
                return U
        U = torch.empty(16, cin // 8, 2, N, 4, device=spec.w.device, dtype=torch.float32)
        _lib.check(_lib.lib().lwg_winograd_panel_f32(_ptr(spec.w), _ptr(U), cin, N, tap9, _stream()), "lwg_winograd_panel_f32")
        spec._wwino = U
    return spec._wwino


WINO4 = True
WINO4_MIN_CIN = 64


def _wino4_use(spec, splitk):
    return WINO4 and not splitk and spec.Cin >= WINO4_MIN_CIN


def _wwino4(spec):
    if spec._wwino4 is None or spec._wwino4.device != spec.w.device:
        K4, N, _ = spec.w.shape
        cin, nt = spec.Cin, spec.ntaps
        assert nt == 9 and cin % 32 == 0 and K4 * 4 == nt * cin, (cin, nt, K4)
        if not spec.w.is_cuda:
            raise RuntimeError("ipercore_amd ops need CUDA (HIP) tensors: the MI355X path has no CPU fallback")
        tap9 = (ctypes.c_int * 9)()
        for t in range(nt):
            tap9[3 * (spec.dy[t] + 1) + spec.dx[t] + 1] = t
        U = torch.empty(4, cin // 8, 4, 2, 9 * N, device=spec.w.device, dtype=torch.float32)
        _lib.check(_lib.lib().lwg_winograd4_panel_f32(_ptr(spec.w), _ptr(U), cin, N, tap9, _stream()), "lwg_winograd4_panel_f32")
        spec._wwino4 = U
    return spec._wwino4


def conv_args(x0, spec, y, x1=None, epi=EPI_NONE, act=ACT_NONE, res=None, xn=None, mean=None, rstd=None,
              out_hw=None, ycoff=0, q4=False):
    B, H, W, C0 = x0.shape
    C1 = 0 if x1 is None else x1.shape[3]
    assert C0 + C1 == spec.Cin, (C0, C1, spec.Cin)
    if q4:
        YB, YCq, YH, YW, four = y.shape
        assert four == 4 and y.dtype == torch.float32 and x0.dtype == torch.float32 and epi == EPI_NONE and y.is_contiguous()
        YC = 4 * YCq
    else:
        YB, YH, YW, YC = y.shape
    if out_hw is None:
        OH, OW = (YH, YW) if spec.omul == 1 else (YH // spec.omul, YW // spec.omul)
    else:
        OH, OW = out_hw
    a = _lib.LwgConvArgs()
    xdt, ydt = x0.dtype, y.dtype
    a.xdt = _lib.DT_BF16 if xdt == torch.bfloat16 else _lib.DT_F32
    a.ydt = _lib.DT_F32_Q4 if q4 else (_lib.DT_BF16 if ydt == torch.bfloat16 else _lib.DT_F32)
    a.x0, a.x1 = _ptr(x0, xdt), _ptr(x1, xdt)
    a.C0, a.C1 = C0, C1
    a.B, a.H, a.W = B, H, W
    a.OH, a.OW, a.M = OH, OW, B * OH * OW
    a.stride, a.ntaps, a.cshift = spec.stride, spec.ntaps, spec.cshift
    a.w, a.N, a.bias = _ptr(spec.w), spec.N, _ptr(spec.bias)
    a.y, a.YH, a.YW, a.YC, a.ycoff = _ptr(y, ydt), YH, YW, YC, ycoff
    a.omul, a.ooy, a.oox = spec.omul, spec.ooy, spec.oox
    a.epi, a.act = epi, act
    a.res, a.xn, a.mean, a.rstd = _ptr(res, ydt), _ptr(xn, ydt), _ptr(mean), _ptr(rstd)
    for i in range(spec.ntaps):
        a.dy[i] = spec.dy[i]
        a.dx[i] = spec.dx[i]
    return a


def _hook_end(a, spec, epi, kind, slices=True, extra=0):
    n = (max(1, int(_lib.lib().lwg_conv_slice_count(a))) if slices else 1) + extra
    CONV_HOOK(False, a.M, spec, epi, {"kernels": n, "kind": kind})


def conv2d(x0, spec, y, x1=None, epi=EPI_NONE, act=ACT_NONE, res=None, xn=None, mean=None, rstd=None,
           out_hw=None, ycoff=0, splitk=False, q4=False):
    a = conv_args(x0, spec, y, x1, epi, act, res, xn, mean, rstd, out_hw, ycoff, q4)
    if q4 and (splitk or CONV_PRECISION not in ("fp32", "winograd") or x0.dtype != torch.float32):
        raise ValueError("channel-quad-plane outputs: fp32 activations on the fp32 MFMA path, no split-K")
    if CONV_HOOK is not None:
        CONV_HOOK(True, a.M, spec, epi, None)
    kind, sliced, extra = "direct", True, 0
    if x0.dtype == torch.bfloat16:
        kind = "bf16"
        if y.dtype != torch.bfloat16 or spec.Cin % 64 != 0:
            raise ValueError("bf16 convolutions need bf16 outputs and Cin % 64 == 0")
        if CONV_PRECISION == "bf16_winograd" and _bf16_wino_eligible(spec, x0, y, x1, epi, act, out_hw, ycoff):
            kind, sliced = "bf16_winograd", False
            panel, bias = _wwino16(spec, epi == EPI_SPADE)
            a.w, a.bias = _ptr(panel, torch.bfloat16), _ptr(bias)
            for i, (dy, dx) in enumerate(_WINO_TAPS):
                a.dy[i], a.dx[i] = dy, dx
            _lib.check(_lib.lib().lwg_conv2d_winograd_bf16(a, _stream()), "lwg_conv2d_winograd_bf16")
        elif _hr_eligible(spec, x0, y, out_hw) or _pw_eligible(spec, x0, y, x1, epi, out_hw):
            panel, bias = _w16hr(spec, epi == EPI_SPADE)
            a.w, a.bias = _ptr(panel, torch.bfloat16), _ptr(bias)
            for i, t in enumerate(_hr_tap_order(spec)):
                a.dy[i], a.dx[i] = spec.dy[t], spec.dx[t]
            _lib.check(_lib.lib().lwg_conv2d_nhwc_bf16_hr(a, _stream()), "lwg_conv2d_nhwc_bf16_hr")
        else:
            a.w = _ptr(_w16v2(spec), torch.bfloat16)
            _lib.check(_lib.lib().lwg_conv2d_nhwc_bf16(a, _stream()), "lwg_conv2d_nhwc_bf16")
    elif y.dtype == torch.bfloat16:
        if BF16_C8 and spec.Cin == 8 and spec.N == 64 and spec.ntaps <= 10 and x1 is None and epi == EPI_NONE and spec.omul == 1:
            a.w = _ptr(_w16c8(spec), torch.bfloat16)
            _lib.check(_lib.lib().lwg_conv2d_nhwc_c8_bf16(a, _stream()), "lwg_conv2d_nhwc_c8_bf16")
        else:
            _lib.check(_lib.lib().lwg_conv2d_nhwc_f32(a, _stream()), "lwg_conv2d_nhwc_f32")
    elif CONV_PRECISION == "winograd" and _wino_eligible(spec, x0, y, x1, epi, act, out_hw, q4, ycoff) and \
            (nws := _wino_plan(a, spec, y, splitk)) is not None:
        kind, sliced = "winograd", False
        if _wino4_use(spec, splitk):
            a.w = _ptr(_wwino4(spec))
            kind = "winograd4"
            _lib.check(_lib.lib().lwg_conv2d_winograd4_f32(a, _stream()), "lwg_conv2d_winograd4_f32")
        elif nws:
            a.w = _ptr(_wwino(spec))
            ws, extra = torch.empty(nws, device=x0.device, dtype=torch.float32), 1
            _lib.check(_lib.lib().lwg_conv2d_winograd_f32_ws(a, _ptr(ws), _stream()), "lwg_conv2d_winograd_f32_ws")
        else:
            a.w = _ptr(_wwino(spec))
            _lib.check(_lib.lib().lwg_conv2d_winograd_f32(a, _stream()), "lwg_conv2d_winograd_f32")
    elif CONV_PRECISION == "split" and spec.Cin % 32 == 0:
        a.w = _ptr(_w16x3(spec), torch.bfloat16)
        kind = "split"
        _lib.check(_lib.lib().lwg_conv2d_nhwc_f32_split(a, _stream()), "lwg_conv2d_nhwc_f32_split")
    else:
        nws = _lib.lib().lwg_conv2d_ws_floats(a) if splitk else 0
        if nws:
            ws = torch.empty(nws, device=x0.device, dtype=torch.float32)
            _lib.check(_lib.lib().lwg_conv2d_nhwc_f32_ws(a, _ptr(ws), _stream()), "lwg_conv2d_nhwc_f32_ws")
        else:
            _lib.check(_lib.lib().lwg_conv2d_nhwc_f32(a, _stream()), "lwg_conv2d_nhwc_f32")
    if CONV_HOOK is not None:
        _hook_end(a, spec, epi, kind, sliced, extra)
    return y


WINO_UP4 = True
F32_UP4 = True
BF16_UP4 = True


def _parity_specs_ok(specs):
    s0 = specs[0]
    return (len(specs) == 4 and all(s.ntaps == 4 and s.omul == 2 and s.stride == 1 and (s.ooy, s.oox) == (i >> 1, i & 1) and s.N == s0.N and s.Cin == s0.Cin
                                    and [(dy - (i >> 1), dx - (i & 1)) for dy, dx in zip(s.dy, s.dx)] == list(zip(s0.dy, s0.dx)) for i, s in enumerate(specs)))


def _wwino_t(specs):
    s0 = specs[0]
    U = s0._wwino_t
    if U is not None and U.device == s0.w.device:
        return U
    Cin, N = s0.Cin, s0.N
    G = torch.tensor([[1.0, 0.0], [1.0, 1.0], [0.0, 1.0]], dtype=torch.float64, device=s0.w.device)
    parts = []
    for par, sp in enumerate(specs):
        py, px = par >> 1, par & 1
        W = sp.w.double().permute(0, 2, 1).reshape(4 * Cin, N)
        W = W.view(Cin // 32, 4, 32, N).permute(1, 0, 2, 3).reshape(4, Cin, N)
        g = torch.zeros(2, 2, Cin, N, dtype=torch.float64, device=W.device)
        for t, (dy, dx) in enumerate(zip(sp.dy, sp.dx)):
            g[dy - (py - 1), dx - (px - 1)] = W[t]
        u = torch.einsum("ar,rqcn,bq->abcn", G, g, G)
        if py:
            u[0] = -u[0]
        if px:
            u[:, 0] = -u[:, 0]
        parts.append(u.reshape(9, Cin, N))
    U9 = torch.stack(parts).float()
    U = torch.cat([U9[:, 0:4].permute(0, 2, 3, 1).reshape(4, Cin, 4 * N), U9[:, 4:8].permute(0, 2, 3, 1).reshape(4, Cin, 4 * N), U9[:, 8]], dim=2)
    U = U.view(4, Cin // 8, 4, 2, 9 * N).contiguous()
    s0._wwino_t = U
    return U


_G_X24 = ((1.0, 0.0), (0.5, 0.5), (-1.0 / 6.0, 1.0 / 6.0), (-8.0 / 3.0, -4.0 / 3.0), (0.0, 0.5))


def _wwino_t24(specs):
    s0 = specs[0]
    U = s0._wwino_t24
    if U is not None and U.device == s0.w.device:
        return U
    Cin, N = s0.Cin, s0.N
    Gy = torch.tensor([[1.0, 0.0], [1.0, 1.0], [0.0, 1.0]], dtype=torch.float64, device=s0.w.device)
    Gx = torch.tensor(_G_X24, dtype=torch.float64, device=s0.w.device)
    parts = []
    for par, sp in enumerate(specs):
        py, px = par >> 1, par & 1
        W = sp.w.double().permute(0, 2, 1).reshape(4 * Cin, N)
        W = W.view(Cin // 32, 4, 32, N).permute(1, 0, 2, 3).reshape(4, Cin, N)
        g = torch.zeros(2, 2, Cin, N, dtype=torch.float64, device=W.device)
        for t, (dy, dx) in enumerate(zip(sp.dy, sp.dx)):
            g[dy - (py - 1), dx - (px - 1)] = W[t]
        u = torch.einsum("ar,rqcn,bq->abcn", Gy, g, Gx)
        if py:
            u[0] = -u[0]
        parts.append(torch.cat([u[:, :3].reshape(9, Cin, N), u[:, 3:].reshape(6, Cin, N)]))
    U15 = torch.stack(parts).float()
    quad = lambda lo, hi: U15[:, lo:hi].permute(0, 2, 3, 1).reshape(4, Cin, (hi - lo) * N)
    U = torch.cat([quad(0, 4), quad(4, 8), U15[:, 8], quad(9, 13), U15[:, 13], U15[:, 14]], dim=2)
    U = U.view(4, Cin // 8, 4, 2, 15 * N).contiguous()
    s0._wwino_t24 = U
    return U


WINO_UP4_24 = True
WINO_UP4_24_MIN_HW = 64 * 64


def _up4_24(x):
    return WINO_UP4_24 and x.shape[1] * x.shape[2] >= WINO_UP4_24_MIN_HW


class _FusedTransposeSpec(object):

    def __init__(self, s0, panel):
        self.N, self.Cin, self.ntaps, self.stride, self.omul = 4 * s0.N, s0.Cin, 16, 1, 2
        self.algo_kn, self.w = 4 * s0.algo_kn, panel


def conv_transpose2d(x, specs, y, act=ACT_NONE, splitk=False, out_hw=None, q4=False):
    s0 = specs[0]
    if (BF16_UP4 and BF16_HR and x.dtype == torch.bfloat16 and y.dtype == torch.bfloat16 and len(specs) == 4 and s0.Cin in (64, 128)
            and s0.N % 64 == 0 and all(s.ntaps == 4 and s.omul == 2 and (s.ooy, s.oox) == (i >> 1, i & 1) for i, s in enumerate(specs))):
        a = conv_args(x, s0, y, act=act)
        panel = getattr(s0, "_w16up", None)
        if panel is None or panel.device != s0.w.device:
            panel = torch.stack([_w16hr(s, False)[0] for s in specs]).contiguous()
            s0._w16up = panel
        a.w = _ptr(panel, torch.bfloat16)
        if CONV_HOOK is not None:
            whole = _FusedTransposeSpec(s0, panel)
            CONV_HOOK(True, a.M, whole, EPI_NONE, None)
        _lib.check(_lib.lib().lwg_conv_transpose4_nhwc_bf16(a, _stream()), "lwg_conv_transpose4_nhwc_bf16")
        if CONV_HOOK is not None:
            _hook_end(a, whole, EPI_NONE, "up4")
        return y
    if (WINO_UP4 and CONV_PRECISION == "winograd" and not splitk and out_hw is None and x.is_cuda and x.dtype == torch.float32 and y.dtype == torch.float32
            and s0.Cin % 32 == 0 and s0.N % 32 == 0 and _parity_specs_ok(specs)):
        a = conv_args(x, s0, y, act=act, q4=q4)
        f24 = _up4_24(x)
        panel = _wwino_t24(specs) if f24 else _wwino_t(specs)
        a.w = _ptr(panel)
        if CONV_HOOK is not None:
            whole = _FusedTransposeSpec(s0, panel)
            CONV_HOOK(True, a.M, whole, EPI_NONE, None)
        if f24:
            _lib.check(_lib.lib().lwg_conv_transpose4_winograd24_f32(a, _stream()), "lwg_conv_transpose4_winograd24_f32")
        else:
            _lib.check(_lib.lib().lwg_conv_transpose4_winograd_f32(a, _stream()), "lwg_conv_transpose4_winograd_f32")
        if CONV_HOOK is not None:
            _hook_end(a, whole, EPI_NONE, "winograd_up4", False)
        return y
    if (F32_UP4 and x.is_cuda and x.dtype == torch.float32 and y.dtype == torch.float32 and CONV_PRECISION in ("fp32", "winograd") and s0.Cin % 32 == 0
            and _parity_specs_ok(specs)):
        a = conv_args(x, s0, y, act=act, q4=q4)
        if _lib.lib().lwg_conv_transpose4_is_one_grid(a):
            panel = getattr(s0, "_w32up", None)
            if panel is None or panel.device != s0.w.device:
                panel = torch.stack([s.w.reshape(-1) for s in specs]).contiguous()
                s0._w32up = panel
            a.w = _ptr(panel)
            if CONV_HOOK is not None:
                whole = _FusedTransposeSpec(s0, panel)
                CONV_HOOK(True, a.M, whole, EPI_NONE, None)
            _lib.check(_lib.lib().lwg_conv_transpose4_nhwc_f32(a, _stream()), "lwg_conv_transpose4_nhwc_f32")
            if CONV_HOOK is not None:
                _hook_end(a, whole, EPI_NONE, "up4")
            return y
    for s in specs:
        conv2d(x, s, y, act=act, splitk=splitk, out_hw=None if out_hw is None else out_hw(s), q4=q4)
    return y


def instnorm_stats(x, mean, rstd, ws, eps=1e-5, nsplit=None):
    B, H, W, C = x.shape
    HW = H * W
    if nsplit is None:
        nsplit = max(1, min(64, HW // 64))
    assert ws.numel() >= B * C * nsplit * 3
    if x.dtype == torch.bfloat16:
        _lib.check(_lib.lib().lwg_instnorm_stats_nhwc_bf16(_ptr(x, torch.bfloat16), B, HW, C, eps, _ptr(mean), _ptr(rstd), _ptr(ws), nsplit,
                                                            _stream()), "lwg_instnorm_stats_nhwc_bf16")
        return
    _lib.check(_lib.lib().lwg_instnorm_stats_nhwc_f32(_ptr(x), B, HW, C, eps, _ptr(mean), _ptr(rstd), _ptr(ws), nsplit,
                                                       _stream()), "lwg_instnorm_stats_nhwc_f32")


def instnorm_apply(x, mean, rstd, y, act=ACT_NONE, res=None):
    B, H, W, C = x.shape
    _lib.check(_lib.lib().lwg_instnorm_apply_nhwc_f32(_ptr(x), _ptr(mean), _ptr(rstd), _ptr(res), _ptr(y), B, H * W, C, act,
                                                       _stream()), "lwg_instnorm_apply_nhwc_f32")
    return y


def flow_resize(T, h, w):
    B, ns, S = T.shape[0], T.shape[1], T.shape[2]
    T = T.contiguous()
    out = torch.empty(B, ns, h, w, 2, device=T.device, dtype=torch.float32)
    _lib.check(_lib.lib().lwg_flow_resize_f32(_ptr(T), B * ns, S, h, w, _ptr(out), _stream()), "lwg_flow_resize_f32")
    return out


def lwb_attention(q, Ks, Vs, bk, bv, T, out, src_batched=False):
    B, h, w, C = q.shape
    ns = T.shape[1]
    S = T.shape[2]
    assert T.shape[0] == B and Ks.shape[0] == (B * ns if src_batched else ns) and tuple(Ks.shape[1:]) == (h, w, C)
    if q.dtype == torch.bfloat16:
        bf = torch.bfloat16
        _lib.check(_lib.lib().lwg_lwb_attention_bf16(_ptr(q, bf), _ptr(Ks, bf), _ptr(Vs, bf), _ptr(bk), _ptr(bv), _ptr(T), _ptr(out, bf), B, ns, h,
                                                      w, C, S, 1 if src_batched else 0, _stream()), "lwg_lwb_attention_bf16")
        return out
    _lib.check(_lib.lib().lwg_lwb_attention_f32(_ptr(q), _ptr(Ks), _ptr(Vs), _ptr(bk), _ptr(bv), _ptr(T), _ptr(out), B, ns, h,
                                                 w, C, S, 1 if src_batched else 0, _stream()), "lwg_lwb_attention_f32")
    return out


def attn_records(h, w, C, dtype=torch.float32):
    n = _lib.lib().lwg_lwb_attention_x_records(int(h), int(w), int(C), 2 if dtype == torch.bfloat16 else 4)
    if n <= 0:
        raise ValueError(f"lwb_attention_x: unsupported (h, w, C, dtype) = {(h, w, C, dtype)}")
    return n


def lwb_attention_x(x, Kq, kappa, Vs, bv, T, out, stats=None, src_batched=False):
    B, h, w, C = x.shape
    ns = T.shape[1]
    nsrc = B * ns if src_batched else ns
    assert tuple(T.shape) == (B, ns, h, w, 2), (tuple(T.shape), (B, ns, h, w, 2))
    assert tuple(Kq.shape) == (nsrc, h, w, C) and tuple(Vs.shape) == (nsrc, h, w, C) and tuple(kappa.shape) == (nsrc, h, w)
    assert Kq.dtype == x.dtype and Vs.dtype == x.dtype and out.dtype == x.dtype and kappa.dtype == torch.float32
    assert stats is None or stats.numel() >= B * attn_records(h, w, C, x.dtype) * C * 3
    if x.dtype == torch.bfloat16:
        bf = torch.bfloat16
        _lib.check(_lib.lib().lwg_lwb_attention_x_bf16(_ptr(x, bf), _ptr(Kq, bf), _ptr(kappa), _ptr(Vs, bf), _ptr(bv), _ptr(T), _ptr(out, bf),
                                                        _ptr(stats), B, ns, h, w, C, 1 if src_batched else 0, _stream()), "lwg_lwb_attention_x_bf16")
        return out
    _lib.check(_lib.lib().lwg_lwb_attention_x_f32(_ptr(x), _ptr(Kq), _ptr(kappa), _ptr(Vs), _ptr(bv), _ptr(T), _ptr(out), _ptr(stats), B, ns, h, w,
                                                   C, 1 if src_batched else 0, _stream()), "lwg_lwb_attention_x_f32")
    return out


def instnorm_finalize_ws(B, C, nrec):
    return int(_lib.lib().lwg_instnorm_finalize_ws_floats(int(B), int(C), int(nrec)))


def instnorm_finalize(ws, B, C, nrec, mean, rstd, eps=1e-5):
    assert ws.numel() >= instnorm_finalize_ws(B, C, nrec)
    _lib.check(_lib.lib().lwg_instnorm_finalize_f32(_ptr(ws), B, C, nrec, float(eps), _ptr(mean), _ptr(rstd), _stream()), "lwg_instnorm_finalize_f32")


def lwb_fuse(tsf_x, src_x, T, out, gate=None, scale_w=1.0, scale_o=1.0, src_batched=False):
    B, h, w, C = tsf_x.shape
    ns, S = T.shape[1], T.shape[2]
    assert T.shape[0] == B and src_x.shape[0] == (B * ns if src_batched else ns) and tuple(src_x.shape[1:]) == (h, w, C)
    assert src_x.dtype == tsf_x.dtype and out.dtype == tsf_x.dtype and (gate is None or gate.dtype == tsf_x.dtype)
    assert T.dtype == torch.float32
    if tsf_x.dtype == torch.bfloat16:
        bf = torch.bfloat16
        _lib.check(_lib.lib().lwg_lwb_fuse_bf16(_ptr(tsf_x, bf), _ptr(src_x, bf), _ptr(gate, bf), _ptr(T), _ptr(out, bf), B, ns, h, w, C, S,
                                                1 if src_batched else 0, float(scale_w), float(scale_o), _stream()), "lwg_lwb_fuse_bf16")
        return out
    _lib.check(_lib.lib().lwg_lwb_fuse_f32(_ptr(tsf_x), _ptr(src_x), _ptr(gate), _ptr(T), _ptr(out), B, ns, h, w, C, S,
                                           1 if src_batched else 0, float(scale_w), float(scale_o), _stream()), "lwg_lwb_fuse_f32")
    return out


def lwb_fuse_bwd(src_x, gate, T, dout, src_batched=False, scale_w=1.0, scale_o=1.0):
    B, h, w, C = dout.shape
    ns, S = T.shape[1], T.shape[2]
    assert T.shape[0] == B and src_x.shape[0] == (B * ns if src_batched else ns) and tuple(src_x.shape[1:]) == (h, w, C)
    assert gate is None or gate.shape == dout.shape
    dout = dout.contiguous()
    d_tsf = torch.empty_like(dout)
    d_src = torch.zeros_like(src_x)
    d_gate = None if gate is None else torch.empty_like(dout)
    _lib.check(_lib.lib().lwg_lwb_fuse_bwd_f32(_ptr(src_x), _ptr(gate), _ptr(T), _ptr(dout), _ptr(d_tsf), _ptr(d_src), _ptr(d_gate), B, ns, h, w, C,
                                               S, 1 if src_batched else 0, float(scale_w), float(scale_o), _stream()), "lwg_lwb_fuse_bwd_f32")
    return d_tsf, d_src, d_gate


def lwb_attention_bwd(q, Ks, Vs, bk, bv, T, dout, src_batched=False):
    B, h, w, C = q.shape
    ns, S = T.shape[1], T.shape[2]
    dout = dout.contiguous()
    dq = torch.empty_like(q)
    dKs = torch.zeros_like(Ks)
    dVs = torch.zeros_like(Vs)
    _lib.check(_lib.lib().lwg_lwb_attention_bwd_f32(_ptr(q), _ptr(Ks), _ptr(Vs), _ptr(bk), _ptr(bv), _ptr(T), _ptr(dout), _ptr(dq),
                                                     _ptr(dKs), _ptr(dVs), B, ns, h, w, C, S, 1 if src_batched else 0, _stream()),
               "lwg_lwb_attention_bwd_f32")
    return dq, dKs, dVs


def lwb_attention_kv(q, kv, bk, bv, T, out, src_batched=False):
    B, h, w, C = q.shape
    ns, S = T.shape[1], T.shape[2]
    assert T.shape[0] == B and kv.shape[0] == (B * ns if src_batched else ns) and tuple(kv.shape[1:]) == (h, w, 2 * C)
    _lib.check(_lib.lib().lwg_lwb_attention_kv_f32(_ptr(q), _ptr(kv), _ptr(bk), _ptr(bv), _ptr(T), _ptr(out), B, ns, h, w, C, S,
                                                    1 if src_batched else 0, _stream()), "lwg_lwb_attention_kv_f32")
    return out


def lwb_attention_kv_bwd(q, kv, bk, bv, T, dout, src_batched=False):
    B, h, w, C = q.shape
    ns, S = T.shape[1], T.shape[2]
    dout = dout.contiguous()
    dq = torch.empty_like(q)
    dkv = torch.zeros_like(kv)
    _lib.check(_lib.lib().lwg_lwb_attention_kv_bwd_f32(_ptr(q), _ptr(kv), _ptr(bk), _ptr(bv), _ptr(T), _ptr(dout), _ptr(dq), _ptr(dkv),
                                                        B, ns, h, w, C, S, 1 if src_batched else 0, _stream()), "lwg_lwb_attention_kv_bwd_f32")
    return dq, dkv


# ... 617 lines not shown
```

Baseline: 1216 frames/s.

## Skip Winograd conv tiles whose SPADE flow taps fall entirely outside the source

Adds a mark/scan pass over the warp flow that sorts output tiles into heavy ones (some bilinear tap lands in the image, dilated by the conv receptive field) and light ones (every tap lands outside). A new list variant of the F(4x4,3x3) Winograd kernel computes only the heavy tiles. For light tiles it copies a per-resolution calibration map, precomputed once from an all-out-of-image attention pass, and applies the SPADE modulation epilogue to it. This removes the shared and gamma/beta conv work in background regions. The risks are the extra mark/scan launches and a calibration map cached per module state, so it can go stale if weights change. The skip lists are also cached by flow data pointer, so they can go stale if that buffer is reused with new contents.

```diff
diff --git a/include/lwg_hip.h b/include/lwg_hip.h
--- a/include/lwg_hip.h
+++ b/include/lwg_hip.h
@@ -67,6 +67,15 @@
 } LwgWinoDesc;
 int lwg_winograd_panels_f32(const LwgWinoDesc* descs_dev, int ndesc, int total_blocks, lwg_stream_t stream);
 int lwg_conv2d_winograd4_f32(const LwgConvArgs* args, lwg_stream_t stream);
+typedef struct LwgConvLists {
+    const int* heavy;
+    const int* light;
+    const int* counts;
+    const float* cal;
+} LwgConvLists;
+int lwg_conv2d_winograd4_list_f32(const LwgConvArgs* args, const LwgConvLists* lists, lwg_stream_t stream);
+int lwg_conv2d_winograd4_list_applies(const LwgConvArgs* args);
+int lwg_spade_skip_lists_f32(const float* T, int B, int ns, int h, int w, int d, int* marks, int* heavy, int* light, int* counts, lwg_stream_t stream);
 int lwg_winograd4_panel_f32(const float* wpanel, float* upk, int Cin, int N, const int* tap9, lwg_stream_t stream);
 int lwg_conv2d_nhwc_bf16_hr(const LwgConvArgs* args, lwg_stream_t stream);
 int lwg_conv2d_winograd_bf16(const LwgConvArgs* args, lwg_stream_t stream);
diff --git a/ipercore_amd/_lib.py b/ipercore_amd/_lib.py
--- a/ipercore_amd/_lib.py
+++ b/ipercore_amd/_lib.py
@@ -37,6 +37,10 @@
     _fields_ = [("wpanel", ctypes.c_void_p), ("upk", ctypes.c_void_p), ("Cin", c_i), ("N", c_i), ("first_block", c_i), ("tap9", c_i * 9)]
 
 
+class LwgConvLists(ctypes.Structure):
+    _fields_ = [("heavy", c_f), ("light", c_f), ("counts", c_f), ("cal", c_f)]
+
+
 class LwgPackDesc(ctypes.Structure):
     _fields_ = [("w", c_f), ("out", c_f)] + [(n, c_i) for n in ("D1", "KHW", "transposed", "ntaps", "cin", "cin_pad", "nout", "n_pad", "Kp",
                                                                "first_block")] + [("kidx", c_i * LWG_MAX_TAPS)]
@@ -57,6 +61,9 @@
     "lwg_winograd_panel_f32": (c_i, [c_f, c_f, c_i, c_i, ctypes.POINTER(c_i), c_f]),
     "lwg_winograd_panels_f32": (c_i, [c_f, c_i, c_i, c_f]),
     "lwg_conv2d_winograd4_f32": (c_i, [ctypes.POINTER(LwgConvArgs), c_f]),
+    "lwg_conv2d_winograd4_list_f32": (c_i, [ctypes.POINTER(LwgConvArgs), ctypes.POINTER(LwgConvLists), c_f]),
+    "lwg_conv2d_winograd4_list_applies": (c_i, [ctypes.POINTER(LwgConvArgs)]),
+    "lwg_spade_skip_lists_f32": (c_i, [c_f, c_i, c_i, c_i, c_i, c_i, c_f, c_f, c_f, c_f, c_f]),
     "lwg_winograd4_panel_f32": (c_i, [c_f, c_f, c_i, c_i, ctypes.POINTER(c_i), c_f]),
     "lwg_conv2d_nhwc_bf16_hr": (c_i, [ctypes.POINTER(LwgConvArgs), c_f]),
     "lwg_conv2d_winograd_bf16": (c_i, [ctypes.POINTER(LwgConvArgs), c_f]),
diff --git a/ipercore_amd/csrc/conv_winograd4.hip b/ipercore_amd/csrc/conv_winograd4.hip
--- a/ipercore_amd/csrc/conv_winograd4.hip
+++ b/ipercore_amd/csrc/conv_winograd4.hip
@@ -70,8 +70,19 @@
     v[5] = __builtin_fmaf(-5.f, r[3], __builtin_fmaf(4.f, r[1], r[5]));
 }
 
-template <int EPI, bool TWO, bool SM = false>
-__global__ __launch_bounds__(SM ? 256 : W4_THREADS, 1) void lwg_conv_winograd4_kernel(const LwgConvArgs a) {
+__device__ __forceinline__ float w4_spade_mod(float x, float mu, float rs, float gam, float bet) { return (x - mu) * rs * (1.f + gam) + bet; }
+__device__ __forceinline__ void w4_act16(int act, floatx4 (&o)[4]) {
+    lwg_act_dispatch(act, [&](auto ACTC) {
+        constexpr int EA = decltype(ACTC)::value;
+#pragma unroll
+        for (int i = 0; i < 4; ++i)
+#pragma unroll
+            for (int c = 0; c < 4; ++c) o[i][c] = lwg_act_c<EA>(o[i][c], act);
+    });
+}
+
+template <int EPI, bool TWO, bool SM, bool LIST>
+__device__ __forceinline__ void w4_body(const LwgConvArgs& a, const LwgConvLists& sk) {
     constexpr bool SMS = SM && EPI == LWG_EPI_SPADE;
     constexpr int NVP = SM && !SMS ? 2 : 1;
     constexpr int NTH = SM ? 256 : W4_THREADS;
@@ -90,6 +101,10 @@
     const CwGrid g = cw_grid(a.B, H, W, N, 4 * W4_PBX, 4 * W4_PBY, NBV);
     const CwOrder o = cw_order(cw4_order_kind(LWG_W4_XCD, LWG_W4_CHUNK, SM, gridDim.x, N / NBV, Cin, N, g.tiles, g.total), gridDim.x, blockIdx.x, N / NBV, g);
     int blk = blockIdx.x;
+    const int nht = LIST ? min(max(__builtin_amdgcn_readfirstlane(sk.counts[0]), 0), g.tiles) : 0;
+    const int nhe = nht * (N / NBV);
+    const bool lst = LIST ? nht < g.tiles : false;
+    const bool run = lst ? blk < nhe : true;
     const int nst = Cin / W4_KS;
     const __amdgpu_buffer_rsrc_t ru = __builtin_amdgcn_make_buffer_rsrc(const_cast<float*>(a.w), 0, (int)(144u * (unsigned)Cin * (unsigned)N), 0x00020000);
     const int q = wid & 3, ct = SM ? 0 : wid >> 2;
@@ -99,7 +114,17 @@
     unsigned uvoff, uvoffc;
     auto setup = [&](int id) {
         int cb, t;
-        cw_block(o, id, cb, t);
+        if constexpr (LIST) {
+            if (lst) {
+                int slot;
+                cw_list_entry(id, N / NBV, slot, cb);
+                t = min(max(__builtin_amdgcn_readfirstlane(sk.heavy[slot]), 0), g.tiles - 1);
+            } else {
+                cw_block(o, id, cb, t);
+            }
+        } else {
+            cw_block(o, id, cb, t);
+        }
         bk.locate(a, g, t, 4 * W4_PBX, 4 * W4_PBY, SMS ? cw4_n0_spade_small(cb) : cw_n0(cb, NBV));
         int tids = tid;
         asm volatile("" : "+v"(tids));
@@ -108,7 +133,7 @@
         uvoff = (unsigned)(((lane >> 5) * 9 * N + 4 * col) * 4);
         uvoffc = (unsigned)(((lane >> 5) * 9 * N + 8 * N + col) * 4);
     };
-    setup(blk);
+    if (run) setup(blk);
     int wst[NQ];
 #pragma unroll
     for (int k = 0; k < NQ; ++k) {
@@ -362,12 +387,12 @@
 #pragma unroll
         for (int k = 0; k < NQ; ++k) rreg[k] = rld1(nst > 2 ? 2 : 1, k);
     };
-    issue_loads();
+    if (run) issue_loads();
 #ifdef LWG_W4_TS
     int lab_bi = 0;
 #endif
     W4TSA(11);
-    for (;;) {
+    if (run) for (;;) {
     W4TS(0);
 #pragma unroll
     for (int k = 0; k < NQ; ++k) {
@@ -486,7 +511,8 @@
         if (ph == 1) {
             W4TS(8);
             nblk = blk + (int)gridDim.x;
-            more = cw_has_block(o, nblk);
+            if constexpr (LIST) more = lst ? nblk < nhe : cw_has_block(o, nblk);
+            else more = cw_has_block(o, nblk);
             setup(more ? nblk : blk);
             W4TS(9);
             issue_loads();
@@ -532,7 +558,7 @@
 #pragma unroll
                 for (int i = 0; i < 4; ++i)
 #pragma unroll
-                    for (int c = 0; c < 4; ++c) o[i][c] = (ext[0][i][c] - mu[c]) * rs[c] * (1.f + gam[i][c]) + o[i][c];
+                    for (int c = 0; c < 4; ++c) o[i][c] = w4_spade_mod(ext[0][i][c], mu[c], rs[c], gam[i][c], o[i][c]);
             } else if (EPI == LWG_EPI_RESIDUAL) {
                 if (a.act == LWG_ACT_RELU_MASK) {
 #pragma unroll
@@ -544,13 +570,7 @@
                     for (int i = 0; i < 4; ++i) o[i] += ext[h][i];
                 }
             }
-            lwg_act_dispatch(a.act, [&](auto ACTC) {
-                constexpr int EA = decltype(ACTC)::value;
-#pragma unroll
-                for (int i = 0; i < 4; ++i)
-#pragma unroll
-                    for (int c = 0; c < 4; ++c) o[i][c] = lwg_act_c<EA>(o[i][c], a.act);
-            });
+            w4_act16(a.act, o);
 #pragma unroll
             for (int i = 0; i < 4; ++i)
                 __builtin_amdgcn_raw_buffer_store_b128(__builtin_bit_cast(w4_u4, o[i]), ry, (int)cw4_out_group(vo[NVP == 2 ? h : 0][i], h, EPI != LWG_EPI_SPADE && !SM), 0, W4_NT_ST);
@@ -569,6 +589,76 @@
 #ifdef LWG_W4_TS
     if (tid == 0) reinterpret_cast<unsigned long long*>(const_cast<float*>(a.res))[(size_t)blockIdx.x * 16 + 13] = (unsigned long long)lab_bi;
 #endif
+    if constexpr (LIST) {
+        typedef unsigned int w4_u4 __attribute__((ext_vector_type(4)));
+        constexpr int NQD = EPI == LWG_EPI_SPADE ? 8 : 16;
+        const int ncb = N / NBV;
+        const int nend = nhe + min(max(__builtin_amdgcn_readfirstlane(sk.counts[1]), 0), g.tiles - nht) * ncb;
+        const unsigned img_bytes = (unsigned)(H * W) * (unsigned)a.YC * 4u;
+        const __amdgpu_buffer_rsrc_t rc = __builtin_amdgcn_make_buffer_rsrc(const_cast<float*>(sk.cal), 0, (int)((unsigned)(H * W) * (unsigned)(EPI == LWG_EPI_SPADE ? N : a.YC) * 4u), 0x00020000);
+#pragma unroll 1
+        for (int id = cw_list_first_light((int)blockIdx.x, (int)gridDim.x, nhe); id < nend; id += (int)gridDim.x) {
+            int slot, cb;
+            cw_list_entry(id - nhe, ncb, slot, cb);
+            const int t = min(max(__builtin_amdgcn_readfirstlane(sk.light[slot]), 0), g.tiles - 1);
+            const int eb = __builtin_amdgcn_readfirstlane(cw_image(g, t)), en0 = cw_n0(cb, NBV);
+            int ex0, ey0;
+            cw_corner(g, t - eb * g.bx * g.by, 4 * W4_PBX, 4 * W4_PBY, ex0, ey0);
+            const __amdgpu_buffer_rsrc_t ry = __builtin_amdgcn_make_buffer_rsrc(y + (size_t)eb * H * W * a.YC, 0, (int)img_bytes, 0x00020000);
+            int px, py, q4;
+            cw4_light_elem(tid, 0, W4_THREADS, NQD, px, py, q4);
+            if constexpr (EPI == LWG_EPI_SPADE) {
+                const __amdgpu_buffer_rsrc_t re = __builtin_amdgcn_make_buffer_rsrc(const_cast<float*>(a.xn) + (size_t)eb * H * W * a.YC, 0, (int)img_bytes, 0x00020000);
+                const int cbase = en0 >> 1;
+                const floatx4 mu = *reinterpret_cast<const floatx4*>(a.mean + (size_t)eb * a.YC + cbase + 4 * q4);
+                const floatx4 rs = *reinterpret_cast<const floatx4*>(a.rstd + (size_t)eb * a.YC + cbase + 4 * q4);
+#pragma unroll 1
+                for (int it = 0; it < 512 * NQD / W4_THREADS; it += 4) {
+                    unsigned vo[4];
+                    floatx4 o[4], gam[4], xv[4];
+#pragma unroll
+                    for (int i = 0; i < 4; ++i) {
+                        cw4_light_elem(tid, it + i, W4_THREADS, NQD, px, py, q4);
+                        vo[i] = cw4_out_voff(ex0 + px, ey0 + py, H, W, a.YC, cbase + 4 * q4);
+                        const unsigned vc = cw4_out_voff(ex0 + px, ey0 + py, H, W, N, en0 + 4 * q4);
+                        gam[i] = cw_buf_load(rc, cw4_out_group(vc, 0, true), 0u);
+                        o[i] = cw_buf_load(rc, cw4_out_group(vc, 1, true), 0u);
+                        xv[i] = cw_buf_load<W4_NT_RES>(re, vo[i], 0u);
+                    }
+#pragma unroll
+                    for (int i = 0; i < 4; ++i)
+#pragma unroll
+                        for (int c = 0; c < 4; ++c) o[i][c] = w4_spade_mod(xv[i][c], mu[c], rs[c], gam[i][c], o[i][c]);
+                    w4_act16(a.act, o);
+#pragma unroll
+                    for (int i = 0; i < 4; ++i) __builtin_amdgcn_raw_buffer_store_b128(__builtin_bit_cast(w4_u4, o[i]), ry, (int)vo[i], 0, W4_NT_ST);
+                }
+            } else {
+#pragma unroll 1
+                for (int it = 0; it < 512 * NQD / W4_THREADS; it += 4) {
+                    unsigned vo[4];
+                    floatx4 o[4];
+#pragma unroll
+                    for (int i = 0; i < 4; ++i) {
+                        cw4_light_elem(tid, it + i, W4_THREADS, NQD, px, py, q4);
+                        vo[i] = cw4_out_voff(ex0 + px, ey0 + py, H, W, a.YC, a.ycoff + en0 + 4 * q4);
+                        o[i] = cw_buf_load(rc, vo[i], 0u);
+                    }
+#pragma unroll
+                    for (int i = 0; i < 4; ++i) __builtin_amdgcn_raw_buffer_store_b128(__builtin_bit_cast(w4_u4, o[i]), ry, (int)vo[i], 0, W4_NT_ST);
+                }
+            }
+        }
+    }
+}
+
+template <int EPI, bool TWO, bool SM = false>
+__global__ __launch_bounds__(SM ? 256 : W4_THREADS, 1) void lwg_conv_winograd4_kernel(const LwgConvArgs a) {
+    w4_body<EPI, TWO, SM, false>(a, LwgConvLists{});
+}
+template <int EPI>
+__global__ __launch_bounds__(W4_THREADS, 1) void lwg_conv_winograd4_list_kernel(const LwgConvArgs a, const LwgConvLists sk) {
+    w4_body<EPI, false, false, true>(a, sk);
 }
 
 
@@ -633,3 +723,22 @@
     if (a.epi == LWG_EPI_RESIDUAL) return sm ? lwg_wino4_go<LWG_EPI_RESIDUAL, true>(a, grid, lds, stream) : lwg_wino4_go<LWG_EPI_RESIDUAL, false>(a, grid, lds, stream);
     return sm ? lwg_wino4_go<LWG_EPI_NONE, true>(a, grid, lds, stream) : lwg_wino4_go<LWG_EPI_NONE, false>(a, grid, lds, stream);
 }
+
+static bool lwg_wino4_list_ok(const LwgConvArgs* pa) {
+    return pa && cw_contract_ok(*pa, 144ull, 256ll) && pa->C1 == 0 && (pa->epi == LWG_EPI_NONE || pa->epi == LWG_EPI_SPADE) &&
+           cw_contract_calib_ok(*pa) && cw_total_blocks(pa->B, pa->H, pa->W, pa->N, 4 * W4_PBX, 4 * W4_PBY, W4_NB) < (1ll << 30);
+}
+extern "C" int lwg_conv2d_winograd4_list_applies(const LwgConvArgs* pa) {
+    if (!lwg_wino4_list_ok(pa)) return 0;
+    return !(LWG_W4_SMALL && 2 * cw_total_blocks(pa->B, pa->H, pa->W, pa->N, 4 * W4_PBX, 4 * W4_PBY, W4_NB) <= lwg_device_cus());
+}
+extern "C" int lwg_conv2d_winograd4_list_f32(const LwgConvArgs* pa, const LwgConvLists* pl, lwg_stream_t stream_) {
+    if (!lwg_wino4_list_ok(pa) || !pl || !pl->heavy || !pl->light || !pl->counts || !pl->cal) return (int)hipErrorInvalidValue;
+    if (!lwg_conv2d_winograd4_list_applies(pa)) return lwg_conv2d_winograd4_f32(pa, stream_);
+    hipStream_t stream = reinterpret_cast<hipStream_t>(stream_);
+    const LwgConvArgs& a = *pa;
+    const size_t lds = (size_t)(W4_BIAS_OFF + 64) * 4;
+    const dim3 grid = cw_persistent_grid(cw_total_blocks(a.B, a.H, a.W, a.N, 4 * W4_PBX, 4 * W4_PBY, W4_NB), lwg_device_cus());
+    return a.epi == LWG_EPI_SPADE ? cw_launch_lists<lwg_conv_winograd4_list_kernel<LWG_EPI_SPADE>>(grid, W4_THREADS, lds, stream, a, *pl)
+                                  : cw_launch_lists<lwg_conv_winograd4_list_kernel<LWG_EPI_NONE>>(grid, W4_THREADS, lds, stream, a, *pl);
+}
diff --git a/ipercore_amd/csrc/lwb_attn_x.hip b/ipercore_amd/csrc/lwb_attn_x.hip
--- a/ipercore_amd/csrc/lwb_attn_x.hip
+++ b/ipercore_amd/csrc/lwb_attn_x.hip
@@ -1,5 +1,6 @@
 #include "lwg_common.h"
 #include "lwg_conv_args.h"
+#include "lwg_lwb_taps.h"
 
 typedef unsigned int uintx4 __attribute__((ext_vector_type(4)));
 
@@ -141,14 +142,7 @@
             }
         }
     };
-    auto taps_of = [&](const float2 t, float (&wt)[4], int& tx0, int& ty0) {
-        const float ix = ((t.x + 1.f) * (float)w - 1.f) * 0.5f, iy = ((t.y + 1.f) * (float)h - 1.f) * 0.5f;
-        const float fx0 = floorf(ix), fy0 = floorf(iy);
-        const float wx1 = ix - fx0, wy1 = iy - fy0, wx0 = (fx0 + 1.f) - ix, wy0 = (fy0 + 1.f) - iy;
-        tx0 = (int)fminf(fmaxf(fx0, -2.f), (float)w + 1.f);
-        ty0 = (int)fminf(fmaxf(fy0, -2.f), (float)h + 1.f);
-        wt[0] = wy0 * wx0; wt[1] = wy0 * wx1; wt[2] = wy1 * wx0; wt[3] = wy1 * wx1;
-    };
+    auto taps_of = [&](const float2 t, float (&wt)[4], int& tx0, int& ty0) { lwb_taps_of(t, w, h, wt, tx0, ty0); };
     auto fold = [&](const float (&ka)[CPL], const float (&va)[CPL], float kap, const float (&xv)[CPL], float& mrun, float& lrun, float (&o)[CPL]) {
         float dot = 0.f;
 #pragma unroll
@@ -194,7 +188,7 @@
                 float wt[4];
                 int tx0, ty0;
                 taps_of(t, wt, tx0, ty0);
-                mine |= live && tx0 >= -1 && tx0 < w && ty0 >= -1 && ty0 < h;
+                mine |= live && lwb_tap_in_image(tx0, ty0, w, h);
             }
         }
         if (__syncthreads_or(mine ? 1 : 0) == 0) {
@@ -296,7 +290,7 @@
             float wt[4];
             int tx0, ty0;
             taps_of(t, wt, tx0, ty0);
-            const bool any_tap = live && tx0 >= -1 && tx0 < w && ty0 >= -1 && ty0 < h;
+            const bool any_tap = live && lwb_tap_in_image(tx0, ty0, w, h);
             float ka[CPL], va[CPL], kap = 0.f;
 #pragma unroll
             for (int k = 0; k < CPL; ++k) ka[k] = va[k] = 0.f;
diff --git a/ipercore_amd/csrc/lwg_conv_wino.h b/ipercore_amd/csrc/lwg_conv_wino.h
--- a/ipercore_amd/csrc/lwg_conv_wino.h
+++ b/ipercore_amd/csrc/lwg_conv_wino.h
@@ -75,6 +75,17 @@
 }
 CW_FN unsigned cw4_out_group(unsigned vo, int h, bool grouped) { return vo + (grouped ? 128u * (unsigned)h : 0u); }
 
+struct CwWindow { int x0, y0, x1, y1; };
+CW_FN CwWindow cw_block_window(int x0, int y0, int ex, int ey, int d, int H, int W) {
+    return CwWindow{x0 - d > 0 ? x0 - d : 0, y0 - d > 0 ? y0 - d : 0, x0 + ex + d < W ? x0 + ex + d : W, y0 + ey + d < H ? y0 + ey + d : H};
+}
+CW_FN void cw_list_entry(int e, int ncb, int& slot, int& cb) { slot = e / ncb, cb = e - slot * ncb; }
+CW_FN int cw_list_first_light(int wg, int nwg, int nhe) { return wg >= nhe ? wg : wg + (nhe - wg + nwg - 1) / nwg * nwg; }
+CW_FN void cw4_light_elem(int tid, int it, int nth, int nq, int& px, int& py, int& q4) {
+    const int e = it * nth + tid, p = e / nq;
+    q4 = e - p * nq, px = p & 31, py = p >> 5;
+}
+
 #define CW_NO_OUT_BUFFER (-1ll)
 CW_FN bool cw_contract_ok(const LwgConvArgs& a, unsigned long long pair_bytes, long long out_slack) {
     if (!a.x0 || !a.w || !a.y || a.M <= 0 || a.ntaps != 9 || a.stride != 1 || a.omul != 1 || a.C0 <= 0 || (a.C0 % CW_KS) != 0 || a.C1 < 0 ||
@@ -92,6 +103,9 @@
     if ((unsigned long long)a.H * a.W * cmax * 4ull >= (unsigned long long)CW_OOB || pair_bytes * (a.C0 + a.C1) * a.N >= 0xffffffffull) return false;
     if (out_slack >= 0 && (unsigned long long)a.H * a.W * a.YC * 4ull + (unsigned long long)out_slack >= (unsigned long long)CW_OOB) return false;
     return true;
+}
+CW_FN bool cw_contract_calib_ok(const LwgConvArgs& a) {
+    return (unsigned long long)a.H * a.W * (unsigned long long)(a.epi == LWG_EPI_SPADE ? a.N : a.YC) * 4ull + 256ull < (unsigned long long)CW_OOB;
 }
 CW_FN bool cwb_contract_ok(const LwgConvArgs& a) {
     if (!a.x0 || !a.w || !a.y || a.B <= 0 || a.H <= 0 || a.W <= 0 || a.C0 <= 0 || a.C1 < 0 || a.N <= 0 || a.xdt != LWG_DT_BF16 || a.ydt != LWG_DT_BF16 ||
@@ -177,5 +191,12 @@
     hipLaunchKernelGGL(KERNEL, grid, dim3(threads), lds, stream, a);
     return (int)hipGetLastError();
 }
+template <void (*KERNEL)(const LwgConvArgs, const LwgConvLists)>
+static inline int cw_launch_lists(dim3 grid, unsigned threads, size_t lds, hipStream_t stream, const LwgConvArgs& a, const LwgConvLists& l) {
+    static unsigned long long done = 0ull;
+    if (hipError_t e = lwg_allow_dynamic_lds(reinterpret_cast<const void*>(KERNEL), lds, done); e != hipSuccess) return (int)e;
+    hipLaunchKernelGGL(KERNEL, grid, dim3(threads), lds, stream, a, l);
+    return (int)hipGetLastError();
+}
 static inline dim3 cw_persistent_grid(long long total, int cus) { return dim3((unsigned)(LWG_WINO_PERSIST && total > cus ? cus : total)); }
 #endif
diff --git a/ipercore_amd/csrc/lwg_lwb_taps.h b/ipercore_amd/csrc/lwg_lwb_taps.h
--- /dev/null
+++ b/ipercore_amd/csrc/lwg_lwb_taps.h
@@ -0,0 +1,12 @@
+#pragma once
+#include "lwg_common.h"
+
+__device__ __forceinline__ void lwb_taps_of(const float2 t, int w, int h, float (&wt)[4], int& tx0, int& ty0) {
+    const float ix = ((t.x + 1.f) * (float)w - 1.f) * 0.5f, iy = ((t.y + 1.f) * (float)h - 1.f) * 0.5f;
+    const float fx0 = floorf(ix), fy0 = floorf(iy);
+    const float wx1 = ix - fx0, wy1 = iy - fy0, wx0 = (fx0 + 1.f) - ix, wy0 = (fy0 + 1.f) - iy;
+    tx0 = (int)fminf(fmaxf(fx0, -2.f), (float)w + 1.f);
+    ty0 = (int)fminf(fmaxf(fy0, -2.f), (float)h + 1.f);
+    wt[0] = wy0 * wx0; wt[1] = wy0 * wx1; wt[2] = wy1 * wx0; wt[3] = wy1 * wx1;
+}
+__device__ __forceinline__ bool lwb_tap_in_image(int tx0, int ty0, int w, int h) { return tx0 >= -1 && tx0 < w && ty0 >= -1 && ty0 < h; }
diff --git a/ipercore_amd/csrc/spade_skip.hip b/ipercore_amd/csrc/spade_skip.hip
--- /dev/null
+++ b/ipercore_amd/csrc/spade_skip.hip
@@ -0,0 +1,66 @@
+#include <hip/hip_runtime.h>
+#include "lwg_common.h"
+#include "lwg_conv_wino.h"
+#include "lwg_lwb_taps.h"
+
+#define SK_EX 32
+#define SK_EY 16
+
+__global__ __launch_bounds__(256) void lwg_spade_skip_mark_kernel(const float2* __restrict__ T, int B, int ns, int h, int w, int d, int* __restrict__ marks) {
+    const CwGrid g = cw_grid(B, h, w, CW_NB, SK_EX, SK_EY, CW_NB);
+    const int t = blockIdx.x, b = cw_image(g, t);
+    int x0, y0;
+    cw_corner(g, t - b * g.bx * g.by, SK_EX, SK_EY, x0, y0);
+    const CwWindow win = cw_block_window(x0, y0, SK_EX, SK_EY, d, h, w);
+    const int ww = win.x1 - win.x0, n = ww * (win.y1 - win.y0);
+    bool mine = false;
+    for (int s = 0; s < ns; ++s) {
+        const float2* Ts = T + ((size_t)b * ns + s) * h * w;
+        for (int i = threadIdx.x; i < n; i += 256) {
+            const int yy = i / ww, y = win.y0 + yy, x = win.x0 + (i - yy * ww);
+            float wt[4];
+            int tx0, ty0;
+            lwb_taps_of(Ts[(size_t)y * w + x], w, h, wt, tx0, ty0);
+            mine |= lwb_tap_in_image(tx0, ty0, w, h);
+        }
+    }
+    const int any = __syncthreads_or(mine ? 1 : 0);
+    if (threadIdx.x == 0) marks[t] = any ? 1 : 0;
+}
+
+__global__ __launch_bounds__(1024) void lwg_spade_skip_scan_kernel(const int* __restrict__ marks, int n, int* __restrict__ heavy, int* __restrict__ light,
+                                                                   int* __restrict__ counts) {
+    __shared__ int part[1024];
+    const int tid = threadIdx.x, per = (n + 1023) / 1024;
+    const int i0 = tid * per < n ? tid * per : n, i1 = i0 + per < n ? i0 + per : n;
+    int c = 0;
+    for (int i = i0; i < i1; ++i) c += marks[i] != 0;
+    part[tid] = c;
+    __syncthreads();
+    for (int off = 1; off < 1024; off <<= 1) {
+        const int v = tid >= off ? part[tid - off] : 0;
+        __syncthreads();
+        part[tid] += v;
+        __syncthreads();
+    }
+    int hv = part[tid] - c;
+    for (int i = i0; i < i1; ++i) {
+        if (marks[i] != 0) heavy[hv++] = i;
+        else light[i - hv] = i;
+    }
+    if (tid == 1023) {
+        counts[0] = part[1023];
+        counts[1] = n - part[1023];
+    }
+}
+
+extern "C" int lwg_spade_skip_lists_f32(const float* T, int B, int ns, int h, int w, int d, int* marks, int* heavy, int* light, int* counts,
+                                        lwg_stream_t stream_) {
+    if (!T || !marks || !heavy || !light || !counts || B <= 0 || ns <= 0 || h <= 0 || w <= 0 || d < 0 || d > 64) return (int)hipErrorInvalidValue;
+    const long long tiles = cw_total_blocks(B, h, w, CW_NB, SK_EX, SK_EY, CW_NB);
+    if (tiles >= (1ll << 30) || (long long)h * w >= (1ll << 30)) return (int)hipErrorInvalidValue;
+    hipStream_t stream = reinterpret_cast<hipStream_t>(stream_);
+    hipLaunchKernelGGL(lwg_spade_skip_mark_kernel, dim3((unsigned)tiles), dim3(256), 0, stream, reinterpret_cast<const float2*>(T), B, ns, h, w, d, marks);
+    hipLaunchKernelGGL(lwg_spade_skip_scan_kernel, dim3(1), dim3(1024), 0, stream, marks, (int)tiles, heavy, light, counts);
+    return (int)hipGetLastError();
+}
diff --git a/ipercore_amd/networks/generator.py b/ipercore_amd/networks/generator.py
--- a/ipercore_amd/networks/generator.py
+++ b/ipercore_amd/networks/generator.py
@@ -145,6 +145,23 @@
         else:
             y = ops.conv2d(x, spec, x.new_empty(B, H, W, spec.N), act=ops.ACT_TANH)
             return ops.nhwc_to_nchw(y, channels=3)
+
+
+def spade_calibration(st, x):
+    _, h, w, C = x.shape
+    cal = st.setdefault("cal", {})
+    if (h, w) not in cal:
+        hook, ops.CONV_HOOK = ops.CONV_HOOK, None
+        try:
+            z = x.new_zeros(1, h, w, C)
+            T = x.new_full((1, 1, h, w, 2), -2.0)
+            att = ops.lwb_attention_x(z, z, x.new_zeros(1, h, w), z, st["bv"], T, torch.empty_like(z))
+            actv = ops.conv2d(att, st["shared"], x.new_empty(1, h, w, st["shared"].N), act=ops.ACT_RELU)
+            gb = ops.conv2d(actv, st["gb"], x.new_empty(1, h, w, st["gb"].N))
+        finally:
+            ops.CONV_HOOK = hook
+        cal[(h, w)] = (actv, gb)
+    return cal[(h, w)]
 
 
 def _param_version(gen):
@@ -262,8 +279,14 @@
         att = ops.lwb_attention_x(tsf_x, kv[0], kv[2], kv[1], st["bv"], flow, torch.empty_like(tsf_x), stats=ws,
                                   src_batched=batched)
         ops.instnorm_finalize(ws, B, C, nrec, mean, rstd, eps=1e-5)
-        actv = ops.conv2d(att, st["shared"], tsf_x.new_empty(B, h, w, st["shared"].N), act=ops.ACT_RELU)
-        return ops.conv2d(actv, st["gb"], torch.empty_like(tsf_x), epi=ops.EPI_SPADE, xn=tsf_x, mean=mean, rstd=rstd)
+        actv, out = tsf_x.new_empty(B, h, w, st["shared"].N), torch.empty_like(tsf_x)
+        l1 = l5 = None
+        if ops.conv2d_lists_apply(att, st["shared"], actv, act=ops.ACT_RELU):
+            l1 = scratch.lists(flow, ops.SPADE_SKIP_D[0]) + (spade_calibration(st, tsf_x)[0],)
+        if ops.conv2d_lists_apply(actv, st["gb"], out, epi=ops.EPI_SPADE, xn=tsf_x, mean=mean, rstd=rstd):
+            l5 = scratch.lists(flow, ops.SPADE_SKIP_D[1]) + (spade_calibration(st, tsf_x)[1],)
+        ops.conv2d(att, st["shared"], actv, act=ops.ACT_RELU, **({} if l1 is None else {"lists": l1}))
+        return ops.conv2d(actv, st["gb"], out, epi=ops.EPI_SPADE, xn=tsf_x, mean=mean, rstd=rstd, **({} if l5 is None else {"lists": l5}))
 
     @staticmethod
     def _upconv(x, specs, act, q4=False):
@@ -472,6 +495,12 @@
             self.flows[key] = ops.flow_resize(Tst, h, w)
         return self.flows[key]
 
+    def lists(self, flow, d):
+        key = ("lists", flow.shape[2], flow.shape[3], d, flow.data_ptr())
+        if key not in self.flows:
+            self.flows[key] = ops.spade_skip_lists(flow, d)
+        return self.flows[key]
+
     def get(self, n, device):
         if self.buf is None or self.buf.numel() < n or self.buf.device != device:
             self.buf = torch.empty(max(n, 1 << 16), device=device, dtype=torch.float32)
diff --git a/ipercore_amd/ops.py b/ipercore_amd/ops.py
--- a/ipercore_amd/ops.py
+++ b/ipercore_amd/ops.py
@@ -293,6 +293,37 @@
         _lib.check(_lib.lib().lwg_winograd4_panel_f32(_ptr(spec.w), _ptr(U), cin, N, tap9, _stream()), "lwg_winograd4_panel_f32")
         spec._wwino4 = U
     return spec._wwino4
+
+
+SPADE_SKIP = True
+SPADE_SKIP_D = (1, 5)
+
+
+_LISTS_APPLY = {}
+
+
+def spade_skip_lists(flow, d):
+    B, ns, h, w, two = flow.shape
+    assert two == 2 and flow.dtype == torch.float32
+    tiles = B * ((h + 15) // 16) * ((w + 31) // 32)
+    buf = torch.empty(3 * tiles + 2, device=flow.device, dtype=torch.int32)
+    marks, heavy, light, counts = buf[:tiles], buf[tiles:2 * tiles], buf[2 * tiles:3 * tiles], buf[3 * tiles:]
+    i32 = torch.int32
+    _lib.check(_lib.lib().lwg_spade_skip_lists_f32(_ptr(flow), B, ns, h, w, int(d), _ptr(marks, i32), _ptr(heavy, i32), _ptr(light, i32),
+                                                   _ptr(counts, i32), _stream()), "lwg_spade_skip_lists_f32")
+    return heavy, light, counts
+
+
+def conv2d_lists_apply(x0, spec, y, epi=EPI_NONE, act=ACT_NONE, xn=None, mean=None, rstd=None):
+    if not SPADE_SKIP or CONV_PRECISION != "winograd" or not x0.is_cuda or x0.dtype != torch.float32 or not _wino4_use(spec, False) or \
+            not _wino_eligible(spec, x0, y, None, epi, act, None, False):
+        return False
+    key = (x0.shape, y.shape, spec.Cin, spec.N, epi, act)
+    if key not in _LISTS_APPLY:
+        a = conv_args(x0, spec, y, None, epi, act, None, xn, mean, rstd)
+        a.w = _ptr(_wwino4(spec))
+        _LISTS_APPLY[key] = bool(_lib.lib().lwg_conv2d_winograd4_list_applies(a))
+    return _LISTS_APPLY[key]
 
 
 def conv_args(x0, spec, y, x1=None, epi=EPI_NONE, act=ACT_NONE, res=None, xn=None, mean=None, rstd=None,
@@ -336,12 +367,14 @@
 
 
 def conv2d(x0, spec, y, x1=None, epi=EPI_NONE, act=ACT_NONE, res=None, xn=None, mean=None, rstd=None,
-           out_hw=None, ycoff=0, splitk=False, q4=False):
+           out_hw=None, ycoff=0, splitk=False, q4=False, lists=None):
     a = conv_args(x0, spec, y, x1, epi, act, res, xn, mean, rstd, out_hw, ycoff, q4)
     if q4 and (splitk or CONV_PRECISION not in ("fp32", "winograd") or x0.dtype != torch.float32):
         raise ValueError("channel-quad-plane outputs: fp32 activations on the fp32 MFMA path, no split-K")
     if CONV_HOOK is not None:
         CONV_HOOK(True, a.M, spec, epi, None)
+    if lists is not None and not (x0.dtype == torch.float32 and y.dtype == torch.float32 and CONV_PRECISION == "winograd" and _wino4_use(spec, splitk)):
+        raise ValueError("lists: the F(4x4, 3x3) launches of the \"winograd\" mode only (conv2d_lists_apply)")
     kind, sliced, extra = "direct", True, 0
     if x0.dtype == torch.bfloat16:
         kind = "bf16"
@@ -375,7 +408,12 @@
         if _wino4_use(spec, splitk):
             a.w = _ptr(_wwino4(spec))
             kind = "winograd4"
-            _lib.check(_lib.lib().lwg_conv2d_winograd4_f32(a, _stream()), "lwg_conv2d_winograd4_f32")
+            if lists is not None:
+                i32 = torch.int32
+                ld = _lib.LwgConvLists(_ptr(lists[0], i32), _ptr(lists[1], i32), _ptr(lists[2], i32), _ptr(lists[3]))
+                _lib.check(_lib.lib().lwg_conv2d_winograd4_list_f32(a, ctypes.byref(ld), _stream()), "lwg_conv2d_winograd4_list_f32")
+            else:
+                _lib.check(_lib.lib().lwg_conv2d_winograd4_f32(a, _stream()), "lwg_conv2d_winograd4_f32")
         elif nws:
             a.w = _ptr(_wwino(spec))
             ws, extra = torch.empty(nws, device=x0.device, dtype=torch.float32), 1
```

Result: faster. 1296 frames/s, median of 6 (+6.6%).
